# NERSC/swin_v2_weather

Hardware: AMD Instinct MI355X
Metric: ERA5 samples/sec (73x721x1440) swin_73var depth12 (higher is better)
Workload: dtype bf16

## Files before the change

include/swv2.h:

```cpp
#ifndef SWV2_H
#define SWV2_H
#include <stddef.h>
#include <stdint.h>

#ifdef __cplusplus
extern "C" {
#endif

#define SWV2_VERSION 109

enum {
    SWV2_OK = 0,
    SWV2_ERR_INVALID = -1,
    SWV2_ERR_UNSUPPORTED = -2,
    SWV2_ERR_LAUNCH = -3
};

int swv2_version(void);
const char* swv2_last_error(void);

int swv2_attn_geometry(int L, int head_dim, int* Lp, int* DP);

int swv2_attn_fwd_regime(int L, int head_dim, int has_bias, int dbg);

#define SWV2_ATTN_FIRST_GEN 16
#define SWV2_ATTN_PLAIN_STATS 8192
#define SWV2_ATTN_BWD_TWO_PHASE 32

typedef struct swv2_attn_args {
    const void* qkvh;
    const float* logit_scale;
    const float* bias;
    const void* bias_pack;
    void* oh;
    float* lse;
    const void* doh;
    const float* rnorm;
    void* dqkvh;
    float* dlogit_scale;
    float* dbias;
    int Bw, heads, L, head_dim;
    int nwh, nww;
    int mask_thr;
    int max_chunks;
    int dbg;
    void* dbias_ws;
    size_t dbias_ws_bytes;
    int dbias_partials;
} swv2_attn_args;

size_t swv2_attn_dbias_ws_bytes(int heads, int L, int max_chunks);

int swv2_attn_bias_chunks(int Bw);

size_t swv2_attn_pack_bias_bytes(int heads, int L);
int swv2_attn_pack_bias(const float* bias, int heads, int L, void* out, void* stream);
int swv2_attn_pack_bias_multi(const float* bias, int ntab, int heads, int L, void* out, void* stream);

int swv2_attn_fwd(const swv2_attn_args* a, void* stream);
int swv2_attn_bwd(const swv2_attn_args* a, void* stream);


enum swv2_operand_kind {
    SWV2_OP_F32 = 0,
    SWV2_OP_BF16 = 1,
    SWV2_OP_BF16_GELU = 2,
    SWV2_OP_HEADS = 3,
    SWV2_OP_PATCH = 4,
    SWV2_OP_MERGE_LN = 5,
    SWV2_OP_BF16_CSCALE = 6
};

typedef struct swv2_operand {
    int kind;
    const void* ptr;
    const int32_t* rowidx;
    const float* aux0;
    const float* aux1;
    const float* aux2;
    const float* aux3;
    long ld;
    int rows, cols;
    int p[4];
} swv2_operand;

enum swv2_epilogue_kind {
    SWV2_EPI_BF16 = 0,
    SWV2_EPI_F32 = 1,
    SWV2_EPI_QKV_HEADS = 2,
    SWV2_EPI_GELU_GRAD = 3,
    SWV2_EPI_UNPATCH = 4,
    SWV2_EPI_HEADS = 5,
    SWV2_EPI_F32_ACC = 6,
    SWV2_EPI_BF16_GELU = 7,
    SWV2_EPI_UNPATCH_LOSS = 8
};

typedef struct swv2_epilogue {
    int kind;
    void* out;
    const float* bias;
    const void* aux;
    float* aux_out;
    const int32_t* rowidx;
    long ld;
    int p[5];
    const float* loss_tar;
    const float* loss_qw;
    float* loss_part;
    void* loss_resid;
    int q[3];
} swv2_epilogue;

int swv2_linear(const swv2_operand* a, const void* w_bf16, const swv2_epilogue* e, int N, void* stream);

#define SWV2_LINEAR_RESIDENT_QKV128 0
#define SWV2_LINEAR_RESIDENT_QKV192X3 1
#define SWV2_LINEAR_RESIDENT_DX128 2
#define SWV2_LINEAR_WIDE_DMA 3
#define SWV2_LINEAR_WIDE 4
#define SWV2_LINEAR_TILE64 5
#define SWV2_LINEAR_TILE128 6
int swv2_linear_kernel(const swv2_operand* a, const swv2_epilogue* e, int N);

int swv2_linear_wgrad(const swv2_operand* dy, const swv2_operand* x, float* dW, float* db, const int32_t* nmap,
                      const int32_t* kmap, int ldw, int splits, void* stream);
size_t swv2_linear_wgrad_ws_bytes(int M, int N, int K, int splits);
int swv2_linear_wgrad_ws(const swv2_operand* dy, const swv2_operand* x, float* dW, float* db, const int32_t* nmap,
                         const int32_t* kmap, int ldw, int splits, void* ws, size_t ws_bytes, void* stream);
#define SWV2_WGRAD_WIDE 0
#define SWV2_WGRAD_TILE 1
int swv2_linear_wgrad_kernel(const swv2_operand* dy, const swv2_operand* x, int splits, size_t ws_bytes);

typedef struct swv2_wgrad_item {
    swv2_operand dy, x;
    float* dW;
    float* db;
    const int32_t* nmap;
    const int32_t* kmap;
    int ldw;
} swv2_wgrad_item;
size_t swv2_block_wgrad_ws_bytes(int C, int hidden, int heads_dp, int slices);
int swv2_block_wgrad(const swv2_wgrad_item* items4, int slices, void* ws, size_t ws_bytes, void* stream);
#define SWV2_BLOCK_WGRAD_SLAB 0
#define SWV2_BLOCK_WGRAD_GROUPED 1
int swv2_block_wgrad_kernel(const swv2_wgrad_item* items4, int slices, size_t ws_bytes);

int swv2_qk_normalize(void* qkvh_bf16, float* rnorm, int Bw, int heads, int Lp, int L, int DP, void* stream);

int swv2_prep_weight(const float* w, int rows, int cols, int transpose, const int32_t* row_map, int out_rows,
                     const int32_t* col_map, int out_cols, void* out_bf16, void* stream);

typedef struct swv2_prep_item {
    const float* w;
    int rows, cols, transpose;
    const int32_t* row_map;
    int out_rows;
    const int32_t* col_map;
    int out_cols;
    void* out;
    int out_f32;
} swv2_prep_item;
int swv2_prep_chunk(void);
int swv2_prep_item_chunks(int out_rows, int out_cols, int transpose);
int swv2_prep_multi(const swv2_prep_item* items_dev, const int* chunks_dev, int n_chunks, void* stream);

#define SWV2_LN_BWD_MAX_BLOCKS 512
typedef struct swv2_ln_args {
    const void* a;
    const float* res;
    const float* gamma;
    const float* beta;
    const float* scale;
    const int32_t* rowidx;
    float* y;
    float* mean;
    float* rstd;
    const float* dy;
    void* da;
    float* dgamma;
    float* dbeta;
    float* ws;
    int M, C, res_mod, rows_per_sample;
    float eps;
} swv2_ln_args;

int swv2_ln_residual_fwd(const swv2_ln_args* a, void* stream);
int swv2_ln_residual_bwd(const swv2_ln_args* a, void* stream);

int swv2_batch_sum(const float* in, float* out, int B, long n, int accumulate, void* stream);

int swv2_merge_stats(const float* x, float* mean, float* rstd, int B, int H, int W, int C, float eps, void* stream);
int swv2_merge_ln_bwd(const float* x, const void* dn_bf16, const float* gamma, const float* mean, const float* rstd,
                      float* dx, float* dgamma, float* dbeta, int B, int H, int W, int C, void* stream);

int swv2_loss_sums(const float* prd, const float* tar, const float* quad_w, float* sums, int BC, int H, int W, void* stream);
int swv2_loss_grad(const float* prd, const float* tar, const float* quad_w, const float* coef, float* dprd, int BC, int H,
                   int W, void* stream);
#define SWV2_LOSS_PART_SLICES 8
#define SWV2_LOSS_GROUP_ROWS 32
#define SWV2_LOSS_DUMP_BYTES 2048
#define SWV2_LOSS_RESID_PITCH(N) (((N) + 63) / 64 * 64)
int swv2_loss_part_reduce(const float* part, int M, int T, int B, int Cout, int Ct, int coff, float* sums, void* stream);
int swv2_loss_resid_to_image(const void* resid, const float* coef, const float* add, float* out, int B, int Cout, int H, int W, int Cs, int Cadd,
                             void* stream);
int swv2_loss_finalize(const float* sums, int layers, const float* chw, int BC, int C, int absolute, int squared, float* loss, float* coef,
                       void* stream);

int swv2_adam_step(float* p, const float* g, float* m, float* v, long n, float lr, float beta1, float beta2, float eps,
                   int step, float grad_inv_scale, void* stream);

typedef struct swv2_adam_item {
    float* p;
    const float* g;
    float* m;
    float* v;
    long n;
} swv2_adam_item;
int swv2_adam_chunk(void);
int swv2_adam_multi(const swv2_adam_item* items_dev, const int* chunks_dev, int n_chunks, float lr, float beta1, float beta2,
                    float eps, int step, float grad_inv_scale, void* stream);

int swv2_era5_select_normalize(const float* raw, float* out, const int* chan, const float* mean, const float* stdv, int B, int S,
                               int Csel, int Craw, int Hraw, int Wraw, int H, int W, int Cout_total, int coff, void* stream);
int swv2_era5_zenith(float* out, const float* sun, int B, int nz, int H, int W, int Cout_total, int coff, void* stream);
int swv2_era5_static(const float* stat, float* out, int B, int Cs, int H, int W, int Cout_total, int coff, void* stream);

typedef struct {
    const void* oh;
    const void* wp;
    const float* bp;
    const float* gamma; const float* beta; const float* scale;
    const int32_t* rowidx;
    const float* x;
    void* a1; float* mean; float* rstd;
    float* y;
    int Bw, Lp, heads, C, rows_per_sample;
    float eps;
} swv2_proj_ln_args;
typedef struct {
    const float* dy;
    const void* a1; const float* mean; const float* rstd; const float* gamma; const float* scale;
    const int32_t* rowidx;
    const void* wpt;
    void* da1;
    void* doh;
    float* dgamma; float* dbeta; float* ws;
    int Bw, Lp, heads, C, rows_per_sample;
} swv2_proj_ln_bwd_args;
int swv2_proj_ln_supported(int C, int heads, int head_pad);
size_t swv2_proj_ln_bwd_ws_floats(int Mw, int C);
int swv2_proj_ln_fwd(const swv2_proj_ln_args* a, void* stream);
int swv2_proj_ln_bwd(const swv2_proj_ln_bwd_args* a, void* stream);

typedef struct {
    const float* x;
    const void* w1;
    const float* b1;
    const void* w2;
    const float* b2;
    const float* gamma;
    const float* beta;
    const float* scale;
    void* hpre;
    void* a2;
    float* mean;
    float* rstd;
    float* y;
    int M, C, hidden, rows_per_sample;
    float eps;
} swv2_mlp_args;
int swv2_mlp_supported(int C, int hidden);
int swv2_mlp_recompute_supported(int C, int hidden);
int swv2_mlp_fwd(const swv2_mlp_args* a, void* stream);

typedef struct {
    const float* dy;
    const void* a2;
    const float* mean;
    const float* rstd;
    const float* gamma;
    const float* scale;
    const void* hpre;
    const void* w2t;
    const void* w1t;
    void* da2;
    void* dh;
    float* dx;
    float* dgamma;
    float* dbeta;
    float* ws;
    int M, C, hidden, rows_per_sample;
    const float* x;
    const void* w1;
    const float* b1;
} swv2_mlp_bwd_args;
size_t swv2_mlp_bwd_ws_floats(int M, int C);
int swv2_mlp_bwd(const swv2_mlp_bwd_args* a, void* stream);

int swv2_cpb_fwd(const float* w1, const float* b1, const float* w2, const float* b2, const void* keep_bf16, float* bias,
                 int wh, int ww, int heads, int hidden, float drop_p, void* stream);
int swv2_cpb_bwd(const float* dbias, const float* w1, const float* b1, const float* w2, const void* keep_bf16, float* dw1,
                 float* db1, float* dw2, float* db2, int wh, int ww, int heads, int hidden, float drop_p, void* stream);
size_t swv2_cpb_bwd_ws_bytes(int wh, int ww, int heads, int hidden);
int swv2_cpb_bwd_ws(const float* dbias, const float* w1, const float* b1, const float* w2, const void* keep_bf16, float* dw1,
                    float* db1, float* dw2, float* db2, int wh, int ww, int heads, int hidden, float drop_p, void* ws,
                    size_t ws_bytes, void* stream);

int swv2_cpb_fwd_multi(const float* const* params_dev, int nblk, const uint32_t* keep_bits, float* bias, int wh, int ww, int heads,
                       int hidden, float drop_p, void* stream);
size_t swv2_cpb_bwd_multi_ws_bytes(int nblk, int wh, int ww, int heads, int hidden);
int swv2_cpb_bwd_multi(const float* dbias_tables, int nchunk, const float* const* params_dev, int nblk, const uint32_t* keep_bits,
                       float* grads, int wh, int ww, int heads, int hidden, float drop_p, void* ws, size_t ws_bytes, void* stream);

typedef struct swv2_block_desc {
    int B, T, C, heads, head_dim, hidden, L, Lp, DP, nwh, nww, mask_thr;
    const int32_t* rowidx;
    const int32_t* qkv_map;
    const int32_t* proj_map;
    const float *logit_scale, *qkv_b_pad, *proj_b, *n1_w, *n1_b, *fc1_b, *fc2_b, *n2_w, *n2_b;
    const void *w_qkv, *w_proj, *w_fc1, *w_fc2;
    const void *w_qkvt, *w_projt, *w_fc1t, *w_fc2t;
    const float* x;
    const float* bias;
    void* bias_pack;
    const float* dp1;
    const float* dp2;
    void* qkvh;  float* rnorm; void* oh; float* lse; void* a1; float* mean1; float* rstd1; float* x1;
    void* hpre;  void* hact;   void* a2; float* mean2; float* rstd2;
    float* x2;
    const float* dx2;
    void *da2, *dh, *da1, *doh, *dqkvh;
    float* dx1;
    float* ln_ws;
    float* dx;
    float *d_logit_scale, *d_bias, *d_qkv_w, *d_qkv_b, *d_proj_w, *d_proj_b, *d_n1_w, *d_n1_b, *d_fc1_w, *d_fc1_b,
          *d_fc2_w, *d_fc2_b, *d_n2_w, *d_n2_b;
    int wgrad_splits;
    int ev_kernel;
    void* ev_start;
    void* ev_stop;
    int fuse_proj_ln;
    int fuse_mlp;
    void* wgrad_ws;
    size_t wgrad_ws_bytes;
    int wgrad_group;
    void* grad_zero;
    size_t grad_zero_bytes;
    size_t ln_ws_floats;
    int bias_prepacked;
    float* dbias_part;
    size_t dbias_part_bytes;
} swv2_block_desc;

enum swv2_block_step {
    SWV2_STEP_RNORM_ZERO = 1,
    SWV2_STEP_QKV,
    SWV2_STEP_QK_NORMALIZE,
    SWV2_STEP_PACK_BIAS,
    SWV2_STEP_ATTN_FWD,
    SWV2_STEP_PROJ, SWV2_STEP_LN1_FWD,
    SWV2_STEP_PROJ_LN_FWD,
    SWV2_STEP_FC1, SWV2_STEP_FC2, SWV2_STEP_LN2_FWD,
    SWV2_STEP_MLP_FWD,
    SWV2_STEP_LN2_BWD, SWV2_STEP_WGRAD_FC2, SWV2_STEP_DH, SWV2_STEP_WGRAD_FC1, SWV2_STEP_DX1,
    SWV2_STEP_MLP_BWD,
    SWV2_STEP_LN1_BWD,
    SWV2_STEP_PROJ_LN_BWD,
    SWV2_STEP_WGRAD_PROJ, SWV2_STEP_DOH, SWV2_STEP_ATTN_BWD, SWV2_STEP_WGRAD_QKV, SWV2_STEP_DX,
    SWV2_STEP_LN_FOLD,
    SWV2_STEP_WGRAD_GROUP,
    SWV2_STEP_COUNT
};
#define SWV2_BLOCK_MAX_STEPS 12
enum { SWV2_DBIAS_NONE = 0,
       SWV2_DBIAS_ATOMICS = 1,
       SWV2_DBIAS_WGRAD_WS = 2,
       SWV2_DBIAS_PART = 3 };
typedef struct swv2_block_plan_t {
    int mlp_fused;
    int proj_ln_fused;
    int ln_deferred;
    int wgrad_grouped;
    int wgrad_kernel;
    int grad_zero_in_kernel;
    int attn_fwd_chunks, attn_bwd_chunks;
    int dbias_dest;
    size_t need_hact_bytes;
    size_t need_ln_ws_floats;
    size_t need_wgrad_ws_bytes;
    int n_fwd, n_bwd;
    int fwd[SWV2_BLOCK_MAX_STEPS], bwd[SWV2_BLOCK_MAX_STEPS];
} swv2_block_plan_t;
int swv2_block_plan(const swv2_block_desc* d, swv2_block_plan_t* out);
int swv2_block_step_id(int step);
const char* swv2_block_step_name(int step);

int swv2_block_fwd(const swv2_block_desc* d, void* stream);
int swv2_block_bwd(const swv2_block_desc* d, void* stream);

#ifdef __cplusplus
}
#endif
#endif
```

swin_v2_weather_amd/_lib.py:

```python
from __future__ import annotations

import ctypes as C
import os
import subprocess
import threading

HERE = os.path.dirname(os.path.abspath(__file__))
CSRC = os.path.join(HERE, "csrc")
LIB_PATH = os.environ.get("SWV2_LIB") or os.path.join(HERE, "libswv2.so")
SOURCES = ["capi.hip", "attn.hip", "attn2.hip", "attn_bwd_stream.hip", "attn_wide.hip", "attn_d256.hip", "gemm.hip", "gemm_tn.hip", "gemm_tn_slab.hip", "rowops.hip", "block.hip", "cpb.hip", "mlp.hip", "proj_ln.hip", "dataio.hip"]

ABI_VERSION = 109

_lib = None
_lock = threading.Lock()


class Swv2Error(RuntimeError):
    pass


def build_library(force: bool = False, verbose: bool = False) -> str:
    srcs = [os.path.join(CSRC, s) for s in SOURCES]
    deps = srcs + [os.path.join(CSRC, "common.h"), os.path.join(CSRC, "gemm_common.h"), os.path.join(CSRC, "attn_common.h"), os.path.join(HERE, "..", "include", "swv2.h")]
    if not force and os.path.exists(LIB_PATH) and all(os.path.getmtime(LIB_PATH) >= os.path.getmtime(d) for d in deps):
        return LIB_PATH
    hipcc = os.environ.get("HIPCC", "/opt/rocm/bin/hipcc")
    objs, procs = [], []
    os.makedirs(os.path.join(HERE, "build"), exist_ok=True)
    for s in srcs:
        o = os.path.join(HERE, "build", os.path.basename(s) + ".o")
        objs.append(o)
        cmd = [hipcc, "--offload-arch=gfx950", "-O3", "-std=c++17", "-fPIC", "-c", s, "-o", o]
        procs.append((cmd, subprocess.Popen(cmd, stdout=subprocess.PIPE, stderr=subprocess.STDOUT)))
    for cmd, p in procs:
        out, _ = p.communicate()
        if p.returncode != 0:
            raise Swv2Error("hipcc failed: %s\n%s" % (" ".join(cmd), out.decode()))
        if verbose and out:
            print(out.decode())
    cmd = [hipcc, "--offload-arch=gfx950", "-shared", "-fPIC", "-o", LIB_PATH] + objs
    r = subprocess.run(cmd, stdout=subprocess.PIPE, stderr=subprocess.STDOUT)
    if r.returncode != 0:
        raise Swv2Error("link failed: %s\n%s" % (" ".join(cmd), r.stdout.decode()))
    return LIB_PATH


def source_hash() -> str:
    import glob
    import hashlib
    h = hashlib.sha256()
    files = sorted(glob.glob(os.path.join(CSRC, "*"))) + [os.path.join(HERE, "..", "include", "swv2.h")]
    for f in files:
        if os.path.isfile(f):
            h.update(os.path.basename(f).encode())
            h.update(open(f, "rb").read())
    return h.hexdigest()[:16]


class AttnArgs(C.Structure):
    _fields_ = [("qkvh", C.c_void_p), ("logit_scale", C.c_void_p), ("bias", C.c_void_p), ("bias_pack", C.c_void_p), ("oh", C.c_void_p),
                ("lse", C.c_void_p), ("doh", C.c_void_p), ("rnorm", C.c_void_p), ("dqkvh", C.c_void_p),
                ("dlogit_scale", C.c_void_p), ("dbias", C.c_void_p),
                ("Bw", C.c_int), ("heads", C.c_int), ("L", C.c_int), ("head_dim", C.c_int),
                ("nwh", C.c_int), ("nww", C.c_int), ("mask_thr", C.c_int), ("max_chunks", C.c_int), ("dbg", C.c_int),
                ("dbias_ws", C.c_void_p), ("dbias_ws_bytes", C.c_size_t), ("dbias_partials", C.c_int)]


class Operand(C.Structure):
    _fields_ = [("kind", C.c_int), ("ptr", C.c_void_p), ("rowidx", C.c_void_p), ("aux0", C.c_void_p),
                ("aux1", C.c_void_p), ("aux2", C.c_void_p), ("aux3", C.c_void_p), ("ld", C.c_long),
                ("rows", C.c_int), ("cols", C.c_int), ("p", C.c_int * 4)]


class PrepItem(C.Structure):
    _fields_ = [("w", C.c_void_p), ("rows", C.c_int), ("cols", C.c_int), ("transpose", C.c_int), ("row_map", C.c_void_p),
                ("out_rows", C.c_int), ("col_map", C.c_void_p), ("out_cols", C.c_int), ("out", C.c_void_p), ("out_f32", C.c_int)]


class WgradItem(C.Structure):
    _fields_ = [("dy", Operand), ("x", Operand), ("dW", C.c_void_p), ("db", C.c_void_p), ("nmap", C.c_void_p),
                ("kmap", C.c_void_p), ("ldw", C.c_int)]


class Epilogue(C.Structure):
    _fields_ = [("kind", C.c_int), ("out", C.c_void_p), ("bias", C.c_void_p), ("aux", C.c_void_p),
                ("aux_out", C.c_void_p), ("rowidx", C.c_void_p), ("ld", C.c_long), ("p", C.c_int * 5),
                ("loss_tar", C.c_void_p), ("loss_qw", C.c_void_p), ("loss_part", C.c_void_p),
                ("loss_resid", C.c_void_p),
                ("q", C.c_int * 3)]


class ProjLnArgs(C.Structure):
    _fields_ = [(n, C.c_void_p) for n in ("oh", "wp", "bp", "gamma", "beta", "scale", "rowidx", "x", "a1", "mean", "rstd", "y")] + \
               [(n, C.c_int) for n in ("Bw", "Lp", "heads", "C", "rows_per_sample")] + [("eps", C.c_float)]


class ProjLnBwdArgs(C.Structure):
    _fields_ = [(n, C.c_void_p) for n in ("dy", "a1", "mean", "rstd", "gamma", "scale", "rowidx", "wpt", "da1", "doh", "dgamma", "dbeta",
                                           "ws")] + [(n, C.c_int) for n in ("Bw", "Lp", "heads", "C", "rows_per_sample")]


class MlpArgs(C.Structure):
    _fields_ = [(n, C.c_void_p) for n in ("x", "w1", "b1", "w2", "b2", "gamma", "beta", "scale", "hpre", "a2", "mean", "rstd", "y")] + \
               [(n, C.c_int) for n in ("M", "C", "hidden", "rows_per_sample")] + [("eps", C.c_float)]


class MlpBwdArgs(C.Structure):
    _fields_ = [(n, C.c_void_p) for n in ("dy", "a2", "mean", "rstd", "gamma", "scale", "hpre", "w2t", "w1t", "da2", "dh", "dx",
                                           "dgamma", "dbeta", "ws")] + [(n, C.c_int) for n in ("M", "C", "hidden", "rows_per_sample")] + \
               [(n, C.c_void_p) for n in ("x", "w1", "b1")]


class LnArgs(C.Structure):
    _fields_ = [("a", C.c_void_p), ("res", C.c_void_p), ("gamma", C.c_void_p), ("beta", C.c_void_p),
                ("scale", C.c_void_p), ("rowidx", C.c_void_p), ("y", C.c_void_p), ("mean", C.c_void_p),
                ("rstd", C.c_void_p), ("dy", C.c_void_p), ("da", C.c_void_p), ("dgamma", C.c_void_p),
                ("dbeta", C.c_void_p), ("ws", C.c_void_p), ("M", C.c_int), ("C", C.c_int), ("res_mod", C.c_int),
                ("rows_per_sample", C.c_int), ("eps", C.c_float)]


LN_BWD_MAX_BLOCKS = 512
ATTN_FIRST_GEN, ATTN_PLAIN_STATS, ATTN_BWD_TWO_PHASE = 16, 8192, 32
LOSS_PART_SLICES = 8
LOSS_GROUP_ROWS = 32
LOSS_DUMP_BYTES = 2048


def loss_resid_pitch(n: int) -> int:
    return (n + 63) // 64 * 64
class BlockDesc(C.Structure):
    _fields_ = ([(n, C.c_int) for n in ("B", "T", "C", "heads", "head_dim", "hidden", "L", "Lp", "DP", "nwh", "nww", "mask_thr")] +
                [(n, C.c_void_p) for n in (
                    "rowidx", "qkv_map", "proj_map",
                    "logit_scale", "qkv_b_pad", "proj_b", "n1_w", "n1_b", "fc1_b", "fc2_b", "n2_w", "n2_b",
                    "w_qkv", "w_proj", "w_fc1", "w_fc2", "w_qkvt", "w_projt", "w_fc1t", "w_fc2t",
                    "x", "bias", "bias_pack", "dp1", "dp2",
                    "qkvh", "rnorm", "oh", "lse", "a1", "mean1", "rstd1", "x1", "hpre", "hact", "a2", "mean2", "rstd2", "x2",
                    "dx2", "da2", "dh", "da1", "doh", "dqkvh", "dx1", "ln_ws", "dx",
                    "d_logit_scale", "d_bias", "d_qkv_w", "d_qkv_b", "d_proj_w", "d_proj_b", "d_n1_w", "d_n1_b", "d_fc1_w",
                    "d_fc1_b", "d_fc2_w", "d_fc2_b", "d_n2_w", "d_n2_b")] +
                [("wgrad_splits", C.c_int), ("ev_kernel", C.c_int), ("ev_start", C.c_void_p), ("ev_stop", C.c_void_p),
                 ("fuse_proj_ln", C.c_int), ("fuse_mlp", C.c_int), ("wgrad_ws", C.c_void_p), ("wgrad_ws_bytes", C.c_size_t), ("wgrad_group", C.c_int), ("grad_zero", C.c_void_p),
                 ("grad_zero_bytes", C.c_size_t), ("ln_ws_floats", C.c_size_t),
                 ("bias_prepacked", C.c_int), ("dbias_part", C.c_void_p), ("dbias_part_bytes", C.c_size_t)])


BLOCK_MAX_STEPS = 12
DBIAS_NONE, DBIAS_ATOMICS, DBIAS_WGRAD_WS, DBIAS_PART = range(4)


class BlockPlan(C.Structure):
    _fields_ = ([(n, C.c_int) for n in ("mlp_fused", "proj_ln_fused", "ln_deferred", "wgrad_grouped", "wgrad_kernel", "grad_zero_in_kernel",
                                        "attn_fwd_chunks", "attn_bwd_chunks", "dbias_dest")] +
                [(n, C.c_size_t) for n in ("need_hact_bytes", "need_ln_ws_floats", "need_wgrad_ws_bytes")] +
                [("n_fwd", C.c_int), ("n_bwd", C.c_int), ("fwd", C.c_int * BLOCK_MAX_STEPS), ("bwd", C.c_int * BLOCK_MAX_STEPS)])

    def steps(self, phase):
        lib = load()
        return [lib.swv2_block_step_name(s).decode() for s in getattr(self, phase)[:getattr(self, "n_" + phase)]]


def block_plan(desc: BlockDesc) -> BlockPlan:
    plan = BlockPlan()
    check(load().swv2_block_plan(C.byref(desc), C.byref(plan)), "swv2_block_plan")
    return plan


OP_F32, OP_BF16, OP_BF16_GELU, OP_HEADS, OP_PATCH, OP_MERGE_LN, OP_BF16_CSCALE = range(7)
EPI_BF16, EPI_F32, EPI_QKV_HEADS, EPI_GELU_GRAD, EPI_UNPATCH, EPI_HEADS, EPI_F32_ACC, EPI_BF16_GELU, EPI_UNPATCH_LOSS = range(9)
LINEAR_RESIDENT_QKV128, LINEAR_RESIDENT_QKV192X3, LINEAR_RESIDENT_DX128, LINEAR_WIDE_DMA, LINEAR_WIDE, LINEAR_TILE64, LINEAR_TILE128 = range(7)
LINEAR_WIDE_KERNELS, LINEAR_TILE_KERNELS = (LINEAR_WIDE_DMA, LINEAR_WIDE), (LINEAR_TILE64, LINEAR_TILE128)
WGRAD_WIDE, WGRAD_TILE = range(2)
BLOCK_WGRAD_SLAB, BLOCK_WGRAD_GROUPED = range(2)

_P, _I, _L, _F = C.c_void_p, C.c_int, C.c_long, C.c_float
SYMBOLS = {
    "swv2_version": (_I, []),
    "swv2_last_error": (C.c_char_p, []),
    "swv2_attn_geometry": (_I, [_I, _I, C.POINTER(_I), C.POINTER(_I)]),
    "swv2_attn_fwd_regime": (_I, [_I, _I, _I, _I]),
    "swv2_attn_pack_bias_bytes": (C.c_size_t, [_I, _I]),
    "swv2_attn_dbias_ws_bytes": (C.c_size_t, [_I, _I, _I]),
    "swv2_attn_pack_bias": (_I, [_P, _I, _I, _P, _P]),
    "swv2_attn_pack_bias_multi": (_I, [_P, _I, _I, _I, _P, _P]),
    "swv2_attn_bias_chunks": (_I, [_I]),
    "swv2_attn_fwd": (_I, [C.POINTER(AttnArgs), _P]),
    "swv2_attn_bwd": (_I, [C.POINTER(AttnArgs), _P]),
    "swv2_linear": (_I, [C.POINTER(Operand), _P, C.POINTER(Epilogue), _I, _P]),
    "swv2_linear_kernel": (_I, [C.POINTER(Operand), C.POINTER(Epilogue), _I]),
    "swv2_linear_wgrad_kernel": (_I, [C.POINTER(Operand), C.POINTER(Operand), _I, C.c_size_t]),
    "swv2_block_wgrad_kernel": (_I, [C.POINTER(WgradItem), _I, C.c_size_t]),
    "swv2_linear_wgrad": (_I, [C.POINTER(Operand), C.POINTER(Operand), _P, _P, _P, _P, _I, _I, _P]),
    "swv2_linear_wgrad_ws_bytes": (C.c_size_t, [_I, _I, _I, _I]),
    "swv2_qk_normalize": (_I, [_P, _P, _I, _I, _I, _I, _I, _P]),
    "swv2_block_wgrad_ws_bytes": (C.c_size_t, [_I, _I, _I, _I]),
    "swv2_block_wgrad": (_I, [C.POINTER(WgradItem), _I, _P, C.c_size_t, _P]),
    "swv2_linear_wgrad_ws": (_I, [C.POINTER(Operand), C.POINTER(Operand), _P, _P, _P, _P, _I, _I, _P, C.c_size_t, _P]),
    "swv2_prep_weight": (_I, [_P, _I, _I, _I, _P, _I, _P, _I, _P, _P]),
    "swv2_ln_residual_fwd": (_I, [C.POINTER(LnArgs), _P]),
    "swv2_ln_residual_bwd": (_I, [C.POINTER(LnArgs), _P]),
    "swv2_batch_sum": (_I, [_P, _P, _I, _L, _I, _P]),
    "swv2_merge_stats": (_I, [_P, _P, _P, _I, _I, _I, _I, _F, _P]),
    "swv2_merge_ln_bwd": (_I, [_P, _P, _P, _P, _P, _P, _P, _P, _I, _I, _I, _I, _P]),
    "swv2_loss_sums": (_I, [_P, _P, _P, _P, _I, _I, _I, _P]),
    "swv2_loss_grad": (_I, [_P, _P, _P, _P, _P, _I, _I, _I, _P]),
    "swv2_loss_part_reduce": (_I, [_P, _I, _I, _I, _I, _I, _I, _P, _P]),
    "swv2_loss_resid_to_image": (_I, [_P, _P, _P, _P, _I, _I, _I, _I, _I, _I, _P]),
    "swv2_loss_finalize": (_I, [_P, _I, _P, _I, _I, _I, _I, _P, _P, _P]),
    "swv2_prep_chunk": (_I, []),
    "swv2_prep_item_chunks": (_I, [_I, _I, _I]),
    "swv2_prep_multi": (_I, [_P, _P, _I, _P]),
    "swv2_adam_chunk": (_I, []),
    "swv2_adam_multi": (_I, [_P, _P, _I, _F, _F, _F, _F, _I, _F, _P]),
    "swv2_adam_step": (_I, [_P, _P, _P, _P, _L, _F, _F, _F, _F, _I, _F, _P]),
    "swv2_era5_select_normalize": (_I, [_P, _P, _P, _P, _P] + [_I] * 10 + [_P]),
    "swv2_era5_zenith": (_I, [_P, _P, _I, _I, _I, _I, _I, _I, _P]),
    "swv2_era5_static": (_I, [_P, _P, _I, _I, _I, _I, _I, _I, _P]),
    "swv2_proj_ln_supported": (_I, [_I, _I, _I]),
    "swv2_proj_ln_bwd_ws_floats": (C.c_size_t, [_I, _I]),
    "swv2_proj_ln_fwd": (_I, [C.POINTER(ProjLnArgs), _P]),
    "swv2_proj_ln_bwd": (_I, [C.POINTER(ProjLnBwdArgs), _P]),
    "swv2_mlp_supported": (_I, [_I, _I]),
    "swv2_mlp_recompute_supported": (_I, [_I, _I]),
    "swv2_mlp_fwd": (_I, [C.POINTER(MlpArgs), _P]),
    "swv2_mlp_bwd_ws_floats": (C.c_size_t, [_I, _I]),
    "swv2_mlp_bwd": (_I, [C.POINTER(MlpBwdArgs), _P]),
    "swv2_cpb_fwd": (_I, [_P, _P, _P, _P, _P, _P, _I, _I, _I, _I, _F, _P]),
    "swv2_cpb_bwd": (_I, [_P, _P, _P, _P, _P, _P, _P, _P, _P, _I, _I, _I, _I, _F, _P]),
    "swv2_cpb_bwd_ws": (_I, [_P, _P, _P, _P, _P, _P, _P, _P, _P, _I, _I, _I, _I, _F, _P, C.c_size_t, _P]),
    "swv2_cpb_bwd_ws_bytes": (C.c_size_t, [_I, _I, _I, _I]),
    "swv2_cpb_fwd_multi": (_I, [_P, _I, _P, _P, _I, _I, _I, _I, _F, _P]),
    "swv2_cpb_bwd_multi_ws_bytes": (C.c_size_t, [_I, _I, _I, _I, _I]),
    "swv2_cpb_bwd_multi": (_I, [_P, _I, _P, _I, _P, _P, _I, _I, _I, _I, _F, _P, C.c_size_t, _P]),
    "swv2_block_plan": (_I, [C.POINTER(BlockDesc), C.POINTER(BlockPlan)]),
    "swv2_block_step_id": (_I, [_I]),
    "swv2_block_step_name": (C.c_char_p, [_I]),
    "swv2_block_fwd": (_I, [C.POINTER(BlockDesc), _P]),
    "swv2_block_bwd": (_I, [C.POINTER(BlockDesc), _P]),
}


def load() -> C.CDLL:
    global _lib
    if _lib is not None:
        return _lib
    with _lock:
        if _lib is None:
            if not os.path.exists(LIB_PATH):
                raise Swv2Error(f"{LIB_PATH} not found: run `python -c 'import __graft_entry__ as g; g.build()'` "
                                "(the HIP library is required; there is no fallback path)")
            import torch
            lib = C.CDLL(LIB_PATH)
            for name, (res, args) in SYMBOLS.items():
                fn = getattr(lib, name)
                fn.restype, fn.argtypes = res, args
            got = lib.swv2_version()
            if got != ABI_VERSION:
                raise Swv2Error(f"{LIB_PATH} reports ABI revision {got}, this binding mirrors revision {ABI_VERSION} of include/swv2.h: "
                                "rebuild the library (python -c 'import __graft_entry__ as g; g.build()')")
            _lib = lib
    return _lib


def check(rc: int, what: str = "") -> None:
    if rc != 0:
        msg = load().swv2_last_error()
        raise Swv2Error(f"{what} failed with code {rc}: {msg.decode() if msg else ''}")
```

swin_v2_weather_amd/csrc/block.hip:

```cpp
#include "common.h"

namespace {

swv2_operand op(int kind, const void* p, int rows, int cols, long ld, const int32_t* rowidx = nullptr) {
    swv2_operand o = {};
    o.kind = kind; o.ptr = p; o.rowidx = rowidx; o.ld = ld; o.rows = rows; o.cols = cols;
    return o;
}
swv2_operand op_heads(const void* p, int Bw, int heads, int parts, int Lp, int DP) {
    swv2_operand o = op(SWV2_OP_HEADS, p, Bw * Lp, parts * heads * DP, parts);
    o.p[0] = heads; o.p[2] = Lp; o.p[3] = DP;
    return o;
}
swv2_epilogue epi(int kind, void* out, long ld, const float* bias = nullptr, const void* aux = nullptr,
                  float* aux_out = nullptr, const int32_t* rowidx = nullptr) {
    swv2_epilogue e = {};
    e.kind = kind; e.out = out; e.ld = ld; e.bias = bias; e.aux = aux; e.aux_out = aux_out; e.rowidx = rowidx;
    return e;
}
swv2_attn_args attn(const swv2_block_desc* d, int max_chunks) {
    swv2_attn_args a = {};
    a.qkvh = d->qkvh; a.logit_scale = d->logit_scale; a.bias = d->bias; a.bias_pack = d->bias ? d->bias_pack : nullptr;
    a.oh = d->oh; a.lse = d->lse;
    a.Bw = d->B * d->nwh * d->nww; a.heads = d->heads; a.L = d->L; a.head_dim = d->head_dim; a.nwh = d->nwh; a.nww = d->nww;
    a.mask_thr = d->mask_thr; a.max_chunks = max_chunks;
    return a;
}
void wgrad_items(const swv2_block_desc* d, bool fused, swv2_wgrad_item it[4]) {
    const int BT = d->B * d->T, Bw = d->B * d->nwh * d->nww, Mw = Bw * d->Lp, C = d->C, h = d->heads, hid = d->hidden;
    it[0].dy = op(SWV2_OP_BF16, d->da2, BT, C, C);
    it[0].x = fused ? op(SWV2_OP_BF16_GELU, d->hpre, BT, hid, hid) : op(SWV2_OP_BF16, d->hact, BT, hid, hid);
    it[0].dW = d->d_fc2_w; it[0].db = d->d_fc2_b; it[0].ldw = hid;
    it[1].dy = op(SWV2_OP_BF16, d->dh, BT, hid, hid); it[1].x = op(SWV2_OP_F32, d->x1, BT, C, C);
    it[1].dW = d->d_fc1_w; it[1].db = d->d_fc1_b; it[1].ldw = C;
    it[2].dy = op(SWV2_OP_BF16, d->da1, Mw, C, C); it[2].x = op_heads(d->oh, Bw, h, 1, d->Lp, d->DP);
    it[2].dW = d->d_proj_w; it[2].db = d->d_proj_b; it[2].kmap = d->proj_map; it[2].ldw = C;
    it[3].dy = op_heads(d->dqkvh, Bw, h, 3, d->Lp, d->DP); it[3].x = op(SWV2_OP_F32, d->x, Mw, C, C, d->rowidx);
    it[3].dW = d->d_qkv_w; it[3].db = d->d_qkv_b; it[3].nmap = d->qkv_map; it[3].ldw = C;
}
#define TRY(x) do { int rc_ = (x); if (rc_) return rc_; } while (0)

const struct { int id; const char* name; } STEPS[SWV2_STEP_COUNT] = {
    {0, "end"},
    {0, "rnorm_zero"}, {1, "qkv"}, {0, "qk_normalize"}, {0, "pack_bias"}, {2, "attn_fwd"}, {3, "proj"}, {4, "ln1_fwd"}, {3, "proj_ln_fwd"},
    {5, "fc1"}, {6, "fc2"}, {7, "ln2_fwd"}, {5, "mlp_fwd"},
    {11, "ln2_bwd"}, {12, "wgrad_fc2"}, {13, "dh"}, {14, "wgrad_fc1"}, {15, "dx1"}, {13, "mlp_bwd"}, {16, "ln1_bwd"}, {16, "proj_ln_bwd"},
    {17, "wgrad_proj"}, {18, "doh"}, {19, "attn_bwd"}, {20, "wgrad_qkv"}, {21, "dx"}, {0, "ln_fold"}, {22, "wgrad_group"},
};
static_assert(SWV2_STEP_WGRAD_GROUP + 1 == SWV2_STEP_COUNT && SWV2_STEP_MLP_FWD == 12 && SWV2_STEP_LN2_BWD == 13, "STEPS follows enum swv2_block_step");

#define LAUNCH(step, x)                                                                                     \
    do {                                                                                                    \
        const bool t_ = d->ev_kernel == STEPS[step].id && d->ev_start && d->ev_stop;                         \
        if (t_) (void)hipEventRecord((hipEvent_t)d->ev_start, (hipStream_t)st);                             \
        TRY(x);                                                                                             \
        if (t_) (void)hipEventRecord((hipEvent_t)d->ev_stop, (hipStream_t)st);                              \
    } while (0)

int plan_block(const swv2_block_desc* d, swv2_block_plan_t* p) {
    SWV2_CHECK_ARG(d && p, "swv2_block_plan: null descriptor or plan");
    SWV2_CHECK_ARG(d->B > 0 && d->T > 0 && d->C > 0 && d->heads > 0 && d->hidden > 0 && d->Lp > 0 && d->DP > 0 && d->nwh > 0 && d->nww > 0,
                   "swv2_block_plan: non-positive geometry");
    *p = {};
    const int BT = d->B * d->T, Bw = d->B * d->nwh * d->nww, Mw = Bw * d->Lp, C = d->C, h = d->heads, hid = d->hidden;
    const int sp = d->wgrad_splits > 0 ? d->wgrad_splits : 64;
    const size_t ws_bytes = d->wgrad_ws ? d->wgrad_ws_bytes : 0;
    const size_t ln_pair = swv2_mlp_bwd_ws_floats(BT, C) + swv2_proj_ln_bwd_ws_floats(Mw, C);
    p->need_ln_ws_floats = std::max((size_t)SWV2_LN_BWD_MAX_BLOCKS * 2 * C, ln_pair);
    p->need_wgrad_ws_bytes = d->wgrad_group ? swv2_block_wgrad_ws_bytes(C, hid, h * d->DP, 0) : 0;
    const int prod[4][3] = {{BT, C, hid}, {BT, hid, C}, {Mw, C, h * d->DP}, {Mw, 3 * h * d->DP, C}};
    for (const auto& q : prod)
        p->need_wgrad_ws_bytes = std::max(p->need_wgrad_ws_bytes, swv2_linear_wgrad_ws_bytes(q[0], q[1], q[2], sp));

    p->mlp_fused = d->fuse_mlp && swv2_mlp_supported(C, hid);
    p->proj_ln_fused = d->fuse_proj_ln && swv2_proj_ln_supported(C, h, d->DP);
    p->need_hact_bytes = p->mlp_fused ? 0 : (size_t)BT * hid * 2;
    p->ln_deferred = p->mlp_fused && p->proj_ln_fused && d->ln_ws_floats >= ln_pair;
    p->wgrad_grouped = d->wgrad_group && p->mlp_fused && d->wgrad_ws && ws_bytes >= swv2_block_wgrad_ws_bytes(C, hid, h * d->DP, 0);
    p->wgrad_kernel = -1;
    p->grad_zero_in_kernel = p->mlp_fused && d->grad_zero != nullptr;
    p->attn_fwd_chunks = d->bias ? 32 : 64;
    p->attn_bwd_chunks = 64;
    if (d->bias) {
        p->attn_bwd_chunks = swv2_attn_bias_chunks(Bw);
        p->dbias_dest = d->dbias_part ? SWV2_DBIAS_PART : ws_bytes ? SWV2_DBIAS_WGRAD_WS : SWV2_DBIAS_ATOMICS;
    } else if (d->Lp == 176 && h <= 256) {
        p->attn_bwd_chunks = 256 / h;
    }

    auto fwd = [&](int s) { p->fwd[p->n_fwd++] = s; };
    auto bwd = [&](int s) { p->bwd[p->n_bwd++] = s; };
    const bool wide = d->DP > 64;
    if (wide) fwd(SWV2_STEP_RNORM_ZERO);
    fwd(SWV2_STEP_QKV);
    if (wide) fwd(SWV2_STEP_QK_NORMALIZE);
    if (d->bias && d->bias_pack && !d->bias_prepacked) fwd(SWV2_STEP_PACK_BIAS);
    fwd(SWV2_STEP_ATTN_FWD);
    if (p->proj_ln_fused) fwd(SWV2_STEP_PROJ_LN_FWD);
    else { fwd(SWV2_STEP_PROJ); fwd(SWV2_STEP_LN1_FWD); }
    if (p->mlp_fused) fwd(SWV2_STEP_MLP_FWD);
    else { fwd(SWV2_STEP_FC1); fwd(SWV2_STEP_FC2); fwd(SWV2_STEP_LN2_FWD); }

    const bool single = !p->wgrad_grouped;
    if (p->mlp_fused) {
        bwd(SWV2_STEP_MLP_BWD);
        if (single) { bwd(SWV2_STEP_WGRAD_FC2); bwd(SWV2_STEP_WGRAD_FC1); }
    } else {
        bwd(SWV2_STEP_LN2_BWD); bwd(SWV2_STEP_WGRAD_FC2); bwd(SWV2_STEP_DH); bwd(SWV2_STEP_WGRAD_FC1); bwd(SWV2_STEP_DX1);
    }
    bwd(p->proj_ln_fused ? SWV2_STEP_PROJ_LN_BWD : SWV2_STEP_LN1_BWD);
    if (single) bwd(SWV2_STEP_WGRAD_PROJ);
    if (!p->proj_ln_fused) bwd(SWV2_STEP_DOH);
    bwd(SWV2_STEP_ATTN_BWD);
    if (single) bwd(SWV2_STEP_WGRAD_QKV);
    bwd(SWV2_STEP_DX);
    if (p->ln_deferred && single) bwd(SWV2_STEP_LN_FOLD);
    if (p->wgrad_grouped) bwd(SWV2_STEP_WGRAD_GROUP);
    return SWV2_OK;
}

}

extern "C" int swv2_block_step_id(int step) { return step > 0 && step < SWV2_STEP_COUNT ? STEPS[step].id : -1; }
extern "C" const char* swv2_block_step_name(int step) { return step > 0 && step < SWV2_STEP_COUNT ? STEPS[step].name : nullptr; }

extern "C" int swv2_block_plan(const swv2_block_desc* d, swv2_block_plan_t* p) {
    TRY(plan_block(d, p));
    if (p->wgrad_grouped) {
        swv2_wgrad_item it[4] = {};
        wgrad_items(d, true, it);
        p->wgrad_kernel = swv2_block_wgrad_kernel(it, 0, d->wgrad_ws_bytes);
    }
    return SWV2_OK;
}

extern "C" int swv2_block_fwd(const swv2_block_desc* d, void* st) {
    SWV2_CHECK_ARG(d && d->x && d->x2 && d->qkvh && d->rowidx, "swv2_block_fwd: null descriptor field");
    swv2_block_plan_t p;
    TRY(plan_block(d, &p));
    SWV2_CHECK_ARG(d->hact || !p.need_hact_bytes, "swv2_block_fwd: the separate MLP kernels need hact (swv2_block_plan: need_hact_bytes)");
    const int BT = d->B * d->T, Bw = d->B * d->nwh * d->nww, Mw = Bw * d->Lp, C = d->C, h = d->heads, hid = d->hidden;
    for (int i = 0; i < p.n_fwd; ++i) switch (p.fwd[i]) {
    case SWV2_STEP_RNORM_ZERO:
        if (hipMemsetAsync(d->rnorm, 0, (size_t)Bw * h * 2 * d->Lp * sizeof(float), (hipStream_t)st) != hipSuccess) {
            swv2_set_error("swv2_block_fwd: hipMemsetAsync(rnorm) failed");
            return SWV2_ERR_LAUNCH;
        }
        break;
    case SWV2_STEP_QKV: {
        swv2_operand a = op(SWV2_OP_F32, d->x, Mw, C, C, d->rowidx);
        swv2_epilogue e = epi(SWV2_EPI_QKV_HEADS, d->qkvh, 0, d->qkv_b_pad, nullptr, d->rnorm);
        e.p[0] = h; e.p[2] = d->Lp; e.p[3] = d->DP; e.p[4] = d->L;
        LAUNCH(SWV2_STEP_QKV, swv2_linear(&a, d->w_qkv, &e, 3 * h * d->DP, st));
    } break;
    case SWV2_STEP_QK_NORMALIZE: TRY(swv2_qk_normalize(d->qkvh, (float*)d->rnorm, Bw, h, d->Lp, d->L, d->DP, st)); break;
    case SWV2_STEP_PACK_BIAS: TRY(swv2_attn_pack_bias(d->bias, h, d->L, d->bias_pack, st)); break;
    case SWV2_STEP_ATTN_FWD: {
        swv2_attn_args a = attn(d, p.attn_fwd_chunks);
        LAUNCH(SWV2_STEP_ATTN_FWD, swv2_attn_fwd(&a, st));
    } break;
    case SWV2_STEP_PROJ_LN_FWD: {
        swv2_proj_ln_args m = {};
        m.oh = d->oh; m.wp = d->w_proj; m.bp = d->proj_b; m.gamma = d->n1_w; m.beta = d->n1_b; m.scale = d->dp1; m.rowidx = d->rowidx;
        m.x = d->x; m.a1 = d->a1; m.mean = d->mean1; m.rstd = d->rstd1; m.y = d->x1; m.Bw = Bw; m.Lp = d->Lp; m.heads = h; m.C = C;
        m.rows_per_sample = d->T; m.eps = 1e-5f;
        LAUNCH(SWV2_STEP_PROJ_LN_FWD, swv2_proj_ln_fwd(&m, st));
    } break;
    case SWV2_STEP_PROJ: {
        swv2_operand a = op_heads(d->oh, Bw, h, 1, d->Lp, d->DP);
        swv2_epilogue e = epi(SWV2_EPI_BF16, d->a1, C, d->proj_b);
        LAUNCH(SWV2_STEP_PROJ, swv2_linear(&a, d->w_proj, &e, C, st));
    } break;
    case SWV2_STEP_LN1_FWD: {
        swv2_ln_args l = {};
        l.a = d->a1; l.res = d->x; l.gamma = d->n1_w; l.beta = d->n1_b; l.scale = d->dp1; l.rowidx = d->rowidx; l.y = d->x1;
        l.mean = d->mean1; l.rstd = d->rstd1; l.M = Mw; l.C = C; l.res_mod = 0; l.rows_per_sample = d->T; l.eps = 1e-5f;
        LAUNCH(SWV2_STEP_LN1_FWD, swv2_ln_residual_fwd(&l, st));
    } break;
    case SWV2_STEP_MLP_FWD: {
        swv2_mlp_args m = {};
        m.x = d->x1; m.w1 = d->w_fc1; m.b1 = d->fc1_b; m.w2 = d->w_fc2; m.b2 = d->fc2_b; m.gamma = d->n2_w; m.beta = d->n2_b;
        m.scale = d->dp2; m.hpre = d->hpre; m.a2 = d->a2; m.mean = d->mean2; m.rstd = d->rstd2; m.y = d->x2;
        m.M = BT; m.C = C; m.hidden = hid; m.rows_per_sample = d->T; m.eps = 1e-5f;
        LAUNCH(SWV2_STEP_MLP_FWD, swv2_mlp_fwd(&m, st));
    } break;
    case SWV2_STEP_FC1: {
        swv2_operand a = op(SWV2_OP_F32, d->x1, BT, C, C);
        swv2_epilogue e = epi(SWV2_EPI_BF16_GELU, d->hpre, hid, d->fc1_b, nullptr, (float*)d->hact);
        LAUNCH(SWV2_STEP_FC1, swv2_linear(&a, d->w_fc1, &e, hid, st));
    } break;
    case SWV2_STEP_FC2: {
        swv2_operand a = op(SWV2_OP_BF16, d->hact, BT, hid, hid);
        swv2_epilogue e = epi(SWV2_EPI_BF16, d->a2, C, d->fc2_b);
        LAUNCH(SWV2_STEP_FC2, swv2_linear(&a, d->w_fc2, &e, C, st));
    } break;
    case SWV2_STEP_LN2_FWD: {
        swv2_ln_args l = {};
        l.a = d->a2; l.res = d->x1; l.gamma = d->n2_w; l.beta = d->n2_b; l.scale = d->dp2; l.y = d->x2; l.mean = d->mean2;
        l.rstd = d->rstd2; l.M = BT; l.C = C; l.res_mod = 0; l.rows_per_sample = d->T; l.eps = 1e-5f;
        LAUNCH(SWV2_STEP_LN2_FWD, swv2_ln_residual_fwd(&l, st));
    } break;
    }
    return SWV2_OK;
}

extern "C" int swv2_block_bwd(const swv2_block_desc* d, void* st) {
    SWV2_CHECK_ARG(d && d->dx2 && d->dx && d->da2 && d->dh && d->dx1 && d->da1 && d->doh && d->dqkvh && d->ln_ws,
                   "swv2_block_bwd: null descriptor field");
    swv2_block_plan_t p;
    TRY(plan_block(d, &p));
    SWV2_CHECK_ARG(d->hact || !p.need_hact_bytes, "swv2_block_bwd: the separate MLP kernels need hact (swv2_block_plan: need_hact_bytes)");
    const int BT = d->B * d->T, Bw = d->B * d->nwh * d->nww, Mw = Bw * d->Lp, C = d->C, h = d->heads, hid = d->hidden;
    const int sp = d->wgrad_splits > 0 ? d->wgrad_splits : 64;
    swv2_wgrad_item it[4] = {};
    wgrad_items(d, p.mlp_fused, it);
    float* const ln1_ws = p.ln_deferred ? d->ln_ws + swv2_mlp_bwd_ws_floats(BT, C) : d->ln_ws;
    int n_ln1 = 0, n_ln2 = 0;
    for (int i = 0; i < p.n_bwd; ++i) switch (const int s = p.bwd[i]; s) {
    case SWV2_STEP_MLP_BWD: {
        swv2_mlp_bwd_args m = {};
        m.dy = d->dx2; m.a2 = d->a2; m.mean = d->mean2; m.rstd = d->rstd2; m.gamma = d->n2_w; m.scale = d->dp2; m.hpre = d->hpre;
        m.w2t = d->w_fc2t; m.w1t = d->w_fc1t; m.da2 = d->da2; m.dh = d->dh; m.dx = d->dx1; m.dgamma = d->d_n2_w;
        m.dbeta = d->d_n2_b; m.ws = d->ln_ws; m.M = BT; m.C = C; m.hidden = hid; m.rows_per_sample = d->T;
        LAUNCH(SWV2_STEP_MLP_BWD, swv2_mlp_bwd_impl(&m, st, p.ln_deferred ? &n_ln2 : nullptr, p.grad_zero_in_kernel ? (float*)d->grad_zero : nullptr,
                                                    (long)(d->grad_zero_bytes / 4)));
    } break;
    case SWV2_STEP_LN2_BWD: {
        swv2_ln_args l = {};
        l.a = d->a2; l.dy = d->dx2; l.gamma = d->n2_w; l.scale = d->dp2; l.mean = d->mean2; l.rstd = d->rstd2; l.da = d->da2;
        l.dgamma = d->d_n2_w; l.dbeta = d->d_n2_b; l.ws = d->ln_ws; l.M = BT; l.C = C; l.rows_per_sample = d->T;
        LAUNCH(SWV2_STEP_LN2_BWD, swv2_ln_residual_bwd(&l, st));
    } break;
    case SWV2_STEP_WGRAD_FC2: case SWV2_STEP_WGRAD_FC1: case SWV2_STEP_WGRAD_PROJ: case SWV2_STEP_WGRAD_QKV: {
        const swv2_wgrad_item& w = it[s == SWV2_STEP_WGRAD_FC2 ? 0 : s == SWV2_STEP_WGRAD_FC1 ? 1 : s == SWV2_STEP_WGRAD_PROJ ? 2 : 3];
        LAUNCH(s, swv2_linear_wgrad_ws(&w.dy, &w.x, w.dW, w.db, w.nmap, w.kmap, w.ldw, sp, d->wgrad_ws, d->wgrad_ws_bytes, st));
    } break;
    case SWV2_STEP_DH: {
        swv2_epilogue e = epi(SWV2_EPI_GELU_GRAD, d->dh, hid, nullptr, d->hpre);
        LAUNCH(SWV2_STEP_DH, swv2_linear(&it[0].dy, d->w_fc2t, &e, hid, st));
    } break;
    case SWV2_STEP_DX1: {
        swv2_epilogue e = epi(SWV2_EPI_F32, d->dx1, C, nullptr, d->dx2);
        LAUNCH(SWV2_STEP_DX1, swv2_linear(&it[1].dy, d->w_fc1t, &e, C, st));
    } break;
    case SWV2_STEP_PROJ_LN_BWD: {
        swv2_proj_ln_bwd_args m = {};
        m.dy = d->dx1; m.a1 = d->a1; m.mean = d->mean1; m.rstd = d->rstd1; m.gamma = d->n1_w; m.scale = d->dp1; m.rowidx = d->rowidx;
        m.wpt = d->w_projt; m.da1 = d->da1; m.doh = d->doh; m.dgamma = d->d_n1_w; m.dbeta = d->d_n1_b; m.ws = ln1_ws;
        m.Bw = Bw; m.Lp = d->Lp; m.heads = h; m.C = C; m.rows_per_sample = d->T;
        LAUNCH(SWV2_STEP_PROJ_LN_BWD, swv2_proj_ln_bwd_impl(&m, st, p.ln_deferred ? &n_ln1 : nullptr));
    } break;
    case SWV2_STEP_LN1_BWD: {
        swv2_ln_args l = {};
        l.a = d->a1; l.dy = d->dx1; l.gamma = d->n1_w; l.scale = d->dp1; l.rowidx = d->rowidx; l.mean = d->mean1; l.rstd = d->rstd1;
        l.da = d->da1; l.dgamma = d->d_n1_w; l.dbeta = d->d_n1_b; l.ws = d->ln_ws; l.M = Mw; l.C = C; l.rows_per_sample = d->T;
        LAUNCH(SWV2_STEP_LN1_BWD, swv2_ln_residual_bwd(&l, st));
    } break;
    case SWV2_STEP_DOH: {
        swv2_epilogue e = epi(SWV2_EPI_HEADS, d->doh, 0);
        e.p[0] = h; e.p[2] = d->Lp; e.p[3] = d->DP; e.p[4] = d->L;
        LAUNCH(SWV2_STEP_DOH, swv2_linear(&it[2].dy, d->w_projt, &e, h * d->DP, st));
    } break;
    case SWV2_STEP_ATTN_BWD: {
        swv2_attn_args a = attn(d, p.attn_bwd_chunks);
        a.doh = d->doh; a.rnorm = d->rnorm; a.dqkvh = d->dqkvh; a.dlogit_scale = d->d_logit_scale; a.dbias = d->d_bias;
        if (p.dbias_dest == SWV2_DBIAS_PART) { a.dbias_ws = d->dbias_part; a.dbias_ws_bytes = d->dbias_part_bytes; a.dbias_partials = 1; }
        if (p.dbias_dest == SWV2_DBIAS_WGRAD_WS) { a.dbias_ws = d->wgrad_ws; a.dbias_ws_bytes = d->wgrad_ws_bytes; }
        LAUNCH(SWV2_STEP_ATTN_BWD, swv2_attn_bwd(&a, st));
    } break;
    case SWV2_STEP_DX: {
        swv2_epilogue e = epi(SWV2_EPI_F32, d->dx, C, nullptr, d->dx1, nullptr, d->rowidx);
        LAUNCH(SWV2_STEP_DX, swv2_linear(&it[3].dy, d->w_qkvt, &e, C, st));
    } break;
    case SWV2_STEP_LN_FOLD:
        swv2_launch_ln_partials_reduce2(d->ln_ws, d->d_n2_w, d->d_n2_b, n_ln2, ln1_ws, d->d_n1_w, d->d_n1_b, n_ln1, C, (hipStream_t)st);
        break;
    case SWV2_STEP_WGRAD_GROUP: {
        swv2_ln_partials lnp = {{d->ln_ws, ln1_ws}, {d->d_n2_w, d->d_n1_w}, {d->d_n2_b, d->d_n1_b}, {n_ln2, n_ln1}, C};
        LAUNCH(SWV2_STEP_WGRAD_GROUP, swv2_block_wgrad_ln(it, 0, d->wgrad_ws, d->wgrad_ws_bytes, p.ln_deferred ? &lnp : nullptr, st));
    } break;
    }
    return SWV2_OK;
}
```

swin_v2_weather_amd/csrc/common.h:

```cpp
#pragma once
#include <hip/hip_runtime.h>
#include <stdint.h>
#include <stdio.h>
#include <type_traits>

#include "../../include/swv2.h"

typedef short bf16x4 __attribute__((ext_vector_type(4)));
typedef short bf16x8 __attribute__((ext_vector_type(8)));
typedef __bf16 bf4_t __attribute__((ext_vector_type(4)));
typedef __bf16 bf2_t __attribute__((ext_vector_type(2)));
typedef float f32x4 __attribute__((ext_vector_type(4)));
typedef float f32x2 __attribute__((ext_vector_type(2)));

#define SWV2_LOG2E 1.4426950408889634f
#define SWV2_LN100 4.605170185988092f
#define SWV2_NEG_BIG (-1.0e30f)

__device__ __forceinline__ float bf2f(uint16_t v) { return __uint_as_float(((uint32_t)v) << 16); }
__device__ __forceinline__ float bf2f(short v) { return __uint_as_float(((uint32_t)(uint16_t)v) << 16); }
__device__ __forceinline__ uint16_t f2bf(float f) { return __builtin_bit_cast(uint16_t, (__bf16)f); }
__device__ __forceinline__ uint32_t f2bf2(float lo, float hi) {
    f32x2 v = {lo, hi};
    return __builtin_bit_cast(uint32_t, __builtin_convertvector(v, bf2_t));
}
__device__ __forceinline__ bf16x4 f2bf4(f32x4 v) {
    const uint32_t p[2] = {f2bf2(v[0], v[1]), f2bf2(v[2], v[3])};
    return __builtin_bit_cast(bf16x4, p);
}

__device__ __forceinline__ f32x4 mfma16(bf16x4 a, bf16x4 b, f32x4 c) {
    return __builtin_amdgcn_mfma_f32_16x16x16bf16_1k(a, b, c, 0, 0, 0);
}
__device__ __forceinline__ f32x4 mfma32(bf16x8 a, bf16x8 b, f32x4 c) {
    return __builtin_amdgcn_mfma_f32_16x16x32_bf16(a, b, c, 0, 0, 0);
}
typedef __attribute__((address_space(3))) bf16x4 lds_bf16x4;
__device__ __forceinline__ bf16x4 lds_tr_read(const uint16_t* p) {
    return __builtin_amdgcn_ds_read_tr16_b64_v4i16((lds_bf16x4*)p);
}

__device__ __forceinline__ float wave_sum(float v) {
#pragma unroll
    for (int o = 32; o > 0; o >>= 1) v += __shfl_xor(v, o);
    return v;
}

__device__ __forceinline__ float wave_sum_dpp63(float v) {
    auto dpp = [](float x, auto ctrl, auto rmask) {
        return __builtin_bit_cast(float, __builtin_amdgcn_update_dpp(0, __builtin_bit_cast(int, x), decltype(ctrl)::value, decltype(rmask)::value, 0xf, true));
    };
    v += dpp(v, std::integral_constant<int, 0xb1>{}, std::integral_constant<int, 0xf>{});
    v += dpp(v, std::integral_constant<int, 0x4e>{}, std::integral_constant<int, 0xf>{});
    v += dpp(v, std::integral_constant<int, 0x141>{}, std::integral_constant<int, 0xf>{});
    v += dpp(v, std::integral_constant<int, 0x140>{}, std::integral_constant<int, 0xf>{});
    v += dpp(v, std::integral_constant<int, 0x142>{}, std::integral_constant<int, 0xa>{});
    v += dpp(v, std::integral_constant<int, 0x143>{}, std::integral_constant<int, 0xc>{});
    return v;
}

#ifdef SWV2_ALLSUM_SHFL
__device__ __forceinline__ float xor16_allsum(float x) { return x + __shfl_xor(x, 16); }
__device__ __forceinline__ float xor32_allsum(float x) { return x + __shfl_xor(x, 32); }
template <int G>
__device__ __forceinline__ float group_allsum(float v) {
#pragma unroll
    for (int o = 1; o < G; o <<= 1) v += __shfl_xor(v, o);
    return v;
}
#else
__device__ __forceinline__ float xor16_allsum(float x) {
    float y = x;
    asm volatile("s_nop 1\n\tv_permlane16_swap_b32 %0, %1\n\ts_nop 1" : "+v"(x), "+v"(y));
    return x + y;
}
__device__ __forceinline__ float xor32_allsum(float x) {
    float y = x;
    asm volatile("s_nop 1\n\tv_permlane32_swap_b32 %0, %1\n\ts_nop 1" : "+v"(x), "+v"(y));
    return x + y;
}
template <int G>
__device__ __forceinline__ float group_allsum(float v) {
    static_assert(G == 1 || G == 2 || G == 4 || G == 8 || G == 16 || G == 32 || G == 64, "power-of-two lane groups");
    auto dpp = [](float x, auto ctrl) {
        return __builtin_bit_cast(float, __builtin_amdgcn_update_dpp(0, __builtin_bit_cast(int, x), decltype(ctrl)::value, 0xf, 0xf, true));
    };
    if constexpr (G >= 2) v += dpp(v, std::integral_constant<int, 0xb1>{});
    if constexpr (G >= 4) v += dpp(v, std::integral_constant<int, 0x4e>{});
    if constexpr (G >= 8) v += dpp(v, std::integral_constant<int, 0x141>{});
    if constexpr (G >= 16) v += dpp(v, std::integral_constant<int, 0x140>{});
    if constexpr (G >= 32) v = xor16_allsum(v);
    if constexpr (G >= 64) v = xor32_allsum(v);
    return v;
}
#endif

void swv2_set_error(const char* fmt, ...);
#define SWV2_CHECK_ARG(cond, ...)                 \
    do {                                          \
        if (!(cond)) {                            \
            swv2_set_error(__VA_ARGS__);          \
            return SWV2_ERR_INVALID;              \
        }                                         \
    } while (0)
#define SWV2_CHECK_LAUNCH(name)                                                      \
    do {                                                                             \
        hipError_t e_ = hipGetLastError();                                           \
        if (e_ != hipSuccess) {                                                      \
            swv2_set_error("%s: launch failed: %s", name, hipGetErrorString(e_));    \
            return SWV2_ERR_LAUNCH;                                                  \
        }                                                                            \
    } while (0)

void swv2_launch_ln_partials_reduce(const float* ws, float* dgamma, float* dbeta, int nblocks, int C, hipStream_t st);
void swv2_launch_ln_partials_reduce2(const float* ws1, float* dg1, float* db1, int n1, const float* ws2, float* dg2, float* db2,
                                     int n2, int C, hipStream_t st);
int swv2_mlp_bwd_impl(const swv2_mlp_bwd_args* a, void* stream, int* deferred, float* zero, long zero_n);
int swv2_proj_ln_bwd_impl(const swv2_proj_ln_bwd_args* a, void* stream, int* deferred);

struct swv2_ln_partials { const float* ws[2]; float* dgamma[2]; float* dbeta[2]; int n[2]; int C; };
int swv2_block_wgrad_ln(const swv2_wgrad_item* items4, int slices, void* ws, size_t ws_bytes, const swv2_ln_partials* ln, void* stream);

static inline int cdiv(long a, long b) { return (int)((a + b - 1) / b); }
```

swin_v2_weather_amd/csrc/gemm.hip:

```cpp
#include "common.h"

#include <cmath>
#include <cstdlib>
#include "gemm_common.h"

namespace {

constexpr int EP = 68;

struct EpiDesc {
    void* out;
    const float* bias;
    const void* aux;
    float* aux_out;
    const int32_t* rowidx;
    long ld;
    int M, N;
    int p0, p1, p2, p3, p4;
    uint32_t mg0, mg1, mg2;
    const float* loss_tar; const float* loss_qw; float* loss_part; uint16_t* loss_resid; int q0, q1, q2, q3;
};

enum { E_BF16 = 0, E_F32 = 1, E_QKV_HEADS = 2, E_GELU_GRAD = 3, E_UNPATCH = 4, E_HEADS = 5, E_F32_ACC = 6, E_BF16_GELU = 7,
       E_UNPATCH_LOSS = 8, E_UNPATCH_LOSS_SKIP = 9 };
// ... 799 lines not shown
                bf[j] = __builtin_shufflevector(trf(Xs, 0, wc * 64 + 16 * j), trf(Xs, 16, wc * 64 + 16 * j), 0, 1, 2, 3, 4, 5, 6, 7);
#pragma unroll
            for (int i = 0; i < 8; ++i)
                af[i] = __builtin_shufflevector(trf(Ys, 0, wr * 128 + 16 * i), trf(Ys, 16, wr * 128 + 16 * i), 0, 1, 2, 3, 4, 5, 6, 7);
            if (want_db && ((t0 + t) % ntk) == tk) {
                const uint4 a = *(const uint4*)(Ys + cs_off), b = *(const uint4*)(Ys + cs_off + 16 * 256);
                float va[8], vb[8];
                unpack8(a, va); unpack8(b, vb);
#pragma unroll
                for (int e = 0; e < 8; ++e) cs[e] += va[e] + vb[e];
            }
            asm volatile("s_waitcnt vmcnt(8)" ::: "memory");
            asm volatile("s_waitcnt lgkmcnt(0)" ::: "memory");
            __builtin_amdgcn_sched_barrier(0);
            __builtin_amdgcn_s_barrier();
            __builtin_amdgcn_sched_barrier(0);
            __builtin_amdgcn_s_setprio(1);
#pragma unroll
            for (int i = 0; i < 8; ++i)
#pragma unroll
                for (int j = 0; j < 4; ++j) acc[i][j] = mfma32(af[i], bf[j], acc[i][j]);
            __builtin_amdgcn_s_setprio(0);
            __builtin_amdgcn_sched_barrier(0);
            __builtin_amdgcn_s_barrier();
            __builtin_amdgcn_sched_barrier(0);
        }
        if (wr == 0) __builtin_amdgcn_s_barrier();
        asm volatile("s_waitcnt vmcnt(0)" ::: "memory");
    }
    __syncthreads();
    Epi<E_F32> ep;
    ep.d.out = part + (size_t)slice * N * K; ep.d.bias = nullptr; ep.d.aux = nullptr; ep.d.aux_out = nullptr; ep.d.rowidx = nullptr;
    ep.d.ld = K; ep.d.M = N; ep.d.N = K;
    wide_epilogue<E_F32>(ep, acc, (float*)smem + wave * 16 * EP, n_base + wr * 128, k_base + wc * 64, lane);
    if (want_db) {
        __syncthreads();
        float* red = (float*)smem;
#pragma unroll
        for (int e = 0; e < 8; ++e) red[(tid >> 5) * 256 + (tid & 31) * 8 + e] = cs[e];
        __syncthreads();
        if (tid < 256) {
            float sum = 0.f;
#pragma unroll
            for (int r = 0; r < 16; ++r) sum += red[r * 256 + tid];
            dbpart[((size_t)slice * ntk + tk) * N + n_base + tid] = sum;
        }
    }
}

template <int AK, int EK>
__global__ __launch_bounds__(WTH) void gemm_nt_wide_kernel(ALoad<AK> al, const uint16_t* __restrict__ Wb, Epi<EK> ep,
                                                           int M, int N, int K, int mtiles, int ntn) {
    static_assert(!ALoad<AK>::ROW_FASTEST, "row-major staging map only");
    constexpr int TILE = (WBM + WBN) * BK;
    __shared__ __attribute__((aligned(1024))) uint16_t smem[2 * TILE];
    static_assert(2 * TILE * 2 >= 8 * 16 * EP * 4, "the epilogue staging re-uses the tile buffers");
    const int tid = threadIdx.x, lane = tid & 63, wave = __builtin_amdgcn_readfirstlane(tid >> 6);
    const int fr = lane & 15, g = lane >> 4;
    const int wr = wave >> 2, wc = wave & 3;
    int mt, nt;
    if (!wide_tile(blockIdx.x & 7, blockIdx.x >> 3, mtiles, ntn, mt, nt)) return;
    const int m_base = mt * WBM, n_base = nt * WBN;
    const uint32_t lds0 = (uint32_t)(uintptr_t)smem;
    f32x4 acc[8][4];
#pragma unroll
    for (int i = 0; i < 8; ++i)
#pragma unroll
        for (int j = 0; j < 4; ++j) acc[i][j] = (f32x4){0.f, 0.f, 0.f, 0.f};
    {
        const int ksteps = K / BK;
        const int drow = wave * 32 + (lane >> 3);
        uint32_t boff[4];
#pragma unroll
        for (int i = 0; i < 4; ++i) {
            const int row = drow + 8 * i, kcl = (lane & 7) ^ ((row >> 1) & 7);
            boff[i] = 2u * (uint32_t)((n_base + row) * K + kcl * 8);
        }
        typename ALoad<AK>::Raw ra[4];
        int arow[4];
        uint32_t aok = 0;
        const int kc = tid & 7;
#pragma unroll
        for (int i = 0; i < 4; ++i) {
            const int src = al.row_of(m_base + (tid >> 3) + 64 * i);
            arow[i] = max(src, 0);
            aok |= (src >= 0 ? 1u : 0u) << i;
        }
        auto issue = [&](int s, int buf) {
            const uint32_t lb = lds0 + (uint32_t)(buf * TILE * 2) + (uint32_t)(wave * 4096) + WBM * BK * 2;
#pragma unroll
            for (int i = 0; i < 4; ++i) dma_x4(Wb + s * BK, boff[i], lb + 1024 * i);
#pragma unroll
            for (int i = 0; i < 4; ++i) ra[i] = al.raw_unc(arow[i], s * BK + kc * 8);
        };
        auto commit = [&](int buf) {
            uint16_t* As = smem + buf * TILE;
#pragma unroll
            for (int i = 0; i < 4; ++i) {
                uint4 v = al.cvt(ra[i]);
                if (!((aok >> i) & 1)) v = make_uint4(0, 0, 0, 0);
                *(uint4*)(As + swz((tid >> 3) + 64 * i, kc)) = v;
            }
        };
        auto compute = [&](int buf) {
            const uint16_t* As = smem + buf * TILE;
            const uint16_t* Bs = As + WBM * BK;
#pragma unroll
            for (int kk = 0; kk < 2; ++kk) {
                bf16x8 bf[4];
#pragma unroll
                for (int j = 0; j < 4; ++j) bf[j] = *(const bf16x8*)(Bs + swz(wc * 64 + j * 16 + fr, kk * 4 + g));
#pragma unroll
                for (int i = 0; i < 8; ++i) {
                    const bf16x8 af = *(const bf16x8*)(As + swz(wr * 128 + i * 16 + fr, kk * 4 + g));
#pragma unroll
                    for (int j = 0; j < 4; ++j) acc[i][j] = mfma32(af, bf[j], acc[i][j]);
                }
            }
        };
        issue(0, 0);
        asm volatile("s_waitcnt vmcnt(0)" ::: "memory");
        commit(0);
        __syncthreads();
        for (int s = 0; s + 1 < ksteps; ++s) {
            issue(s + 1, (s + 1) & 1);
            __builtin_amdgcn_sched_barrier(0);
            compute(s & 1);
            __builtin_amdgcn_sched_barrier(0);
            asm volatile("s_waitcnt vmcnt(0)" ::: "memory");
            commit((s + 1) & 1);
            __syncthreads();
        }
        compute((ksteps - 1) & 1);
        __syncthreads();
    }
    wide_epilogue<EK>(ep, acc, (float*)smem + wave * 16 * EP, m_base + wr * 128, n_base + wc * 64, lane);
}

#ifdef SWV2_RW_STAMPS
__device__ unsigned long long rw_stamps[256 * 8];
#define RSTAMP_DECL unsigned long long st_prev = 0, st_acc[8] = {0, 0, 0, 0, 0, 0, 0, 0};
#define RSTAMP_START() do { asm volatile("s_memtime %0\n\ts_waitcnt lgkmcnt(0)" : "=s"(st_prev) : : "memory"); } while (0)
#define RSTAMP(k) do { unsigned long long t_; asm volatile("s_memtime %0\n\ts_waitcnt lgkmcnt(0)" : "=s"(t_) : : "memory"); \
                       st_acc[k] += t_ - st_prev; st_prev = t_; } while (0)
#define RSTAMP_WAITV() asm volatile("s_waitcnt vmcnt(0)" ::: "memory")
#else
#define RSTAMP_DECL
#define RSTAMP_START() do {} while (0)
#define RSTAMP(k) do {} while (0)
#define RSTAMP_WAITV() do {} while (0)
#endif
__device__ __forceinline__ int swzk(int r, int kc, int K) { return r * K + ((kc ^ ((r >> 1) & 7)) << 3); }

template <int AK, int EK, int N, int K, int BMT, int HS = 16>
__global__ __launch_bounds__(512) void gemm_rw_kernel(ALoad<AK> al, const uint16_t* __restrict__ Wb, Epi<EK> ep, int M) {
    constexpr int NTH = 512, KC = K / 8;
    constexpr int ACH = BMT * KC / NTH;
    constexpr int RT = BMT / 64;
    constexpr int CT = N / 32;
    constexpr int WCH = N * KC / NTH;
    constexpr int A_BYTES = BMT * K * 2, ST_BYTES = 8 * 16 * EP * 4;
    constexpr int AS_BYTES = A_BYTES > ST_BYTES ? A_BYTES : ST_BYTES;
    static_assert(BMT * KC % NTH == 0 && N * KC % NTH == 0 && K % 64 == 0 && N % 64 == 0, "tile shapes");
    static_assert(N * K * 2 + AS_BYTES <= 160 * 1024, "LDS budget");
    __shared__ __attribute__((aligned(16))) uint16_t Ws[N * K];
    __shared__ __attribute__((aligned(16))) unsigned char as_raw[AS_BYTES];
    __shared__ __attribute__((aligned(16))) float bs[N];
    uint16_t* As = (uint16_t*)as_raw;
    float* stage_all = (float*)as_raw;

    const int tid = threadIdx.x, lane = tid & 63, wave = tid >> 6;
    const int fr = lane & 15, g = lane >> 4;
    const int wr = wave >> 1, wc = wave & 1;
    const int ntiles = (M + BMT - 1) / BMT;
    static_assert(EK != E_F32 || (RT == 1 && CT == 4), "the E_F32 prefetch below covers one 16 x 64 wave tile");
    for (int i = tid; i < N; i += NTH) bs[i] = ep.d.bias ? ep.d.bias[i] : 0.f;
    int erow_nxt = -1, erow_cur = -1;
    f32x4 aux_nxt[4], aux_cur[4];
    const int ecol = wc * (N / 2) + (lane & 3) * 16;

    typename ALoad<AK>::Raw ra[ACH];
    int arow[ACH];
    int erow_res = -1;
    auto crow = [&](int c) { return AK == A_HEADS ? ((c >> 1) & (BMT - 1)) : c / KC; };
    auto ccol = [&](int c) { return AK == A_HEADS ? (((c / (2 * BMT)) << 1) | (c & 1)) : c % KC; };
    static_assert(AK != A_HEADS || (BMT & (BMT - 1)) == 0, "head-major chunk map needs a power-of-two tile height");
    uint32_t ain = 0;
    uint32_t aok = 0;
    bool ein = false;
    auto resolve = [&](int t) {
        ain = 0;
#pragma unroll
        for (int i = 0; i < ACH; ++i) {
            const int c = tid + i * NTH, m = t * BMT + crow(c);
            const bool in = (t < ntiles) && (m < M);
            ain |= (uint32_t)in << i;
            if constexpr (AK == A_F32) arow[i] = al.d.rowidx[min(m, M - 1)];
            else arow[i] = min(m, M - 1);
        }
        if constexpr (EK == E_F32) {
            const int m = t * BMT + wr * 16 + (lane >> 2);
            ein = (t < ntiles) && (m < M);
            erow_res = ein ? ep.d.rowidx[m] : -1;
        }
    };
    auto issue = [&]() {
        aok = 0;
#pragma unroll
        for (int i = 0; i < ACH; ++i) {
            const int c = tid + i * NTH;
            const int r = ((ain >> i) & 1) ? arow[i] : -1;
            if constexpr (AK == A_HEADS) ra[i] = al.raw_at(r, ccol(c) * 8);
            else ra[i] = al.raw_unc(max(r, 0), ccol(c) * 8);
            aok |= (uint32_t)(r >= 0) << i;
        }
        if constexpr (EK == E_F32) {
            erow_nxt = ein ? erow_res : -1;
            const float* ax = (const float*)ep.d.aux + (long)max(erow_nxt, 0) * ep.d.ld + ecol;
#pragma unroll
            for (int i = 0; i < 4; ++i) aux_nxt[i] = *(const f32x4*)(ax + 4 * i);
        }
    };
    auto commit = [&]() {
#pragma unroll
        for (int i = 0; i < ACH; ++i) {
            const int c = tid + i * NTH;
            *(uint4*)(As + swzk(crow(c), ccol(c), K)) = ((aok >> i) & 1) ? al.cvt(ra[i]) : make_uint4(0, 0, 0, 0);
        }
    };
    const int G = gridDim.x;
    RSTAMP_DECL
    auto tile_step = [&](int t) {
        RSTAMP_WAITV();
        RSTAMP(0);
        commit();
        if constexpr (EK == E_F32) {
            erow_cur = erow_nxt;
#pragma unroll
            for (int i = 0; i < 4; ++i) aux_cur[i] = aux_nxt[i];
        }
        RSTAMP(1);
        __syncthreads();
        RSTAMP(2);
        issue();
        resolve(t + 2 * G);
        RSTAMP(3);
        f32x4 acc[RT][CT];
#pragma unroll
        for (int i = 0; i < RT; ++i)
#pragma unroll
            for (int j = 0; j < CT; ++j) acc[i][j] = (f32x4){0.f, 0.f, 0.f, 0.f};
#pragma unroll
        for (int ks = 0; ks < K / 32; ++ks) {
            bf16x8 af[RT];
#pragma unroll
            for (int i = 0; i < RT; ++i) af[i] = *(const bf16x8*)(As + swzk(wr * 16 * RT + i * 16 + fr, ks * 4 + g, K));
#pragma unroll
            for (int j = 0; j < CT; ++j) {
                const bf16x8 bf = *(const bf16x8*)(Ws + swzk(wc * (N / 2) + j * 16 + fr, ks * 4 + g, K));
#pragma unroll
                for (int i = 0; i < RT; ++i) acc[i][j] = mfma32(af[i], bf, acc[i][j]);
            }
        }
        asm volatile("" :: "v"(acc[0][0][0]), "v"(acc[RT - 1][CT - 1][3]));
        RSTAMP(4);
        __syncthreads();
        RSTAMP(5);
        float* st = stage_all + wave * 16 * EP;
#pragma unroll
        for (int i = 0; i < RT; ++i)
#pragma unroll
            for (int j0 = 0; j0 < CT; j0 += 4) {
#pragma unroll
                for (int j = 0; j < 4; ++j)
#pragma unroll
                    for (int r = 0; r < 4; ++r) st[(4 * g + r) * EP + 16 * j + fr] = acc[i][j0 + j][r];
                const int m0 = t * BMT + wr * 16 * RT + i * 16, n0 = wc * (N / 2) + j0 * 16;
                if constexpr (EK == E_QKV_HEADS) {
                    const EpiDesc& d = ep.d;
                    const int h = d.p0, Lp = d.p2, L = d.p4;
                    const int r = lane & 15, slot = lane >> 4, nb = n0 + slot * 16, m = m0 + r;
                    if (m < d.M) {
                        const int ph = HS == 16 ? nb >> 4 : nb >> 5, lp = (h == 1) ? ph : fdiv(ph, h, d.mg1), hd = ph - lp * h;
                        const int part = lp + d.p1;
                        const int bw = fdiv(m, Lp, d.mg0), tt = m - bw * Lp;
                        const bool valid = tt < L;
                        float v[16];
                        float ss = 0.f;
#pragma unroll
                        for (int j = 0; j < 16; j += 4) {
                            const f32x4 x = *(const f32x4*)(st + r * EP + slot * 16 + j) + *(const f32x4*)(bs + nb + j);
#pragma unroll
                            for (int e = 0; e < 4; ++e) {
                                v[j + e] = valid ? x[e] : 0.f;
                                ss = fmaf(v[j + e], v[j + e], ss);
                            }
                        }
                        if constexpr (HS == 32) ss += __shfl_xor(ss, 16);
                        float rn = 1.f;
                        if (part < 2) {
                            rn = 1.f / fmaxf(sqrtf(ss), 1e-12f);
                            if (HS == 16 || !(slot & 1)) d.aux_out[(((long)bw * h + hd) * 2 + part) * Lp + tt] = valid ? rn : 0.f;
                        }
                        uint16_t* o = (uint16_t*)d.out + ((((long)bw * h + hd) * 3 + part) * Lp + tt) * HS + (HS == 32 ? (slot & 1) * 16 : 0);
                        float w8[8];
#pragma unroll
                        for (int e = 0; e < 8; ++e) w8[e] = v[e] * rn;
                        *(uint4*)o = pack8(w8);
#pragma unroll
                        for (int e = 0; e < 8; ++e) w8[e] = v[8 + e] * rn;
                        *(uint4*)(o + 8) = pack8(w8);
                    }
                } else if constexpr (EK == E_F32) {
                    if (erow_cur >= 0) {
                        float* o = (float*)ep.d.out + (long)erow_cur * ep.d.ld + ecol;
                        const int r = lane >> 2, c0 = (lane & 3) * 16;
#pragma unroll
                        for (int q = 0; q < 4; ++q)
                            *(f32x4*)(o + 4 * q) = *(const f32x4*)(st + r * EP + c0 + 4 * q) + *(const f32x4*)(bs + ecol + 4 * q) + aux_cur[q];
                    }
                } else {
                    ep.tile(st, m0, n0, lane);
                }
            }
        RSTAMP(6);
        __syncthreads();
        RSTAMP(7);
    };
    int t = blockIdx.x;
    resolve(t);
    issue();
    resolve(t + G);
#pragma unroll
    for (int i = 0; i < WCH; ++i) {
        const int c = tid + i * NTH, n = c / KC, kc = c - n * KC;
        *(uint4*)(Ws + swzk(n, kc, K)) = *(const uint4*)(Wb + (long)n * K + kc * 8);
    }

    RSTAMP_START();
    for (; t < ntiles; t += G) tile_step(t);
#ifdef SWV2_RW_STAMPS
    if (tid == 0)
        for (int k = 0; k < 8; ++k) rw_stamps[blockIdx.x * 8 + k] = st_acc[k];
#endif
}

enum class LinearKernel {
    RESIDENT_QKV128 = SWV2_LINEAR_RESIDENT_QKV128, RESIDENT_QKV192X3 = SWV2_LINEAR_RESIDENT_QKV192X3, RESIDENT_DX128 = SWV2_LINEAR_RESIDENT_DX128,
    WIDE_DMA = SWV2_LINEAR_WIDE_DMA, WIDE = SWV2_LINEAR_WIDE, TILE64 = SWV2_LINEAR_TILE64, TILE128 = SWV2_LINEAR_TILE128
};

constexpr bool qkv_pair(int ak, int ek) { return ak == A_F32 && ek == E_QKV_HEADS; }
constexpr bool dx_pair(int ak, int ek) { return ak == A_HEADS && ek == E_F32; }
constexpr bool loss_epi(int ek) { return ek == E_UNPATCH_LOSS || ek == E_UNPATCH_LOSS_SKIP; }
constexpr bool wide_pair(int ak, int ek) {
    return (ak == A_F32 || ak == A_BF16 || ak == A_HEADS) &&
           (ek == E_BF16 || ek == E_F32 || ek == E_F32_ACC || ek == E_QKV_HEADS || ek == E_HEADS || ek == E_GELU_GRAD || ek == E_BF16_GELU);
}
constexpr bool dma_loader(int ak) { return ak == A_BF16 || ak == A_HEADS; }

LinearKernel linear_kernel_for(int ak, int ek, const swv2_operand* a, const swv2_epilogue* e, int N, int wide) {
    const int M = a->rows, K = a->cols;
    if (qkv_pair(ak, ek) && M >= 256 * 128 && a->rowidx) {
        if (N == 384 && K == 128 && e->p[3] == 16) return LinearKernel::RESIDENT_QKV128;
        if (N == 768 && K == 192 && e->p[3] == 32 && e->p[0] == 8) return LinearKernel::RESIDENT_QKV192X3;
    }
    if (dx_pair(ak, ek) && N == 128 && K == 384 && M >= 256 * 64 && e->rowidx && e->aux && !a->rowidx) return LinearKernel::RESIDENT_DX128;
    if (wide_pair(ak, ek)) {
        const bool part192 = dx_pair(ak, ek) && N == 192 && K == 768 && !a->rowidx && M >= 64 * WBM &&
                             (double)a->rows * a->cols * 2 < 4.29e9;
        if (wide && (N % WBN == 0 || part192) && K % BK == 0 && (N >= 512 || part192) && K >= 512 && M >= 16 * WBM) {
            const bool small = (double)a->rows * (ak == A_HEADS ? a->cols : a->ld) * 2 < 4.29e9;
            return dma_loader(ak) && small && K % 128 == 0 && (ak == A_HEADS || !a->rowidx) ? LinearKernel::WIDE_DMA : LinearKernel::WIDE;
        }
    }
    if (loss_epi(ek)) return LinearKernel::TILE64;
    if (qkv_pair(ak, ek) || dx_pair(ak, ek)) {
        const double w1 = cdiv(M, BM), w2 = cdiv(M, BM / 2), slots = 768.0;
        const double e1 = w1 / (std::ceil(w1 / slots) * slots), e2 = w2 / (std::ceil(w2 / slots) * slots);
        if (e2 > e1 + 0.08) return LinearKernel::TILE64;
    }
    return LinearKernel::TILE128;
}

int linear_epi_kind(int ak, const swv2_epilogue* e) {
    static_assert(E_BF16 == SWV2_EPI_BF16 && E_BF16_GELU == SWV2_EPI_BF16_GELU && A_F32 == SWV2_OP_F32 && A_BF16_CS == SWV2_OP_BF16_CSCALE,
                  "A_* / E_* mirror the public kinds");
    if (ak == A_BF16_CS) {
        if (e->kind == SWV2_EPI_F32) return E_F32;
        swv2_set_error("swv2_linear: SWV2_OP_BF16_CSCALE supports SWV2_EPI_F32 only (got %d)", e->kind);
        return SWV2_ERR_INVALID;
    }
    if (ak == A_F32 && e->kind == SWV2_EPI_UNPATCH_LOSS) return e->p[3] ? E_UNPATCH_LOSS_SKIP : E_UNPATCH_LOSS;
    if (e->kind >= SWV2_EPI_BF16 && e->kind <= SWV2_EPI_BF16_GELU) return e->kind;
    swv2_set_error("swv2_linear: unknown epilogue kind %d (or not available for operand kind %d)", e->kind, ak);
    return SWV2_ERR_INVALID;
}

template <int EK>
Epi<EK> make_epi(const swv2_epilogue* e, int M, int N) {
    Epi<EK> ep;
    ep.d.out = e->out; ep.d.bias = e->bias; ep.d.aux = e->aux; ep.d.aux_out = e->aux_out; ep.d.rowidx = e->rowidx;
    ep.d.ld = e->ld; ep.d.M = M; ep.d.N = N;
    ep.d.p0 = e->p[0]; ep.d.p1 = e->p[1]; ep.d.p2 = e->p[2]; ep.d.p3 = e->p[3]; ep.d.p4 = e->p[4];
    ep.d.mg0 = ep.d.mg1 = ep.d.mg2 = 0;
    ep.d.loss_tar = nullptr; ep.d.loss_qw = nullptr; ep.d.loss_part = nullptr; ep.d.loss_resid = nullptr; ep.d.q0 = ep.d.q1 = ep.d.q2 = ep.d.q3 = 0;
    if (EK == E_QKV_HEADS || EK == E_HEADS) { ep.d.mg0 = fdiv_magic(e->p[2]); ep.d.mg1 = fdiv_magic(e->p[0]); ep.d.mg2 = fdiv_magic(e->p[3]); }
    if (EK == E_UNPATCH || loss_epi(EK)) { ep.d.mg0 = fdiv_magic((e->p[1] / 4) * (e->p[2] / 4)); ep.d.mg1 = fdiv_magic(e->p[2] / 4); }
    if (loss_epi(EK)) {
        ep.d.loss_tar = e->loss_tar; ep.d.loss_qw = e->loss_qw; ep.d.loss_part = e->loss_part; ep.d.loss_resid = (uint16_t*)e->loss_resid;
        ep.d.q0 = e->q[0]; ep.d.q1 = e->q[1];
        const long nb = M / ((e->p[1] / 4) * (e->p[2] / 4)), plane = (long)e->p[1] * e->p[2];
        ep.d.q2 = e->q[2] ? e->q[2] : (int)(nb * e->p[0] * plane);
        ep.d.q3 = (int)(nb * e->ld * plane);
    }
    return ep;
}

template <int AK, int EK>
int launch_nt2(const swv2_operand* a, const void* w, const swv2_epilogue* e, int M, int N, int K, hipStream_t st) {
    const Epi<EK> ep = make_epi<EK>(e, M, N);
    const uint16_t* wb = (const uint16_t*)w;
    const LinearKernel kern = linear_kernel_for(AK, EK, a, e, N, swv2_gemm_wide());
    switch (kern) {
        case LinearKernel::RESIDENT_QKV128:
            if constexpr (qkv_pair(AK, EK)) {
                Epi<EK> ep1 = ep;
                ep1.d.p1 = 0;
                hipLaunchKernelGGL((gemm_rw_kernel<AK, EK, 384, 128, 128>), dim3(256), dim3(512), 0, st, make_loader<AK>(a), wb, ep1, M);
            }
            break;
        case LinearKernel::RESIDENT_QKV192X3:
            if constexpr (qkv_pair(AK, EK)) {
                for (int part = 0; part < 3; ++part) {
                    Epi<EK> ep2 = ep;
                    ep2.d.N = 256;
                    ep2.d.p1 = part;
                    ep2.d.bias = e->bias ? e->bias + 256 * part : nullptr;
                    hipLaunchKernelGGL((gemm_rw_kernel<AK, EK, 256, 192, 128, 32>), dim3(256), dim3(512), 0, st, make_loader<AK>(a),
                                       wb + (size_t)part * 256 * 192, ep2, M);
                }
            }
            break;
        case LinearKernel::RESIDENT_DX128:
            if constexpr (dx_pair(AK, EK))
                hipLaunchKernelGGL((gemm_rw_kernel<AK, EK, 128, 384, 64>), dim3(256), dim3(512), 0, st, make_loader<AK>(a), wb, ep, M);
            break;
        case LinearKernel::WIDE_DMA:
        case LinearKernel::WIDE:
            if constexpr (wide_pair(AK, EK)) {
                SWV2_CHECK_ARG((double)N * K * 2 < 4.29e9, "swv2_linear: weight too large for the wide kernel's 32-bit offsets");
                const int mtiles = cdiv(M, WBM), ntn = cdiv(N, WBN), groups = cdiv(mtiles, 8);
                const int vmax = cdiv(groups, 8) * 8 * ntn;
                if (kern == LinearKernel::WIDE_DMA) {
                    if constexpr (dma_loader(AK))
                        hipLaunchKernelGGL((gemm_nt_wide_dma_kernel<AK, EK>), dim3(8 * (vmax < 32 || !swv2_wide_persist() ? vmax : 32)), dim3(WTH), 0, st,
                                           make_loader<AK>(a), wb, ep, M, N, K, mtiles, ntn, vmax);
                } else {
                    hipLaunchKernelGGL((gemm_nt_wide_kernel<AK, EK>), dim3(8 * vmax), dim3(WTH), 0, st, make_loader<AK>(a), wb, ep, M, N, K, mtiles, ntn);
                }
            }
            break;
        case LinearKernel::TILE64:
            if constexpr (qkv_pair(AK, EK) || dx_pair(AK, EK) || loss_epi(EK))
                hipLaunchKernelGGL((gemm_nt_kernel<AK, EK, BM / 2>), dim3(cdiv(M, BM / 2)), dim3(NTHREADS), 0, st, make_loader<AK>(a), wb, ep, M, N, K);
            break;
        case LinearKernel::TILE128:
            if constexpr (!loss_epi(EK))
                hipLaunchKernelGGL((gemm_nt_kernel<AK, EK>), dim3(cdiv(M, BM)), dim3(NTHREADS), 0, st, make_loader<AK>(a), wb, ep, M, N, K);
            break;
    }
    SWV2_CHECK_LAUNCH("swv2_linear");
    return SWV2_OK;
}

template <int AK>
int launch_nt1(const swv2_operand* a, const void* w, const swv2_epilogue* e, int M, int N, int K, hipStream_t st) {
    const int ek = linear_epi_kind(AK, e);
    if (ek < 0) return ek;
    if constexpr (AK == A_BF16_CS) {
        return launch_nt2<AK, E_F32>(a, w, e, M, N, K, st);
    } else {
    if constexpr (AK == A_F32) {
        if (ek == E_UNPATCH_LOSS_SKIP) return launch_nt2<AK, E_UNPATCH_LOSS_SKIP>(a, w, e, M, N, K, st);
        if (ek == E_UNPATCH_LOSS) return launch_nt2<AK, E_UNPATCH_LOSS>(a, w, e, M, N, K, st);
    }
    switch (ek) {
        case E_BF16: return launch_nt2<AK, E_BF16>(a, w, e, M, N, K, st);
        case E_F32: return launch_nt2<AK, E_F32>(a, w, e, M, N, K, st);
        case E_F32_ACC: return launch_nt2<AK, E_F32_ACC>(a, w, e, M, N, K, st);
        case E_QKV_HEADS: return launch_nt2<AK, E_QKV_HEADS>(a, w, e, M, N, K, st);
        case E_HEADS: return launch_nt2<AK, E_HEADS>(a, w, e, M, N, K, st);
        case E_GELU_GRAD: return launch_nt2<AK, E_GELU_GRAD>(a, w, e, M, N, K, st);
        case E_UNPATCH: return launch_nt2<AK, E_UNPATCH>(a, w, e, M, N, K, st);
        case E_BF16_GELU: return launch_nt2<AK, E_BF16_GELU>(a, w, e, M, N, K, st);
    }
    return SWV2_ERR_INVALID;
    }
}

}

int swv2_tn_wide_launch(const swv2_operand* y, const swv2_operand* x, float* part, float* dbpart, int M, int N, int K, int S, hipStream_t st) {
    const int tiles = (N / WBM) * (K / WBN), wgs = S * tiles, per_xcd = cdiv(wgs, 8);
#define SWV2_TNW(YK_, XK_)                                                                                                           \
    hipLaunchKernelGGL((gemm_tn_wide_kernel<YK_, XK_>), dim3(8 * per_xcd), dim3(WTH), 0, st, make_loader<YK_>(y), make_loader<XK_>(x), part, \
                       dbpart, M, N, K, S, wgs, per_xcd)
    if (y->kind == SWV2_OP_BF16 && x->kind == SWV2_OP_BF16) SWV2_TNW(A_BF16, A_BF16);
    else if (y->kind == SWV2_OP_BF16 && x->kind == SWV2_OP_HEADS) SWV2_TNW(A_BF16, A_HEADS);
    else if (y->kind == SWV2_OP_HEADS && x->kind == SWV2_OP_BF16) SWV2_TNW(A_HEADS, A_BF16);
    else { swv2_set_error("swv2_linear_wgrad: wide kernel: operand pair (%d, %d) not instantiated", y->kind, x->kind); return SWV2_ERR_UNSUPPORTED; }
#undef SWV2_TNW
    SWV2_CHECK_LAUNCH("swv2_linear_wgrad");
    return SWV2_OK;
}

#ifdef SWV2_RW_STAMPS
extern "C" int swv2_debug_rw_stamps(void* out) {
    return hipMemcpyFromSymbol(out, HIP_SYMBOL(rw_stamps), sizeof(unsigned long long) * 256 * 8) == hipSuccess ? 0 : -3;
}
#endif

extern "C" int swv2_linear_kernel(const swv2_operand* a, const swv2_epilogue* e, int N) {
    SWV2_CHECK_ARG(a && e && N > 0 && a->rows > 0 && a->cols > 0, "swv2_linear_kernel: null operand / epilogue or empty product");
    SWV2_CHECK_ARG(a->kind >= SWV2_OP_F32 && a->kind <= SWV2_OP_BF16_CSCALE, "swv2_linear_kernel: unknown operand kind %d", a->kind);
    const int ek = linear_epi_kind(a->kind, e);
    return ek < 0 ? ek : (int)linear_kernel_for(a->kind, ek, a, e, N, swv2_gemm_wide());
}

extern "C" int swv2_linear(const swv2_operand* a, const void* w_bf16, const swv2_epilogue* e, int N, void* stream) {
    int rc = check_operand(a, "swv2_linear");
    if (rc) return rc;
    SWV2_CHECK_ARG(w_bf16 && e && e->out && N > 0, "swv2_linear: null weight / epilogue / N");
    SWV2_CHECK_ARG(((uintptr_t)w_bf16 & 15) == 0 && ((uintptr_t)e->out & 15) == 0, "swv2_linear: unaligned pointer");
    if (e->kind == SWV2_EPI_BF16_GELU) SWV2_CHECK_ARG(e->aux_out != nullptr, "swv2_linear: GELU epilogue needs aux_out");
    if (e->kind == SWV2_EPI_BF16 || e->kind == SWV2_EPI_GELU_GRAD || e->kind == SWV2_EPI_BF16_GELU)
        SWV2_CHECK_ARG(e->ld % 8 == 0 && e->ld >= N, "swv2_linear: output pitch %ld must be a multiple of 8 and >= N", e->ld);
    if (e->kind == SWV2_EPI_F32 || e->kind == SWV2_EPI_F32_ACC)
        SWV2_CHECK_ARG(e->ld % 4 == 0 && e->ld >= N, "swv2_linear: output pitch %ld must be a multiple of 4 and >= N", e->ld);
    if (e->kind == SWV2_EPI_QKV_HEADS || e->kind == SWV2_EPI_HEADS)
        SWV2_CHECK_ARG((e->p[3] == 16 || e->p[3] == 32 || e->p[3] == 64 || e->p[3] == 96 || e->p[3] == 128 || e->p[3] == 256) && N % e->p[3] == 0 && e->p[0] > 0 && e->p[2] > 0,
                       "swv2_linear: head-split epilogue needs DP in {16,32,64,96,128,256} and N a multiple of DP (DP=%d N=%d)", e->p[3], N);
    if (e->kind == SWV2_EPI_UNPATCH || e->kind == SWV2_EPI_UNPATCH_LOSS)
        SWV2_CHECK_ARG(N == e->p[0] * 16, "swv2_linear: un-patchify needs N == Cout*16");
    if (e->kind == SWV2_EPI_UNPATCH_LOSS) {
        SWV2_CHECK_ARG(a->kind == SWV2_OP_F32, "swv2_linear: the loss epilogue takes an fp32 operand");
        SWV2_CHECK_ARG((e->p[4] == 0 || (e->p[4] >= e->p[0] && e->q[2] > 0)) && (!e->aux_out || e->ld >= e->p[0]) && e->q[2] >= 0,
                       "swv2_linear: loss epilogue: p[4] (channels of the destination tensor) needs q[2] (its dump offset), aux_out needs ld >= Cout");
        SWV2_CHECK_ARG(e->loss_tar && e->loss_qw && e->loss_part && e->loss_resid && e->q[0] >= e->q[1] + e->p[0] && e->q[1] >= 0,
                       "swv2_linear: the loss epilogue needs target, quadrature weights, sums, residual and q[1] + Cout <= q[0]");
        SWV2_CHECK_ARG((((uintptr_t)e->loss_tar | (uintptr_t)e->loss_resid) & 15) == 0, "swv2_linear: unaligned loss pointer");
        const double plane_ = (double)e->p[1] * e->p[2], nb_ = (double)a->rows / ((e->p[1] / 4) * (e->p[2] / 4));
        SWV2_CHECK_ARG((e->p[1] / 4) * (e->p[2] / 4) >= SWV2_LOSS_GROUP_ROWS, "swv2_linear: the loss epilogue needs at least %d patches per sample", SWV2_LOSS_GROUP_ROWS);
        const double cmax_ = fmax(fmax((double)e->p[3], (double)e->p[0]), fmax((double)e->p[4], e->aux_out ? (double)e->ld : 0.0));
        SWV2_CHECK_ARG(nb_ * e->q[0] * plane_ < 4.29e9 && nb_ * cmax_ * plane_ + 1024 < 4.29e9 && (double)a->rows * SWV2_LOSS_RESID_PITCH(N) + 2048 < 4.29e9 && (double)e->q[2] < 4.29e9,
                       "swv2_linear: the loss epilogue indexes its tensors with 32-bit element offsets (tensor too large)");
    }
    const int M = a->rows, K = a->cols;
    hipStream_t st = (hipStream_t)stream;
    switch (a->kind) {
        case SWV2_OP_F32: return launch_nt1<A_F32>(a, w_bf16, e, M, N, K, st);
        case SWV2_OP_BF16: return launch_nt1<A_BF16>(a, w_bf16, e, M, N, K, st);
        case SWV2_OP_BF16_GELU: return launch_nt1<A_BF16_GELU>(a, w_bf16, e, M, N, K, st);
        case SWV2_OP_HEADS: return launch_nt1<A_HEADS>(a, w_bf16, e, M, N, K, st);
        case SWV2_OP_PATCH: return launch_nt1<A_PATCH>(a, w_bf16, e, M, N, K, st);
        case SWV2_OP_MERGE_LN: return launch_nt1<A_MERGE_LN>(a, w_bf16, e, M, N, K, st);
        case SWV2_OP_BF16_CSCALE: return launch_nt1<A_BF16_CS>(a, w_bf16, e, M, N, K, st);
    }
    swv2_set_error("swv2_linear: unknown operand kind %d", a->kind);
    return SWV2_ERR_INVALID;
}
```

swin_v2_weather_amd/csrc/gemm_common.h:

```cpp
#pragma once
#include <cstdlib>
#include "common.h"

int swv2_tn_wide_launch(const swv2_operand* y, const swv2_operand* x, float* part, float* dbpart, int M, int N, int K, int S, hipStream_t st);

size_t swv2_tn_slab_ws_bytes(int C, int hidden, int heads_dp);
bool swv2_tn_slab_covers(const swv2_wgrad_item* it, size_t ws_bytes);
int swv2_tn_slab_launch(const swv2_wgrad_item* it, void* ws, size_t ws_bytes, const swv2_ln_partials* ln, hipStream_t st);

inline int swv2_env_switch(const char* name) { const char* v = getenv(name); return v ? atoi(v) : 1; }
inline int swv2_gemm_wide() { return swv2_env_switch("SWV2_GEMM_WIDE"); }
inline int swv2_wide_persist() { return swv2_env_switch("SWV2_WIDE_PERSIST"); }

namespace {

constexpr int BM = 128, BN = 128, BK = 64;
constexpr int KCH = BK / 8;
constexpr int NTHREADS = 256;

__device__ __forceinline__ int swz(int r, int kc) { return r * BK + ((kc ^ ((r >> 1) & 7)) << 3); }

__device__ __forceinline__ void erf_parts(float x, float& erf_v, float& gauss) {
    const float z = fabsf(x) * 0.70710678118654752f;
    const float t = __builtin_amdgcn_rcpf(fmaf(0.3275911f, z, 1.f));
    gauss = __expf(-z * z);
    const float poly = t * fmaf(t, fmaf(t, fmaf(t, fmaf(t, 1.061405429f, -1.453152027f), 1.421413741f), -0.284496736f), 0.254829592f);
    const float e = fmaf(-poly, gauss, 1.f);
    erf_v = copysignf(e, x);
}
__device__ __forceinline__ int fdiv(int n, int d, uint32_t magic) {
    int q = (int)__umulhi((uint32_t)n, magic);
    return q - (q * d > n);
}
static inline uint32_t fdiv_magic(int d) { return d > 1 ? (uint32_t)((0x100000000ull + (uint64_t)d - 1) / (uint64_t)d) : 0u; }

__device__ __forceinline__ float gelu_f(float x) {
    float e, gs;
    erf_parts(x, e, gs);
    return 0.5f * x * (1.f + e);
}
__device__ __forceinline__ float gelu_grad_f(float x) {
    float e, gs;
    erf_parts(x, e, gs);
    return fmaf(x * 0.3989422804014327f, gs, 0.5f * (1.f + e));
}

constexpr int GT_LO = (127 - 14) << 7;
constexpr int GT_HALF = 18 * 128;
constexpr int GT_N = 2 * GT_HALF;
typedef unsigned short u16x2_t __attribute__((ext_vector_type(2)));

__device__ __forceinline__ uint16_t gelu_tab_arg(int i) { return (uint16_t)(((i / GT_HALF) << 15) | (GT_LO + i % GT_HALF)); }

template <int ESZ>
__device__ __forceinline__ uint32_t gelu_tab_off2(uint32_t w, bool& bad) {
    const u16x2_t a = __builtin_bit_cast(u16x2_t, w & 0x7fff7fffu);
    const u16x2_t lo = {(unsigned short)GT_LO, (unsigned short)GT_LO};
    const u16x2_t mx = {(unsigned short)(GT_HALF - 1), (unsigned short)(GT_HALF - 1)};
    const u16x2_t idx = a - lo;
    const u16x2_t idc = __builtin_elementwise_min(idx, mx);
    bad = bad || (__builtin_bit_cast(uint32_t, idx) != __builtin_bit_cast(uint32_t, idc));
    const u16x2_t sg = __builtin_bit_cast(u16x2_t, w) >> 15;
    const u16x2_t half = {(unsigned short)GT_HALF, (unsigned short)GT_HALF};
    const u16x2_t off = (idc + sg * half) * (unsigned short)ESZ;
    return __builtin_bit_cast(uint32_t, off);
}

template <int ESZ>
__device__ __forceinline__ uint32_t gelu_tab_off2_abs(uint32_t w, bool& bad) {
    const u16x2_t a = __builtin_bit_cast(u16x2_t, w & 0x7fff7fffu);
    const u16x2_t lo = {(unsigned short)GT_LO, (unsigned short)GT_LO};
    const u16x2_t mx = {(unsigned short)(GT_HALF - 1), (unsigned short)(GT_HALF - 1)};
    const u16x2_t idx = a - lo;
    const u16x2_t idc = __builtin_elementwise_min(idx, mx);
    bad = bad || (__builtin_bit_cast(uint32_t, idx) != __builtin_bit_cast(uint32_t, idc));
    const u16x2_t off = idc * (unsigned short)ESZ;
    return __builtin_bit_cast(uint32_t, off);
}

__device__ __forceinline__ uint4 pack8(const float* v) {
    uint4 r;
    r.x = f2bf2(v[0], v[1]); r.y = f2bf2(v[2], v[3]); r.z = f2bf2(v[4], v[5]); r.w = f2bf2(v[6], v[7]);
    return r;
}
__device__ __forceinline__ void unpack8(uint4 c, float* v) {
    const uint32_t w[4] = {c.x, c.y, c.z, c.w};
#pragma unroll
    for (int i = 0; i < 4; ++i) {
        v[2 * i] = __uint_as_float(w[i] << 16);
        v[2 * i + 1] = __uint_as_float(w[i] & 0xffff0000u);
    }
}

struct LoadDesc {
    const void* ptr;
    const int32_t* rowidx;
    const float* aux0;
    const float* aux1;
    const float* aux2;
    const float* aux3;
    long ld;
    int M, K;
    int p0, p1, p2, p3;
    uint32_t mg0, mg1, mg2;
};

template <int KIND> struct ALoad;

enum { A_F32 = 0, A_BF16 = 1, A_BF16_GELU = 2, A_HEADS = 3, A_PATCH = 4, A_MERGE_LN = 5, A_BF16_CS = 6 };

struct RawF32 { f32x4 a, b; };
__device__ __forceinline__ uint4 cvt_f32x8(const RawF32& r) {
    uint4 o;
    o.x = f2bf2(r.a[0], r.a[1]); o.y = f2bf2(r.a[2], r.a[3]); o.z = f2bf2(r.b[0], r.b[1]); o.w = f2bf2(r.b[2], r.b[3]);
    return o;
}

template <> struct ALoad<A_F32> {
    static constexpr bool ROW_FASTEST = false;
    static constexpr bool LINEAR = true;
    typedef RawF32 Raw;
    LoadDesc d;
    __device__ __forceinline__ Raw raw_lin(uint32_t off) const {
        const float* p = (const float*)d.ptr + off;
        Raw o = {*(const f32x4*)p, *(const f32x4*)(p + 4)};
        return o;
    }
    __device__ __forceinline__ int row_of(int m) const { return m >= d.M ? -1 : (d.rowidx ? d.rowidx[m] : m); }
    __device__ __forceinline__ Raw raw_at(int r, int k0) const {
        Raw z = {(f32x4){0.f, 0.f, 0.f, 0.f}, (f32x4){0.f, 0.f, 0.f, 0.f}};
        if (r < 0 || k0 >= d.K) return z;
        const float* p = (const float*)d.ptr + (long)r * d.ld + k0;
        Raw o = {*(const f32x4*)p, *(const f32x4*)(p + 4)};
        return o;
    }
    __device__ __forceinline__ Raw raw(int m, int k0) const { return raw_at(row_of(m), k0); }
    __device__ __forceinline__ Raw raw_unc(int r, int k0) const {
        const float* p = (const float*)d.ptr + (long)r * d.ld + k0;
        Raw o = {*(const f32x4*)p, *(const f32x4*)(p + 4)};
        return o;
    }
    __device__ __forceinline__ uint4 cvt(const Raw& r) const { return cvt_f32x8(r); }
    __device__ __forceinline__ uint4 chunk(int m, int k0) const { return cvt(raw(m, k0)); }
};
template <> struct ALoad<A_BF16> {
    static constexpr bool ROW_FASTEST = false;
    static constexpr bool LINEAR = true;
    typedef uint4 Raw;
    LoadDesc d;
    __device__ __forceinline__ Raw raw_lin(uint32_t off) const { return *(const uint4*)((const uint16_t*)d.ptr + off); }
    __device__ __forceinline__ uint4 cvt(const Raw& r) const { return r; }
    __device__ __forceinline__ int row_of(int m) const { return m >= d.M ? -1 : (d.rowidx ? d.rowidx[m] : m); }
    __device__ __forceinline__ Raw raw_at(int r, int k0) const {
        if (r < 0 || k0 >= d.K) return make_uint4(0, 0, 0, 0);
        return *(const uint4*)((const uint16_t*)d.ptr + (long)r * d.ld + k0);
    }
    __device__ __forceinline__ Raw raw_unc(int r, int k0) const { return *(const uint4*)((const uint16_t*)d.ptr + (long)r * d.ld + k0); }
    __device__ __forceinline__ Raw raw(int m, int k0) const { return raw_at(row_of(m), k0); }
    __device__ __forceinline__ uint4 chunk(int m, int k0) const { return raw(m, k0); }
};
struct RawCS { uint4 v; float s; };
// ... 203 lines not shown
```

swin_v2_weather_amd/csrc/gemm_tn.hip:

```cpp
#include "gemm_common.h"

namespace {

constexpr int TM = 128;
constexpr int TP = 136;
constexpr int TCH = TM * 16 / NTHREADS;

struct TnOut {
    float* dW; float* db; const int32_t* nmap; const int32_t* kmap; int ldw, M, N, K, ntk, tiles; float* ws;
};
constexpr int TN_SMEM = 2 * TM * TP;

#ifdef SWV2_TN_STAMPS
#define TSTAMP_DECL unsigned long long st_prev = 0, st_acc[8] = {0, 0, 0, 0, 0, 0, 0, 0};
#define TSTAMP_START() do { asm volatile("s_memtime %0\n\ts_waitcnt lgkmcnt(0)" : "=s"(st_prev) : : "memory"); } while (0)
#define TSTAMP(k) do { unsigned long long t_; asm volatile("s_memtime %0\n\ts_waitcnt lgkmcnt(0)" : "=s"(t_) : : "memory"); \
                       st_acc[k] += t_ - st_prev; st_prev = t_; } while (0)
#define TSTAMP_WAITV() asm volatile("s_waitcnt vmcnt(0)" ::: "memory")
#else
#define TSTAMP_DECL
#define TSTAMP_START() do {} while (0)
#define TSTAMP(k) do {} while (0)
#define TSTAMP_WAITV() do {} while (0)
#endif
// ... 340 lines not shown
    o.dW = dW; o.db = db; o.nmap = nmap; o.kmap = kmap; o.ldw = ldw; o.M = M; o.N = N; o.K = K;
    o.ntk = cdiv(K, BN); o.tiles = cdiv(N, BN) * o.ntk; o.ws = ws;
    return o;
}

enum class WgradKernel { WIDE = SWV2_WGRAD_WIDE, TILE = SWV2_WGRAD_TILE };

WgradKernel wgrad_kernel_for(const swv2_operand* y, const swv2_operand* x, size_t ws_bytes, int wide) {
    const int yk = y->kind, xk = x->kind;
    const bool kinds = (yk == A_BF16 || yk == A_HEADS) && (xk == A_BF16 || xk == A_HEADS || xk == A_F32) && !(yk == A_HEADS && xk == A_HEADS) &&
                       !y->rowidx && (xk == A_F32 || !x->rowidx);
    const TnWidePlan wp = tn_wide_plan(y->rows, y->cols, x->cols);
    return wide && wp.ok && kinds && ws_bytes >= wp.total ? WgradKernel::WIDE : WgradKernel::TILE;
}

int launch_tn_wide(const swv2_operand* y, const swv2_operand* x, float* dW, float* db, const int32_t* nmap, const int32_t* kmap, int ldw,
                   int M, int N, int K, float* ws, hipStream_t st) {
    const TnWidePlan wp = tn_wide_plan(M, N, K);
    float* part = ws;
    float* dbpart = db ? (float*)((char*)ws + wp.part_bytes) : nullptr;
    swv2_operand xb = *x;
    if (x->kind == SWV2_OP_F32) {
        uint16_t* cb = (uint16_t*)((char*)ws + wp.part_bytes + wp.db_bytes);
        const long chunks = (long)M * (K / 8);
        hipLaunchKernelGGL(cast_rows_kernel, dim3((unsigned)((chunks + 255) / 256)), dim3(256), 0, st, (const float*)x->ptr, x->rowidx, cb,
                           M, K, x->ld);
        xb.kind = SWV2_OP_BF16; xb.ptr = cb; xb.rowidx = nullptr; xb.ld = K;
    }
    int rc = swv2_tn_wide_launch(y, &xb, part, dbpart, M, N, K, wp.S, st);
    if (rc) return rc;
    const long quads = (long)N * K / 4;
    hipLaunchKernelGGL(tn_wide_reduce_kernel, dim3((unsigned)((quads + 255) / 256)), dim3(256), 0, st, (const float*)part,
                       (const float*)dbpart, dW, db, nmap, kmap, ldw, N, K, wp.S);
    SWV2_CHECK_LAUNCH("swv2_linear_wgrad");
    return SWV2_OK;
}

template <int YK, int XK>
int launch_tn_tile(const swv2_operand* y, const swv2_operand* x, float* dW, float* db, const int32_t* nmap,
                   const int32_t* kmap, int ldw, int M, int N, int K, int splits, float* ws, size_t ws_bytes, hipStream_t st) {
    const TnPlan p = tn_plan(M, N, K, splits);
    if (ws && ws_bytes < p.ws_bytes) {
        swv2_set_error("swv2_linear_wgrad_ws: workspace of %zu bytes, %zu needed (swv2_linear_wgrad_ws_bytes)", ws_bytes, p.ws_bytes);
        return SWV2_ERR_INVALID;
    }
    const TnOut o = tn_out(dW, db, nmap, kmap, ldw, M, N, K, ws);
    if (y->rowidx || (x->rowidx && XK != A_F32)) {
        swv2_set_error("swv2_linear_wgrad: a row gather is supported for a fp32 X operand only (dY kind %d, X kind %d)", y->kind, x->kind);
        return SWV2_ERR_UNSUPPORTED;
    }
    if constexpr (XK == A_F32) {
        if (x->rowidx)
            hipLaunchKernelGGL((gemm_tn_kernel<YK, XK, true>), dim3(p.tiles * p.slices), dim3(NTHREADS), 0, st, make_loader<YK>(y),
                               make_loader<XK>(x), o, p.real_slices);
        else
            hipLaunchKernelGGL((gemm_tn_kernel<YK, XK, false>), dim3(p.tiles * p.slices), dim3(NTHREADS), 0, st, make_loader<YK>(y),
                               make_loader<XK>(x), o, p.real_slices);
    } else {
        hipLaunchKernelGGL((gemm_tn_kernel<YK, XK, false>), dim3(p.tiles * p.slices), dim3(NTHREADS), 0, st, make_loader<YK>(y),
                           make_loader<XK>(x), o, p.real_slices);
    }
    if (ws) {
        TnReduce r = {};
        r.o[0] = o; r.first[0] = 0; r.first[1] = r.first[2] = r.first[3] = r.first[4] = p.tiles; r.slices = p.real_slices;
        hipLaunchKernelGGL(tn_reduce_kernel, dim3(BN * BN / 64, p.tiles), dim3(256), 0, st, r);
    }
    SWV2_CHECK_LAUNCH("swv2_linear_wgrad");
    return SWV2_OK;
}

template <int YK, int XK>
int launch_tn2(const swv2_operand* y, const swv2_operand* x, float* dW, float* db, const int32_t* nmap,
               const int32_t* kmap, int ldw, int M, int N, int K, int splits, float* ws, size_t ws_bytes, hipStream_t st) {
    switch (wgrad_kernel_for(y, x, ws ? ws_bytes : 0, swv2_gemm_wide())) {
        case WgradKernel::WIDE: return launch_tn_wide(y, x, dW, db, nmap, kmap, ldw, M, N, K, ws, st);
        case WgradKernel::TILE: break;
    }
    return launch_tn_tile<YK, XK>(y, x, dW, db, nmap, kmap, ldw, M, N, K, splits, ws, ws_bytes, st);
}

template <int YK>
int launch_tn1(const swv2_operand* y, const swv2_operand* x, float* dW, float* db, const int32_t* nmap,
               const int32_t* kmap, int ldw, int M, int N, int K, int splits, float* ws, size_t wsb, hipStream_t st) {
    if (x->kind == SWV2_OP_F32) return launch_tn2<YK, A_F32>(y, x, dW, db, nmap, kmap, ldw, M, N, K, splits, ws, wsb, st);
    if constexpr (YK == A_BF16) {
        switch (x->kind) {
            case SWV2_OP_BF16: return launch_tn2<YK, A_BF16>(y, x, dW, db, nmap, kmap, ldw, M, N, K, splits, ws, wsb, st);
            case SWV2_OP_BF16_GELU: return launch_tn2<YK, A_BF16_GELU>(y, x, dW, db, nmap, kmap, ldw, M, N, K, splits, ws, wsb, st);
            case SWV2_OP_HEADS: return launch_tn2<YK, A_HEADS>(y, x, dW, db, nmap, kmap, ldw, M, N, K, splits, ws, wsb, st);
            case SWV2_OP_PATCH: return launch_tn2<YK, A_PATCH>(y, x, dW, db, nmap, kmap, ldw, M, N, K, splits, ws, wsb, st);
        }
    }
    if constexpr (YK == A_F32) {
        if (x->kind == SWV2_OP_MERGE_LN) return launch_tn2<YK, A_MERGE_LN>(y, x, dW, db, nmap, kmap, ldw, M, N, K, splits, ws, wsb, st);
    }
    swv2_set_error("swv2_linear_wgrad: operand pair (dY kind %d, X kind %d) is not instantiated", y->kind, x->kind);
    return SWV2_ERR_UNSUPPORTED;
}

}

extern "C" size_t swv2_linear_wgrad_ws_bytes(int M, int N, int K, int splits) {
    if (!(M > 0 && N > 0 && K > 0 && splits > 0)) return 0;
    const TnWidePlan w = tn_wide_plan(M, N, K);
    return std::max(tn_plan(M, N, K, splits).ws_bytes, w.ok ? w.total : (size_t)0);
}

extern "C" int swv2_linear_wgrad_ws(const swv2_operand* dy, const swv2_operand* x, float* dW, float* db, const int32_t* nmap,
                                    const int32_t* kmap, int ldw, int splits, void* ws, size_t ws_bytes, void* stream) {
    int rc = check_operand(dy, "swv2_linear_wgrad(dy)");
    if (rc) return rc;
    rc = check_operand(x, "swv2_linear_wgrad(x)");
    if (rc) return rc;
    SWV2_CHECK_ARG(dW && splits > 0 && ldw > 0, "swv2_linear_wgrad: null dW, non-positive splits or bad pitch");
    SWV2_CHECK_ARG(dy->rows == x->rows, "swv2_linear_wgrad: row counts differ (%d vs %d)", dy->rows, x->rows);
    SWV2_CHECK_ARG(!(db && dy->kind == SWV2_OP_PATCH), "swv2_linear_wgrad: no bias gradient with a patch-layout dY (row-fastest staging)");
    const int M = dy->rows, N = dy->cols, K = x->cols;
    hipStream_t st = (hipStream_t)stream;
    float* w = (float*)ws;
    switch (dy->kind) {
        case SWV2_OP_F32: return launch_tn1<A_F32>(dy, x, dW, db, nmap, kmap, ldw, M, N, K, splits, w, ws_bytes, st);
        case SWV2_OP_BF16: return launch_tn1<A_BF16>(dy, x, dW, db, nmap, kmap, ldw, M, N, K, splits, w, ws_bytes, st);
        case SWV2_OP_HEADS: return launch_tn1<A_HEADS>(dy, x, dW, db, nmap, kmap, ldw, M, N, K, splits, w, ws_bytes, st);
        case SWV2_OP_PATCH: return launch_tn1<A_PATCH>(dy, x, dW, db, nmap, kmap, ldw, M, N, K, splits, w, ws_bytes, st);
        case SWV2_OP_BF16_CSCALE: return launch_tn1<A_BF16_CS>(dy, x, dW, db, nmap, kmap, ldw, M, N, K, splits, w, ws_bytes, st);
    }
    swv2_set_error("swv2_linear_wgrad: unsupported dY operand kind %d", dy->kind);
    return SWV2_ERR_INVALID;
}

extern "C" int swv2_linear_wgrad(const swv2_operand* dy, const swv2_operand* x, float* dW, float* db, const int32_t* nmap,
                                 const int32_t* kmap, int ldw, int splits, void* stream) {
    return swv2_linear_wgrad_ws(dy, x, dW, db, nmap, kmap, ldw, splits, nullptr, 0, stream);
}

extern "C" int swv2_linear_wgrad_kernel(const swv2_operand* dy, const swv2_operand* x, int splits, size_t ws_bytes) {
    SWV2_CHECK_ARG(dy && x && splits > 0 && dy->rows > 0 && dy->rows == x->rows, "swv2_linear_wgrad_kernel: null operand, non-positive splits or row mismatch");
    return (int)wgrad_kernel_for(dy, x, ws_bytes, swv2_gemm_wide());
}

namespace {
int group_slices(int total_tiles, int requested) {
    if (requested > 0) return std::max(8, requested / 8 * 8);
    return std::max(8, (2 * 256 / total_tiles) / 8 * 8);
}
}

extern "C" size_t swv2_block_wgrad_ws_bytes(int C, int hidden, int heads_dp, int slices) {
    if (C <= 0 || hidden <= 0 || heads_dp <= 0) return 0;
    const int tt = 2 * cdiv(C, BN) * cdiv(hidden, BN) + cdiv(C, BN) * cdiv(heads_dp, BN) + cdiv(3 * heads_dp, BN) * cdiv(C, BN);
    return std::max((size_t)group_slices(tt, slices) * tt * BN * BN * sizeof(float), swv2_tn_slab_ws_bytes(C, hidden, heads_dp));
}

extern "C" int swv2_block_wgrad(const swv2_wgrad_item* it, int slices, void* ws, size_t ws_bytes, void* stream) {
    return swv2_block_wgrad_ln(it, slices, ws, ws_bytes, nullptr, stream);
}

namespace {
enum class BlockWgradKernel { SLAB = SWV2_BLOCK_WGRAD_SLAB, GROUPED = SWV2_BLOCK_WGRAD_GROUPED };

BlockWgradKernel block_wgrad_kernel_for(const swv2_wgrad_item* it, int slices, size_t ws_bytes) {
    return slices <= 0 && swv2_tn_slab_covers(it, ws_bytes) ? BlockWgradKernel::SLAB : BlockWgradKernel::GROUPED;
}

int launch_tn_group(const swv2_wgrad_item* it, int slices, void* ws, size_t ws_bytes, const swv2_ln_partials* ln, hipStream_t st) {
    TnGroup g = {};
    int tt = 0;
    for (int i = 0; i < 4; ++i) {
        g.first[i] = tt;
        tt += cdiv(it[i].dy.cols, BN) * cdiv(it[i].x.cols, BN);
    }
    g.first[4] = tt;
    const int S = group_slices(tt, slices);
    SWV2_CHECK_ARG(ws_bytes >= (size_t)S * tt * BN * BN * sizeof(float), "swv2_block_wgrad: workspace of %zu bytes, %zu needed",
                   ws_bytes, (size_t)S * tt * BN * BN * sizeof(float));
    if (ln && ln->C > 0)
        swv2_launch_ln_partials_reduce2(ln->ws[0], ln->dgamma[0], ln->dbeta[0], ln->n[0], ln->ws[1], ln->dgamma[1], ln->dbeta[1], ln->n[1], ln->C, st);
    TnReduce r = {};
    for (int i = 0; i < 4; ++i) {
        g.o[i] = tn_out(it[i].dW, it[i].db, it[i].nmap, it[i].kmap, it[i].ldw, it[i].dy.rows, it[i].dy.cols, it[i].x.cols,
                        (float*)ws + (size_t)g.first[i] * S * BN * BN);
        r.o[i] = g.o[i];
    }
    for (int i = 0; i < 5; ++i) r.first[i] = g.first[i];
    g.y0 = make_loader<A_BF16>(&it[0].dy); g.x0 = make_loader<A_BF16_GELU>(&it[0].x);
    g.y1 = make_loader<A_BF16>(&it[1].dy); g.x1 = make_loader<A_F32>(&it[1].x);
    g.y2 = make_loader<A_BF16>(&it[2].dy); g.x2 = make_loader<A_HEADS>(&it[2].x);
    g.y3 = make_loader<A_HEADS>(&it[3].dy); g.x3 = make_loader<A_F32>(&it[3].x);
    g.slices = r.slices = S;
    hipLaunchKernelGGL(gemm_tn_group_kernel, dim3(tt * S), dim3(NTHREADS), 0, st, g);
    hipLaunchKernelGGL(tn_reduce_kernel, dim3(BN * BN / 64, tt), dim3(256), 0, st, r);
    SWV2_CHECK_LAUNCH("swv2_block_wgrad");
    return SWV2_OK;
}
}

extern "C" int swv2_block_wgrad_kernel(const swv2_wgrad_item* it, int slices, size_t ws_bytes) {
    SWV2_CHECK_ARG(it, "swv2_block_wgrad_kernel: null items");
    return (int)block_wgrad_kernel_for(it, slices, ws_bytes);
}

int swv2_block_wgrad_ln(const swv2_wgrad_item* it, int slices, void* ws, size_t ws_bytes, const swv2_ln_partials* ln, void* stream) {
    SWV2_CHECK_ARG(it && ws, "swv2_block_wgrad: null items or workspace");
    static const int want[4][2] = {{SWV2_OP_BF16, SWV2_OP_BF16_GELU}, {SWV2_OP_BF16, SWV2_OP_F32}, {SWV2_OP_BF16, SWV2_OP_HEADS},
                                   {SWV2_OP_HEADS, SWV2_OP_F32}};
    for (int i = 0; i < 4; ++i) {
        int rc = check_operand(&it[i].dy, "swv2_block_wgrad(dy)");
        if (rc) return rc;
        rc = check_operand(&it[i].x, "swv2_block_wgrad(x)");
        if (rc) return rc;
        SWV2_CHECK_ARG(it[i].dy.kind == want[i][0] && it[i].x.kind == want[i][1],
                       "swv2_block_wgrad: item %d must be (dY kind %d, X kind %d)", i, want[i][0], want[i][1]);
        SWV2_CHECK_ARG(it[i].dW && it[i].ldw > 0 && it[i].dy.rows == it[i].x.rows, "swv2_block_wgrad: item %d: null dW or row mismatch", i);
        SWV2_CHECK_ARG(!it[i].dy.rowidx && (i == 3 ? it[i].x.rowidx != nullptr : it[i].x.rowidx == nullptr),
                       "swv2_block_wgrad: item %d: only the qkv product's X rows are gathered (and they must be)", i);
    }
    switch (block_wgrad_kernel_for(it, slices, ws_bytes)) {
        case BlockWgradKernel::SLAB: return swv2_tn_slab_launch(it, ws, ws_bytes, ln, (hipStream_t)stream);
        case BlockWgradKernel::GROUPED: break;
    }
    return launch_tn_group(it, slices, ws, ws_bytes, ln, (hipStream_t)stream);
}
```

swin_v2_weather_amd/csrc/gemm_tn_slab.hip:

```cpp
#include "gemm_common.h"
#pragma clang diagnostic ignored "-Wc++20-extensions"

namespace {

#ifdef SWV2_SLAB_PART_F32
typedef float sl_part_t;
#else
typedef uint16_t sl_part_t;
#endif
constexpr int SL_TH = 512;
constexpr int SL_SMEM = 160 * 1024;
constexpr int SL_IDX_CAP = 4096;
enum { F_ROW = 0, F_ROWG = 1, F_F32 = 2, F_F32G = 3, F_HEAD = 4 };

__device__ __forceinline__ void sl_dma(const void* base, uint32_t byte_off, uint32_t lds_addr) {
    asm volatile("s_mov_b32 m0, %2\n\ts_nop 0\n\tglobal_load_lds_dwordx4 %0, %1" : : "v"(byte_off), "s"(base), "s"(lds_addr) : "memory");
}

#ifdef SWV2_SLAB_STAMPS
#define SSTAMP_DECL unsigned long long st_prev = 0, st_acc[8] = {0, 0, 0, 0, 0, 0, 0, 0};
#define SSTAMP_START() do { asm volatile("s_memtime %0\n\ts_waitcnt lgkmcnt(0)" : "=s"(st_prev) : : "memory"); } while (0)
#define SSTAMP(k) do { unsigned long long t_; asm volatile("s_waitcnt lgkmcnt(0)\n\ts_memtime %0\n\ts_waitcnt lgkmcnt(0)" : "=s"(t_) : : "memory"); \
                       st_acc[k] += t_ - st_prev; st_prev = t_; } while (0)
#else
// ... 357 lines not shown
    if (want_db && fr == 0) {
#pragma unroll
        for (int i = 0; i < IA; ++i)
            if (i % WGK == wgk) {
#pragma unroll
                for (int r = 0; r < 4; ++r) P.dbpart[(size_t)slice * P.N + n0 + n_w + 16 * i + 4 * g + r] = accdb[i / WGK][r];
            }
    }
}

__global__ __launch_bounds__(SL_TH) void gemm_tn_slab_c128_kernel(SlArgs a) {
    __shared__ __attribute__((aligned(1024))) unsigned char smem[SL_SMEM];
    const int b = blockIdx.x;
    if (b < a.p[1].first) slab_job<F_ROW, F_ROWG, 128, 512, 1, 8, 32, 3>(a.p[0], b - a.p[0].first, smem, a.stamps);
    else if (b < a.p[2].first) slab_job<F_ROW, F_F32, 512, 128, 8, 1, 32, 3>(a.p[1], b - a.p[1].first, smem, a.stamps);
    else if (b < a.p[3].first) slab_job<F_ROW, F_HEAD, 128, 128, 2, 4, 64, 4>(a.p[2], b - a.p[2].first, smem, a.stamps);
    else slab_job<F_HEAD, F_F32G, 384, 128, 8, 1, 32, 3>(a.p[3], b - a.p[3].first, smem, a.stamps);
}
__global__ __launch_bounds__(SL_TH) void gemm_tn_slab_c192_kernel(SlArgs a) {
    __shared__ __attribute__((aligned(1024))) unsigned char smem[SL_SMEM];
    const int b = blockIdx.x;
    if (b < a.p[1].first) slab_job<F_ROW, F_ROWG, 192, 384, 1, 8, 32, 3>(a.p[0], b - a.p[0].first, smem, a.stamps);
    else if (b < a.p[2].first) slab_job<F_ROW, F_F32, 384, 192, 8, 1, 32, 3>(a.p[1], b - a.p[1].first, smem, a.stamps);
    else if (b < a.p[3].first) slab_job<F_ROW, F_HEAD, 192, 256, 2, 4, 32, 4>(a.p[2], b - a.p[2].first, smem, a.stamps);
    else slab_job<F_HEAD, F_F32G, 384, 192, 8, 1, 32, 3, true>(a.p[3], b - a.p[3].first, smem, a.stamps);
}

struct SlLnRed { const float* ws[2]; float* dg[2]; float* db[2]; int n[2]; int C; };
struct SlRed { float* dW; float* db; const int32_t* nmap; const int32_t* kmap; const sl_part_t* part; const float* dbpart;
               int ldw, N, K, TN, TK, WGK, IA, JB, ntk, S, first, dbfirst; };
struct SlRedArgs { SlRed p[4]; int total, dbtotal; SlLnRed ln; int cpw; };
__global__ __launch_bounds__(512) void tn_slab_reduce_kernel(SlRedArgs a) {
    __shared__ f32x4 red[8][64];
    const int b = blockIdx.x;
    const int lane = threadIdx.x & 63, sg = threadIdx.x >> 6;
    if (b >= a.total + a.dbtotal) {
        const int bb = b - a.total - a.dbtotal, per_set = (2 * a.ln.C + 15) / 16;
        const int set = bb / per_set, col = threadIdx.x & 15, sl = threadIdx.x >> 4;
        const int jc = (bb - set * per_set) * 16 + col;
        float sum = 0.f;
        if (jc < 2 * a.ln.C) {
            const float* w = a.ln.ws[set];
#pragma unroll 4
            for (int r = sl; r < a.ln.n[set]; r += 32) sum += w[(size_t)r * 2 * a.ln.C + jc];
        }
        float* redf = (float*)red;
        redf[sl * 16 + col] = sum;
        __syncthreads();
        for (int hh = 16; hh > 0; hh >>= 1) {
            if (sl < hh) redf[sl * 16 + col] += redf[(sl + hh) * 16 + col];
            __syncthreads();
        }
        if (sl == 0 && jc < 2 * a.ln.C) {
            if (jc < a.ln.C) a.ln.dg[set][jc] += redf[col]; else a.ln.db[set][jc - a.ln.C] += redf[col];
        }
        return;
    }
    if (b >= a.total) {
        const int bb = b - a.total;
        const int pi = (bb >= a.p[1].dbfirst) + (bb >= a.p[2].dbfirst) + (bb >= a.p[3].dbfirst);
        const SlRed& p = a.p[pi];
        const int n = (bb - p.dbfirst) * 64 + lane;
        float a0 = 0.f, a1 = 0.f;
        if (p.db && p.dbpart && n < p.N) {
            int q = sg;
            for (; q + 8 < p.S; q += 16) { a0 += p.dbpart[(size_t)q * p.N + n]; a1 += p.dbpart[(size_t)(q + 8) * p.N + n]; }
            if (q < p.S) a0 += p.dbpart[(size_t)q * p.N + n];
        }
        float* redf = (float*)red;
        redf[sg * 64 + lane] = a0 + a1;
        __syncthreads();
        if (sg == 0 && p.db && p.dbpart && n < p.N) {
            const int nn = p.nmap ? p.nmap[n] : n;
            float t = 0.f;
#pragma unroll
            for (int e = 0; e < 8; ++e) t += redf[e * 64 + lane];
            if (nn >= 0) p.db[nn] += t;
        }
        return;
    }
    const int pi = (b >= a.p[1].first) + (b >= a.p[2].first) + (b >= a.p[3].first);
    const SlRed& p = a.p[pi];
    const int NG = 8 / a.cpw;
    const int cg = (b - p.first) * a.cpw + sg / NG, sl0 = sg % NG;
    int kk = -1, nn[4] = {-1, -1, -1, -1};
    float old[4] = {0.f, 0.f, 0.f, 0.f};
    if (sl0 == 0) {
        const int cpt = 8 * p.IA * p.JB, tile = cg / cpt, c = cg - tile * cpt;
        const int wave = c / (p.IA * p.JB), ij = c - wave * (p.IA * p.JB), i = ij / p.JB, jj = ij - i * p.JB;
        const int wgn = wave / p.WGK, wgk = wave - wgn * p.WGK, g = lane >> 4, fr = lane & 15;
        const int n0 = (tile / p.ntk) * p.TN + wgn * p.IA * 16 + 16 * i + 4 * g;
        const int k = (tile % p.ntk) * p.TK + wgk * p.JB * 16 + 16 * jj + fr;
        kk = p.kmap ? p.kmap[k] : k;
#pragma unroll
        for (int r = 0; r < 4; ++r) nn[r] = p.nmap ? p.nmap[n0 + r] : n0 + r;
#pragma unroll
        for (int r = 0; r < 4; ++r) old[r] = p.dW[(long)max(nn[r], 0) * p.ldw + max(kk, 0)];
    }
    const sl_part_t* src = p.part + (size_t)cg * p.S * 256 + lane * 4;
#ifdef SWV2_SLAB_PART_F32
    auto ld = [](const sl_part_t* q) -> f32x4 { return *(const f32x4*)q; };
#else
    auto ld = [](const sl_part_t* q) -> f32x4 {
        const bf16x4 v = *(const bf16x4*)q;
        return (f32x4){bf2f(v[0]), bf2f(v[1]), bf2f(v[2]), bf2f(v[3])};
    };
#endif
    f32x4 s0 = {0.f, 0.f, 0.f, 0.f}, s1 = s0, s2 = s0, s3 = s0;
    int s = sl0;
    for (; s + 3 * NG < p.S; s += 4 * NG) {
        s0 += ld(src + (size_t)s * 256);
        s1 += ld(src + (size_t)(s + NG) * 256);
        s2 += ld(src + (size_t)(s + 2 * NG) * 256);
        s3 += ld(src + (size_t)(s + 3 * NG) * 256);
    }
    for (; s < p.S; s += NG) s0 += ld(src + (size_t)s * 256);
    red[sg][lane] = (s0 + s1) + (s2 + s3);
    __syncthreads();
    if (sl0 == 0 && kk >= 0) {
        f32x4 t;
        if (a.cpw == 1) t = ((red[0][lane] + red[1][lane]) + (red[2][lane] + red[3][lane])) + ((red[4][lane] + red[5][lane]) + (red[6][lane] + red[7][lane]));
        else t = (red[sg][lane] + red[sg + 1][lane]) + (red[sg + 2][lane] + red[sg + 3][lane]);
#pragma unroll
        for (int r = 0; r < 4; ++r)
            if (nn[r] >= 0) p.dW[(long)nn[r] * p.ldw + kk] = old[r] + t[r];
    }
}

struct SlShape { int TN[4], TK[4], SR[4], WGN[4], WGK[4]; };
const SlShape SL_SETS[2] = {{{128, 512, 128, 384}, {512, 128, 128, 128}, {32, 32, 64, 32}, {1, 8, 2, 8}, {8, 1, 4, 1}},
                            {{192, 384, 192, 384}, {384, 192, 256, 192}, {32, 32, 32, 32}, {1, 8, 2, 8}, {8, 1, 4, 1}}};
const int SL_BLOCKS[2][4] = {{128, 512, 8, 16}, {192, 768, 8, 32}};
int sl_set(int C, int hidden, int heads_dp) {
    for (int i = 0; i < 2; ++i)
        if (C == SL_BLOCKS[i][0] && hidden == SL_BLOCKS[i][1] && heads_dp == SL_BLOCKS[i][2] * SL_BLOCKS[i][3]) return i;
    return -1;
}

constexpr int SL_CU_BOUND = 320;
int sl_cus() {
    static thread_local int cus[16] = {};
    int dev = 0;
    if (hipGetDevice(&dev) != hipSuccess || dev < 0 || dev >= 16) return 256;
    if (!cus[dev]) {
        int v = 0;
        if (hipDeviceGetAttribute(&v, hipDeviceAttributeMultiprocessorCount, dev) != hipSuccess || v <= 0) v = 256;
        cus[dev] = v < SL_CU_BOUND ? v : SL_CU_BOUND;
    }
    return cus[dev];
}

struct SlPlan { bool ok; int set; int wgs[4], ntile[4], S[4]; size_t part_off[4], db_off[4], total; };

SlPlan sl_plan(const swv2_wgrad_item* it, int cus) {
    SlPlan p = {};
    const int N[4] = {it[0].dy.cols, it[1].dy.cols, it[2].dy.cols, it[3].dy.cols};
    const int K[4] = {it[0].x.cols, it[1].x.cols, it[2].x.cols, it[3].x.cols};
    const int C = N[0], hid = K[0];
    p.set = sl_set(C, hid, K[2]);
    if (p.set < 0) return p;
    const SlShape& sh = SL_SETS[p.set];
    if (!(N[1] == hid && K[1] == C && N[2] == C && N[3] == 3 * K[2] && K[3] == C)) return p;
    if (!(it[2].x.p[3] == SL_BLOCKS[p.set][3] && it[3].dy.p[3] == SL_BLOCKS[p.set][3] && it[2].x.p[0] == SL_BLOCKS[p.set][2] &&
          it[3].dy.p[0] == SL_BLOCKS[p.set][2])) return p;
    if (!(it[0].dy.ld == C && it[0].x.ld == hid && it[1].dy.ld == hid && it[1].x.ld == C && it[2].dy.ld == C && it[3].x.ld == C)) return p;
    if (cus < 16 || cus > 1024) return p;
    double cost[4], tot = 0;
    const double wgt[4] = {1.55, 1.0, 1.0, 1.1};
    for (int i = 0; i < 4; ++i) {
        const double xb = it[i].x.kind == SWV2_OP_F32 ? 4.0 : 2.0;
        p.ntile[i] = (N[i] / sh.TN[i]) * (K[i] / sh.TK[i]);
        cost[i] = wgt[i] * (double)it[i].dy.rows * (2.0 * N[i] * (K[i] / sh.TK[i]) + xb * K[i] * (N[i] / sh.TN[i]));
        tot += cost[i];
    }
    int used = 0;
    for (int i = 0; i < 4; ++i) {
        const int T = cdiv(it[i].dy.rows, sh.SR[i]);
        int sl = (int)(cus * cost[i] / tot / p.ntile[i] + 0.5);
        sl = std::max(1, std::min(sl, T));
        p.S[i] = sl;
        p.wgs[i] = sl * p.ntile[i];
        used += p.wgs[i];
    }
    for (int guard = 0; used != cus && guard < 64; ++guard) {
        int best = -1;
        double br = 0;
        for (int i = 0; i < 4; ++i) {
            const int T = cdiv(it[i].dy.rows, sh.SR[i]);
            if (used < cus ? (p.S[i] >= T || used + p.ntile[i] > cus) : p.S[i] <= 1) continue;
            const double r = cost[i] / p.S[i];
            if (best < 0 || (used < cus ? r > br : r < br)) { best = i; br = r; }
        }
        if (best < 0) break;
        const int d = used < cus ? 1 : -1;
        p.S[best] += d; p.wgs[best] += d * p.ntile[best]; used += d * p.ntile[best];
    }
    size_t off = 0;
    for (int i = 0; i < 4; ++i) {
        const int T = cdiv(it[i].dy.rows, sh.SR[i]);
        if ((double)it[i].dy.rows * std::max(N[i], K[i]) * 4.0 >= 4.29e9) return p;
        p.part_off[i] = off;
        off += (size_t)p.wgs[i] * sh.TN[i] * sh.TK[i] * sizeof(float);
        p.db_off[i] = off;
        off += (size_t)p.S[i] * N[i] * sizeof(float);
        off = (off + 255) / 256 * 256;
    }
    p.total = off;
    p.ok = true;
    return p;
}

SlOp sl_op(const swv2_operand& o) {
    SlOp s = {};
    s.ptr = o.ptr; s.rowidx = o.rowidx; s.ld = (int)o.ld;
    if (o.kind == SWV2_OP_HEADS) {
        s.heads = o.p[0]; s.parts = (int)o.ld; s.Lp = o.p[2]; s.DP = o.p[3];
        s.mgLp = fdiv_magic(s.Lp); s.mgDP = fdiv_magic(s.DP); s.mgH = fdiv_magic(s.heads);
    }
    return s;
}

}

size_t swv2_tn_slab_ws_bytes(int C, int hidden, int heads_dp) {
    const int set = sl_set(C, hidden, heads_dp);
    if (set < 0) return 0;
    const int cus = SL_CU_BOUND;
    const SlShape& sh = SL_SETS[set];
    size_t tile = 0;
    for (int i = 0; i < 4; ++i) tile = std::max(tile, (size_t)sh.TN[i] * sh.TK[i] * 4);
    return (size_t)cus * tile + (size_t)cus * std::max(hidden, 3 * heads_dp) * 4 + 4 * 256;
}

bool swv2_tn_slab_covers(const swv2_wgrad_item* it, size_t ws_bytes) {
    const SlPlan pl = sl_plan(it, sl_cus());
    if (pl.ok && ws_bytes < pl.total) {
        static int once = 0;
        if (!once++) fprintf(stderr, "swv2: grouped weight gradient declined (workspace %zu bytes, %zu needed): size it with swv2_block_wgrad_ws_bytes; "
                                     "running the 128 x 128 tile kernels\n", ws_bytes, pl.total);
    }
    return pl.ok && ws_bytes >= pl.total;
}

int swv2_tn_slab_launch(const swv2_wgrad_item* it, void* ws, size_t ws_bytes, const swv2_ln_partials* ln, hipStream_t st) {
    const SlPlan pl = sl_plan(it, sl_cus());
    SWV2_CHECK_ARG(pl.ok && ws_bytes >= pl.total, "swv2_block_wgrad(slab): items or workspace not covered (swv2_tn_slab_covers)");
    const SlShape& sh = SL_SETS[pl.set];
    SlArgs a = {};
    SlRedArgs r = {};
    int first = 0, rfirst = 0, dbfirst = 0;
    int cpw = 2;
    for (int i = 0; i < 4; ++i)
        if (pl.S[i] > 40 || ((it[i].dy.cols * it[i].x.cols / 256) & 1)) cpw = 1;
    r.cpw = cpw;
    for (int i = 0; i < 4; ++i) {
        SlProd& p = a.p[i];
        p.y = sl_op(it[i].dy); p.x = sl_op(it[i].x);
        p.part = (sl_part_t*)((char*)ws + pl.part_off[i]);
        p.dbpart = it[i].db ? (float*)((char*)ws + pl.db_off[i]) : nullptr;
        p.M = it[i].dy.rows; p.N = it[i].dy.cols; p.K = it[i].x.cols;
        p.first = first; p.wgs = pl.wgs[i]; p.ntile = pl.ntile[i];
        first += pl.wgs[i];
        SlRed& q = r.p[i];
        q.dW = it[i].dW; q.db = it[i].db; q.nmap = it[i].nmap; q.kmap = it[i].kmap; q.part = p.part; q.dbpart = p.dbpart;
        q.ldw = it[i].ldw; q.N = p.N; q.K = p.K; q.TN = sh.TN[i]; q.TK = sh.TK[i]; q.WGK = sh.WGK[i];
        q.IA = sh.TN[i] / (16 * sh.WGN[i]); q.JB = sh.TK[i] / (16 * sh.WGK[i]); q.ntk = p.K / sh.TK[i]; q.S = pl.S[i]; q.first = rfirst;
        rfirst += p.N * p.K / 256 / cpw;
        q.dbfirst = dbfirst;
        dbfirst += cdiv(p.N, 64);
    }
    r.total = rfirst;
    r.dbtotal = dbfirst;
    int lnblocks = 0;
    if (ln && ln->C > 0) {
        for (int i = 0; i < 2; ++i) { r.ln.ws[i] = ln->ws[i]; r.ln.dg[i] = ln->dgamma[i]; r.ln.db[i] = ln->dbeta[i]; r.ln.n[i] = ln->n[i]; }
        r.ln.C = ln->C;
        lnblocks = 2 * cdiv(2 * ln->C, 16);
    }
#ifdef SWV2_SLAB_STAMPS
    if (ws_bytes >= pl.total + (size_t)first * 64) a.stamps = (unsigned long long*)((char*)ws + ws_bytes - (size_t)first * 64);
    { static int once = 0; if (!once++) fprintf(stderr, "slab plan: workgroups %d %d %d %d\n", pl.wgs[0], pl.wgs[1], pl.wgs[2], pl.wgs[3]); }
#endif
    if (pl.set == 0) hipLaunchKernelGGL(gemm_tn_slab_c128_kernel, dim3(first), dim3(SL_TH), 0, st, a);
    else hipLaunchKernelGGL(gemm_tn_slab_c192_kernel, dim3(first), dim3(SL_TH), 0, st, a);
    hipLaunchKernelGGL(tn_slab_reduce_kernel, dim3(rfirst + dbfirst + lnblocks), dim3(512), 0, st, r);
    SWV2_CHECK_LAUNCH("swv2_block_wgrad(slab)");
    return 0;
}
```

swin_v2_weather_amd/networks/swinv2_global.py:

```python
from __future__ import annotations

import math
import os
from types import SimpleNamespace
from typing import Any, List, Optional, Tuple, Type, Union

import torch
import torch.nn as nn
import torch.nn.functional as F
from torch.utils.checkpoint import checkpoint

from .. import _lib as L
from .. import ops

BF16 = torch.bfloat16


def to_2tuple(x):
    return tuple(x) if isinstance(x, (tuple, list)) else (x, x)


def bchw_to_bhwc(x: torch.Tensor) -> torch.Tensor:
    return x.permute(0, 2, 3, 1)


def bhwc_to_bchw(x: torch.Tensor) -> torch.Tensor:
    return x.permute(0, 3, 1, 2)


def _need_gpu(x: torch.Tensor, who: str):
    if not x.is_cuda:
        raise L.Swv2Error(f"{who}: the swv2 hot path runs on an MI355X only (got a {x.device} tensor); there is no "
                          "CPU fallback")


def _zeros_like_shapes(device, *shapes):
    sizes = [((int(torch.Size(s).numel()) + 3) // 4) * 4 for s in shapes]
    flat = torch.zeros(sum(sizes), dtype=torch.float32, device=device)
    out, off = [], 0
    for s, n in zip(shapes, sizes):
        out.append(flat[off:off + int(torch.Size(s).numel())].view(*s))
        off += n
    return out


_OPT_EPOCH = [0]


def _bump_opt_epoch(*_a, **_k):
    _OPT_EPOCH[0] += 1


from torch.optim.optimizer import register_optimizer_step_post_hook as _reg_opt_hook

_reg_opt_hook(_bump_opt_epoch)


class _WeightCache:

    def __init__(self):
        self._c = {}

    @staticmethod
    def _ver(params):
        return tuple((p.data_ptr(), p._version, _OPT_EPOCH[0]) for p in params)

    def get(self, key, params, builder):
        ver = self._ver(params)
        hit = self._c.get(key)
        if hit is not None and hit[0] == ver:
            return hit[1]
        with torch.no_grad():
            val = builder()
        self._c[key] = (ver, val)
        return val

    def prep(self, key, w, batch, **spec):
        ver = self._ver((w,))
        hit = self._c.get(key)
        if hit is not None and hit[0] == ver:
            return hit[1]
        val = batch.add(w, out=None if hit is None else hit[1], **spec)
        self._c[key] = (None, val)
        batch.on_launched(lambda c=self._c, k=key, v=(ver, val): c.__setitem__(k, v))
        return val


def window_partition(x, window_size: Tuple[int, int]):
    B, H, W, C = x.shape
    x = x.view(B, H // window_size[0], window_size[0], W // window_size[1], window_size[1], C)
    return x.permute(0, 1, 3, 2, 4, 5).contiguous().view(-1, window_size[0], window_size[1], C)


def window_reverse(windows, window_size: Tuple[int, int], img_size: Tuple[int, int]):
    H, W = img_size
    C = windows.shape[-1]
    x = windows.view(-1, H // window_size[0], W // window_size[1], window_size[0], window_size[1], C)
    return x.permute(0, 1, 3, 2, 4, 5).contiguous().view(-1, H, W, C)


def _carve(sizes, align=256):
    offs, off = [], 0
    for s in sizes:
        offs.append(off)
        off += (s + align - 1) // align * align
    return offs, off


class _BlockRunner:

    ACTS = ("qkvh", "rnorm", "oh", "lse", "a1", "mean1", "rstd1", "x1", "hpre", "hact", "a2", "mean2", "rstd2", "bias_pack")
    SCRATCH = ("da2", "dh", "da1", "doh", "dqkvh", "dx1", "ln_ws", "wgrad_ws")

    def __init__(self, blk, plan, Cc, hid, device):
        self.plan, self.C, self.hid, self.device = plan, Cc, hid, device
        h, Lp, DP, Bw, B, T, Lw = plan.heads, plan.Lp, plan.DP, plan.Bw, plan.B, plan.T, plan.L
        BT, Mw = B * T, Bw * Lp
        d = L.BlockDesc()
        d.B, d.T, d.C, d.heads, d.head_dim, d.hidden = B, T, Cc, h, plan.d, hid
        d.L, d.Lp, d.DP, d.nwh, d.nww, d.mask_thr = Lw, Lp, DP, plan.nwh, plan.nww, plan.mask_thr
        d.rowidx, d.qkv_map, d.proj_map = plan.rowidx.data_ptr(), plan.qkv_map.data_ptr(), plan.proj_map.data_ptr()
        d.wgrad_splits = int(os.environ.get("SWV2_WGRAD_SPLITS", "128"))
        d.wgrad_group = int(os.environ.get("SWV2_WGRAD_GROUP", "1"))
        d.fuse_mlp = int(os.environ.get("SWV2_FUSE_MLP", "1"))
        d.fuse_proj_ln = int(os.environ.get("SWV2_FUSE_PROJ_LN", "1"))
        d.wgrad_ws = d.grad_zero = 1
        d.ln_ws_floats = d.wgrad_ws_bytes = 1 << 62
        full = L.block_plan(d)
        d.ln_ws_floats, d.wgrad_ws_bytes = full.need_ln_ws_floats, full.need_wgrad_ws_bytes
        self.launch_plan = lp = L.block_plan(d)
        if any(getattr(lp, n) != getattr(full, n) for n in ("mlp_fused", "proj_ln_fused", "ln_deferred", "wgrad_grouped", "wgrad_kernel")):
            raise L.Swv2Error("swv2_block_plan: the reported workspace needs do not cover the full plan")
        d.wgrad_ws = d.grad_zero = None
        self.desc = d
        act_sizes = [Bw * h * 3 * Lp * DP * 2, Bw * h * 2 * Lp * 4, Bw * h * Lp * DP * 2, Bw * h * Lp * 4, Mw * Cc * 2, Mw * 4,
                     Mw * 4, BT * Cc * 4, BT * hid * 2, lp.need_hact_bytes, BT * Cc * 2, BT * 4, BT * 4,
                     L.load().swv2_attn_pack_bias_bytes(h, Lw)]
        self.act_off, self.act_bytes = _carve(act_sizes)
        scr_sizes = [BT * Cc * 2, BT * hid * 2, Mw * Cc * 2, Bw * h * Lp * DP * 2, Bw * h * 3 * Lp * DP * 2, BT * Cc * 4,
                     d.ln_ws_floats * 4, d.wgrad_ws_bytes]
        self.scr_off, self.scr_bytes = _carve(scr_sizes)
        self.grad_shapes = [(h,), (3 * Cc, Cc), (3 * Cc,), (Cc, Cc), (Cc,), (Cc,), (Cc,), (hid, Cc), (hid,), (Cc, hid), (Cc,),
                            (Cc,), (Cc,)]
        self.grad_names = ["d_logit_scale", "d_qkv_w", "d_qkv_b", "d_proj_w", "d_proj_b", "d_n1_w", "d_n1_b", "d_fc1_w",
                           "d_fc1_b", "d_fc2_w", "d_fc2_b", "d_n2_w", "d_n2_b"]
        gs = [int(torch.Size(s).numel()) * 4 for s in self.grad_shapes]
        self.grad_off, self.grad_bytes = _carve(gs, 64)
        self.bias_elems = h * Lw * Lw

    def set_params(self, wc, logit_scale, qkv_w, qkv_b, proj_w, proj_b, n1_w, n1_b, fc1_w, fc1_b, fc2_w, fc2_b, n2_w, n2_b,
                   backward, batch=None):
        plan, d = self.plan, self.desc
        h, DP = plan.heads, plan.DP
        own = batch is None
        if own:
            batch = ops.PrepBatch()
        keep = [wc.prep("qkv", qkv_w, batch, row_map=plan.qkv_map, out_rows=3 * h * DP),
                wc.prep("qkv_b", qkv_b, batch, row_map=plan.qkv_map, out_rows=3 * h * DP, f32=True),
                wc.prep("proj", proj_w, batch, col_map=plan.proj_map, out_cols=h * DP),
                wc.prep("fc1", fc1_w, batch),
                wc.prep("fc2", fc2_w, batch)]
        d.w_qkv, d.qkv_b_pad, d.w_proj, d.w_fc1, d.w_fc2 = (t.data_ptr() for t in keep)
        if backward:
            kb = [wc.prep("qkvt", qkv_w, batch, transpose=True, col_map=plan.qkv_map, out_cols=3 * h * DP),
                  wc.prep("projt", proj_w, batch, transpose=True, row_map=plan.proj_map, out_rows=h * DP),
                  wc.prep("fc1t", fc1_w, batch, transpose=True),
                  wc.prep("fc2t", fc2_w, batch, transpose=True)]
            d.w_qkvt, d.w_projt, d.w_fc1t, d.w_fc2t = (t.data_ptr() for t in kb)
            keep += kb
        if own:
            batch.launch()
        d.logit_scale, d.proj_b, d.n1_w, d.n1_b = logit_scale.data_ptr(), proj_b.data_ptr(), n1_w.data_ptr(), n1_b.data_ptr()
        d.fc1_b, d.fc2_b, d.n2_w, d.n2_b = fc1_b.data_ptr(), fc2_b.data_ptr(), n2_w.data_ptr(), n2_b.data_ptr()
        return keep

    def set_acts(self, acts):
        base, d = acts.data_ptr(), self.desc
        for name, off in zip(self.ACTS, self.act_off):
            setattr(d, name, base + off)


class _BlockFn(torch.autograd.Function):
    @staticmethod
    def forward(ctx, x, bias, dp1, dp2, logit_scale, qkv_w, qkv_b, proj_w, proj_b, n1_w, n1_b, fc1_w, fc1_b, fc2_w,
                fc2_b, n2_w, n2_b, blk, ckpt=0, cpb=None):
        B, gh, gw, Cc = x.shape
        run = blk._runner(B, x.device)
        d = run.desc
        x = x.contiguous()
        keep = run.set_params(blk._wcache, logit_scale, qkv_w, qkv_b, proj_w, proj_b, n1_w, n1_b, fc1_w, fc1_b, fc2_w, fc2_b,
                              n2_w, n2_b, backward=False)
        bias_c = None if (bias is None or cpb is not None) else bias.detach().float().contiguous()
        acts = torch.empty(run.act_bytes, dtype=torch.uint8, device=x.device)
        x2 = torch.empty(B, gh, gw, Cc, dtype=torch.float32, device=x.device)
        run.set_acts(acts)
        d.x, d.x2 = x.data_ptr(), x2.data_ptr()
        d.bias = None if bias_c is None else bias_c.data_ptr()
        d.bias_prepacked, d.dbias_part, d.dbias_part_bytes = 0, None, 0
        if cpb is not None:
            cpb[0].point(d, cpb[1])
        d.dp1 = None if dp1 is None else dp1.data_ptr()
        d.dp2 = None if dp2 is None else dp2.data_ptr()
        ops.block_event_pair("fwd", d)
        L.check(ops._timed("block_fwd", L.load().swv2_block_fwd, run.desc, ops._stream()), "swv2_block_fwd")
        del keep
        ctx.blk, ctx.run, ctx.has_bias, ctx.ckpt, ctx.cpb = blk, run, bias is not None, int(ckpt), cpb
        e = x.new_empty(0)
        if ckpt:
            acts = e
            xs = x.to(BF16) if ckpt == 2 else x
        else:
            xs = x
        ctx.save_for_backward(xs, bias_c if bias_c is not None else e, dp1 if dp1 is not None else e, dp2 if dp2 is not None else e,
                              acts, logit_scale, qkv_w, qkv_b, proj_w, proj_b, n1_w, n1_b, fc1_w, fc1_b, fc2_w, fc2_b, n2_w, n2_b)
        return x2

    @staticmethod
    def backward(ctx, dx2):
        (x, bias_c, dp1, dp2, acts, logit_scale, qkv_w, qkv_b, proj_w, proj_b, n1_w, n1_b, fc1_w, fc1_b, fc2_w, fc2_b, n2_w,
         n2_b) = ctx.saved_tensors
        blk, run, cpb = ctx.blk, ctx.run, ctx.cpb
        d = run.desc
        dev = x.device
        keep = run.set_params(blk._wcache, logit_scale, qkv_w, qkv_b, proj_w, proj_b, n1_w, n1_b, fc1_w, fc1_b, fc2_w, fc2_b,
                              n2_w, n2_b, backward=True)
        dx2 = dx2.contiguous().float()
        own_bias = ctx.has_bias and cpb is None
        d.bias_prepacked, d.dbias_part, d.dbias_part_bytes = 0, None, 0
        if ctx.ckpt:
            x = x.float() if x.dtype != torch.float32 else x
            acts = torch.empty(run.act_bytes, dtype=torch.uint8, device=dev)
            x2_tmp = torch.empty_like(x)
            run.set_acts(acts)
            d.x, d.x2 = x.data_ptr(), x2_tmp.data_ptr()
            d.bias = bias_c.data_ptr() if own_bias else None
            if cpb is not None:
                cpb[0].point(d, cpb[1])
            d.dp1 = dp1.data_ptr() if dp1.numel() else None
            d.dp2 = dp2.data_ptr() if dp2.numel() else None
            d.ev_kernel = 0
            L.check(L.load().swv2_block_fwd(run.desc, ops._stream()), "swv2_block_fwd (recompute)")
            del x2_tmp
        run.set_acts(acts)
        scratch = torch.empty(run.scr_bytes, dtype=torch.uint8, device=dev)
        sb = scratch.data_ptr()
        for name, off in zip(run.SCRATCH, run.scr_off):
            setattr(d, name, sb + off)
        params = (logit_scale, qkv_w, qkv_b, proj_w, proj_b, n1_w, n1_b, fc1_w, fc1_b, fc2_w, fc2_b, n2_w, n2_b)
        wants_param_grads = any(ctx.needs_input_grad[4:17])
        reuse = blk._pass_grads_of(torch._C._current_graph_task_id()) \
            if (wants_param_grads and os.environ.get("SWV2_GRAD_ACC_INPLACE", "1") != "0") else None
        views = blk._bucket_views(params) if (reuse is None and blk._ddp_bucket_grads and not blk._bv_in_use) else None
        dbias_view = None
        if reuse is not None:
            for name, ptr in zip(run.grad_names, reuse):
                setattr(d, name, ptr)
            d.grad_zero, d.grad_zero_bytes = None, 0
            if ctx.has_bias and cpb is None:
                dbias_view = torch.zeros_like(bias_c)
        elif views is not None:
            blk._bv_in_use = True
            torch._foreach_zero_(views)
            for name, v in zip(run.grad_names, views):
                setattr(d, name, v.data_ptr())
            d.grad_zero, d.grad_zero_bytes = None, 0
        else:
            in_kernel = bool(run.launch_plan.grad_zero_in_kernel)
            nfl = (run.grad_bytes // 4 + 3) // 4 * 4
            nb = (bias_c.numel() + 3) // 4 * 4 if own_bias else 0
            grads = (torch.empty if in_kernel else torch.zeros)(nfl + nb, dtype=torch.float32, device=dev)
            gb = grads.data_ptr()
            d.grad_zero, d.grad_zero_bytes = (gb, (nfl + nb) * 4) if in_kernel else (None, 0)
            if nb:
                dbias_view = grads[nfl:nfl + bias_c.numel()].view_as(bias_c)
            for name, off in zip(run.grad_names, run.grad_off):
                setattr(d, name, gb + off)
        if blk._ddp_bucket_grads and reuse is None:
            blk._queue_view_refresh(params)
        dbias = (dbias_view if dbias_view is not None else torch.zeros_like(bias_c)) if own_bias else None
        dx = torch.empty_like(x)
        d.x, d.dx2, d.dx = x.data_ptr(), dx2.data_ptr(), dx.data_ptr()
        d.bias = bias_c.data_ptr() if own_bias else None
        d.d_bias = dbias.data_ptr() if own_bias else None
        if cpb is not None:
# ... 836 lines not shown
```

Measured before the change: 225.9.

## Fuse qkv weight-gradient partials into the resident dx GEMM kernel

Adds a WG variant of the resident dx GEMM. While it computes dx from dqkv heads, it also stages the gathered input rows x in LDS and accumulates per-slice qkv weight- and bias-gradient partials with MFMA, since the dqkv tile is already resident. The slab wgrad kernel then skips the qkv item and folds those partials in its reduce, so dqkv and x are not streamed a second time. In exchange it adds LDS use, register pressure and extra MFMA work to the dx kernel, plus a larger workspace. It is on by default through SWV2_DX_WGRAD.

After: 228.1 (median of 5 runs). About the same (+1.0%).

```diff
diff --git a/include/swv2.h b/include/swv2.h
--- a/include/swv2.h
+++ b/include/swv2.h
@@ -7,7 +7,7 @@
 extern "C" {
 #endif
 
-#define SWV2_VERSION 109
+#define SWV2_VERSION 110
 
 enum {
     SWV2_OK = 0,
@@ -145,6 +145,14 @@
 #define SWV2_BLOCK_WGRAD_SLAB 0
 #define SWV2_BLOCK_WGRAD_GROUPED 1
 int swv2_block_wgrad_kernel(const swv2_wgrad_item* items4, int slices, size_t ws_bytes);
+
+#define SWV2_LINEAR_RESIDENT_DX128_WGRAD 7
+size_t swv2_dx_wgrad_ws_bytes(int C, int heads_dp);
+size_t swv2_block_wgrad_dx_ws_bytes(int C, int hidden, int heads_dp);
+int swv2_linear_dx_wgrad_kernel(const swv2_operand* a, const swv2_epilogue* e, int N, size_t ws_bytes);
+int swv2_linear_dx_wgrad(const swv2_operand* a, const void* w_bf16, const swv2_epilogue* e, int N, const float* x, long xld, void* ws,
+                         size_t ws_bytes, void* stream);
+int swv2_dx_wgrad_fold(const void* ws, size_t ws_bytes, int rows, float* dW, float* db, const int32_t* nmap, int ldw, void* stream);
 
 int swv2_qk_normalize(void* qkvh_bf16, float* rnorm, int Bw, int heads, int Lp, int L, int DP, void* stream);
 
@@ -351,6 +359,7 @@
     int bias_prepacked;
     float* dbias_part;
     size_t dbias_part_bytes;
+    int dx_wgrad;
 } swv2_block_desc;
 
 enum swv2_block_step {
@@ -391,6 +400,7 @@
     size_t need_wgrad_ws_bytes;
     int n_fwd, n_bwd;
     int fwd[SWV2_BLOCK_MAX_STEPS], bwd[SWV2_BLOCK_MAX_STEPS];
+    int dx_wgrad;
 } swv2_block_plan_t;
 int swv2_block_plan(const swv2_block_desc* d, swv2_block_plan_t* out);
 int swv2_block_step_id(int step);
diff --git a/swin_v2_weather_amd/_lib.py b/swin_v2_weather_amd/_lib.py
--- a/swin_v2_weather_amd/_lib.py
+++ b/swin_v2_weather_amd/_lib.py
@@ -10,7 +10,7 @@
 LIB_PATH = os.environ.get("SWV2_LIB") or os.path.join(HERE, "libswv2.so")
 SOURCES = ["capi.hip", "attn.hip", "attn2.hip", "attn_bwd_stream.hip", "attn_wide.hip", "attn_d256.hip", "gemm.hip", "gemm_tn.hip", "gemm_tn_slab.hip", "rowops.hip", "block.hip", "cpb.hip", "mlp.hip", "proj_ln.hip", "dataio.hip"]
 
-ABI_VERSION = 109
+ABI_VERSION = 110
 
 _lib = None
 _lock = threading.Lock()
@@ -143,7 +143,7 @@
                 [("wgrad_splits", C.c_int), ("ev_kernel", C.c_int), ("ev_start", C.c_void_p), ("ev_stop", C.c_void_p),
                  ("fuse_proj_ln", C.c_int), ("fuse_mlp", C.c_int), ("wgrad_ws", C.c_void_p), ("wgrad_ws_bytes", C.c_size_t), ("wgrad_group", C.c_int), ("grad_zero", C.c_void_p),
                  ("grad_zero_bytes", C.c_size_t), ("ln_ws_floats", C.c_size_t),
-                 ("bias_prepacked", C.c_int), ("dbias_part", C.c_void_p), ("dbias_part_bytes", C.c_size_t)])
+                 ("bias_prepacked", C.c_int), ("dbias_part", C.c_void_p), ("dbias_part_bytes", C.c_size_t), ("dx_wgrad", C.c_int)])
 
 
 BLOCK_MAX_STEPS = 12
@@ -154,7 +154,7 @@
     _fields_ = ([(n, C.c_int) for n in ("mlp_fused", "proj_ln_fused", "ln_deferred", "wgrad_grouped", "wgrad_kernel", "grad_zero_in_kernel",
                                         "attn_fwd_chunks", "attn_bwd_chunks", "dbias_dest")] +
                 [(n, C.c_size_t) for n in ("need_hact_bytes", "need_ln_ws_floats", "need_wgrad_ws_bytes")] +
-                [("n_fwd", C.c_int), ("n_bwd", C.c_int), ("fwd", C.c_int * BLOCK_MAX_STEPS), ("bwd", C.c_int * BLOCK_MAX_STEPS)])
+                [("n_fwd", C.c_int), ("n_bwd", C.c_int), ("fwd", C.c_int * BLOCK_MAX_STEPS), ("bwd", C.c_int * BLOCK_MAX_STEPS), ("dx_wgrad", C.c_int)])
 
     def steps(self, phase):
         lib = load()
@@ -170,6 +170,7 @@
 OP_F32, OP_BF16, OP_BF16_GELU, OP_HEADS, OP_PATCH, OP_MERGE_LN, OP_BF16_CSCALE = range(7)
 EPI_BF16, EPI_F32, EPI_QKV_HEADS, EPI_GELU_GRAD, EPI_UNPATCH, EPI_HEADS, EPI_F32_ACC, EPI_BF16_GELU, EPI_UNPATCH_LOSS = range(9)
 LINEAR_RESIDENT_QKV128, LINEAR_RESIDENT_QKV192X3, LINEAR_RESIDENT_DX128, LINEAR_WIDE_DMA, LINEAR_WIDE, LINEAR_TILE64, LINEAR_TILE128 = range(7)
+LINEAR_RESIDENT_DX128_WGRAD = 7
 LINEAR_WIDE_KERNELS, LINEAR_TILE_KERNELS = (LINEAR_WIDE_DMA, LINEAR_WIDE), (LINEAR_TILE64, LINEAR_TILE128)
 WGRAD_WIDE, WGRAD_TILE = range(2)
 BLOCK_WGRAD_SLAB, BLOCK_WGRAD_GROUPED = range(2)
@@ -196,6 +197,11 @@
     "swv2_qk_normalize": (_I, [_P, _P, _I, _I, _I, _I, _I, _P]),
     "swv2_block_wgrad_ws_bytes": (C.c_size_t, [_I, _I, _I, _I]),
     "swv2_block_wgrad": (_I, [C.POINTER(WgradItem), _I, _P, C.c_size_t, _P]),
+    "swv2_dx_wgrad_ws_bytes": (C.c_size_t, [_I, _I]),
+    "swv2_block_wgrad_dx_ws_bytes": (C.c_size_t, [_I, _I, _I]),
+    "swv2_linear_dx_wgrad_kernel": (_I, [C.POINTER(Operand), C.POINTER(Epilogue), _I, C.c_size_t]),
+    "swv2_linear_dx_wgrad": (_I, [C.POINTER(Operand), _P, C.POINTER(Epilogue), _I, _P, _L, _P, C.c_size_t, _P]),
+    "swv2_dx_wgrad_fold": (_I, [_P, C.c_size_t, _I, _P, _P, _P, _I, _P]),
     "swv2_linear_wgrad_ws": (_I, [C.POINTER(Operand), C.POINTER(Operand), _P, _P, _P, _P, _I, _I, _P, C.c_size_t, _P]),
     "swv2_prep_weight": (_I, [_P, _I, _I, _I, _P, _I, _P, _I, _P, _P]),
     "swv2_ln_residual_fwd": (_I, [C.POINTER(LnArgs), _P]),
diff --git a/swin_v2_weather_amd/csrc/block.hip b/swin_v2_weather_amd/csrc/block.hip
--- a/swin_v2_weather_amd/csrc/block.hip
+++ b/swin_v2_weather_amd/csrc/block.hip
@@ -78,6 +78,15 @@
     p->ln_deferred = p->mlp_fused && p->proj_ln_fused && d->ln_ws_floats >= ln_pair;
     p->wgrad_grouped = d->wgrad_group && p->mlp_fused && d->wgrad_ws && ws_bytes >= swv2_block_wgrad_ws_bytes(C, hid, h * d->DP, 0);
     p->wgrad_kernel = -1;
+    {
+        swv2_operand a = op_heads(p, Bw, h, 3, d->Lp, d->DP);
+        swv2_epilogue e = epi(SWV2_EPI_F32, p, C, nullptr, p, nullptr, (const int32_t*)p);
+        const size_t dx_ws = swv2_block_wgrad_dx_ws_bytes(C, hid, h * d->DP);
+        const bool dx_able = d->dx_wgrad && d->wgrad_group && p->mlp_fused && dx_ws && swv2_linear_kernel(&a, &e, C) == SWV2_LINEAR_RESIDENT_DX128 &&
+                             (double)Mw * 768 < 4.29e9;
+        if (dx_able) p->need_wgrad_ws_bytes = std::max(p->need_wgrad_ws_bytes, dx_ws);
+        p->dx_wgrad = dx_able && p->wgrad_grouped && ws_bytes >= dx_ws;
+    }
     p->grad_zero_in_kernel = p->mlp_fused && d->grad_zero != nullptr;
     p->attn_fwd_chunks = d->bias ? 32 : 64;
     p->attn_bwd_chunks = 64;
@@ -130,6 +139,7 @@
         swv2_wgrad_item it[4] = {};
         wgrad_items(d, true, it);
         p->wgrad_kernel = swv2_block_wgrad_kernel(it, 0, d->wgrad_ws_bytes);
+        if (p->wgrad_kernel != SWV2_BLOCK_WGRAD_SLAB) p->dx_wgrad = 0;
     }
     return SWV2_OK;
 }
@@ -214,6 +224,8 @@
     const int sp = d->wgrad_splits > 0 ? d->wgrad_splits : 64;
     swv2_wgrad_item it[4] = {};
     wgrad_items(d, p.mlp_fused, it);
+    if (p.dx_wgrad && swv2_block_wgrad_kernel(it, 0, d->wgrad_ws_bytes) != SWV2_BLOCK_WGRAD_SLAB) p.dx_wgrad = 0;
+    void* const qkv_part = p.dx_wgrad ? (char*)d->wgrad_ws + swv2_block_dx_part_offset(C, hid, h * d->DP) : nullptr;
     float* const ln1_ws = p.ln_deferred ? d->ln_ws + swv2_mlp_bwd_ws_floats(BT, C) : d->ln_ws;
     int n_ln1 = 0, n_ln2 = 0;
     for (int i = 0; i < p.n_bwd; ++i) switch (const int s = p.bwd[i]; s) {
@@ -270,15 +282,16 @@
     } break;
     case SWV2_STEP_DX: {
         swv2_epilogue e = epi(SWV2_EPI_F32, d->dx, C, nullptr, d->dx1, nullptr, d->rowidx);
-        LAUNCH(SWV2_STEP_DX, swv2_linear(&it[3].dy, d->w_qkvt, &e, C, st));
+        if (qkv_part) LAUNCH(SWV2_STEP_DX, swv2_block_dx_wgrad(&it[3].dy, d->w_qkvt, &e, C, d->x, C, qkv_part, st));
+        else LAUNCH(SWV2_STEP_DX, swv2_linear(&it[3].dy, d->w_qkvt, &e, C, st));
     } break;
     case SWV2_STEP_LN_FOLD:
         swv2_launch_ln_partials_reduce2(d->ln_ws, d->d_n2_w, d->d_n2_b, n_ln2, ln1_ws, d->d_n1_w, d->d_n1_b, n_ln1, C, (hipStream_t)st);
         break;
     case SWV2_STEP_WGRAD_GROUP: {
         swv2_ln_partials lnp = {{d->ln_ws, ln1_ws}, {d->d_n2_w, d->d_n1_w}, {d->d_n2_b, d->d_n1_b}, {n_ln2, n_ln1}, C};
-        LAUNCH(SWV2_STEP_WGRAD_GROUP, swv2_block_wgrad_ln(it, 0, d->wgrad_ws, d->wgrad_ws_bytes, p.ln_deferred ? &lnp : nullptr, st));
-    } break;
-    }
-    return SWV2_OK;
-}
+        LAUNCH(SWV2_STEP_WGRAD_GROUP, swv2_block_wgrad_ln(it, 0, d->wgrad_ws, d->wgrad_ws_bytes, p.ln_deferred ? &lnp : nullptr, qkv_part, st));
+    } break;
+    }
+    return SWV2_OK;
+}
diff --git a/swin_v2_weather_amd/csrc/common.h b/swin_v2_weather_amd/csrc/common.h
--- a/swin_v2_weather_amd/csrc/common.h
+++ b/swin_v2_weather_amd/csrc/common.h
@@ -119,6 +119,9 @@
 int swv2_proj_ln_bwd_impl(const swv2_proj_ln_bwd_args* a, void* stream, int* deferred);
 
 struct swv2_ln_partials { const float* ws[2]; float* dgamma[2]; float* dbeta[2]; int n[2]; int C; };
-int swv2_block_wgrad_ln(const swv2_wgrad_item* items4, int slices, void* ws, size_t ws_bytes, const swv2_ln_partials* ln, void* stream);
+int swv2_block_wgrad_ln(const swv2_wgrad_item* items4, int slices, void* ws, size_t ws_bytes, const swv2_ln_partials* ln, const void* qkv_part,
+                        void* stream);
+int swv2_block_dx_wgrad(const swv2_operand* a, const void* w, const swv2_epilogue* e, int N, const float* x, long xld, void* part, void* stream);
+size_t swv2_block_dx_part_offset(int C, int hidden, int heads_dp);
 
 static inline int cdiv(long a, long b) { return (int)((a + b - 1) / b); }
diff --git a/swin_v2_weather_amd/csrc/gemm.hip b/swin_v2_weather_amd/csrc/gemm.hip
--- a/swin_v2_weather_amd/csrc/gemm.hip
+++ b/swin_v2_weather_amd/csrc/gemm.hip
@@ -975,8 +975,10 @@
 #endif
 __device__ __forceinline__ int swzk(int r, int kc, int K) { return r * K + ((kc ^ ((r >> 1) & 7)) << 3); }
 
-template <int AK, int EK, int N, int K, int BMT, int HS = 16>
-__global__ __launch_bounds__(512) void gemm_rw_kernel(ALoad<AK> al, const uint16_t* __restrict__ Wb, Epi<EK> ep, int M) {
+struct RwWgrad { const float* x; uint16_t* part; float* dbpart; long xld; };
+
+template <int AK, int EK, int N, int K, int BMT, int HS = 16, bool WG = false>
+__global__ __launch_bounds__(512) void gemm_rw_kernel(ALoad<AK> al, const uint16_t* __restrict__ Wb, Epi<EK> ep, int M, [[maybe_unused]] RwWgrad wg) {
     constexpr int NTH = 512, KC = K / 8;
     constexpr int ACH = BMT * KC / NTH;
     constexpr int RT = BMT / 64;
@@ -985,10 +987,14 @@
     constexpr int A_BYTES = BMT * K * 2, ST_BYTES = 8 * 16 * EP * 4;
     constexpr int AS_BYTES = A_BYTES > ST_BYTES ? A_BYTES : ST_BYTES;
     static_assert(BMT * KC % NTH == 0 && N * KC % NTH == 0 && K % 64 == 0 && N % 64 == 0, "tile shapes");
-    static_assert(N * K * 2 + AS_BYTES <= 160 * 1024, "LDS budget");
+    static_assert(!WG || (AK == A_HEADS && EK == E_F32 && N == 128 && K == 384 && BMT == 64), "WG: the dx instantiation only");
+    constexpr int X_BYTES = WG ? BMT * N * 2 : N * 4;
+    static_assert(N * K * 2 + AS_BYTES + X_BYTES <= 160 * 1024, "LDS budget");
     __shared__ __attribute__((aligned(16))) uint16_t Ws[N * K];
     __shared__ __attribute__((aligned(16))) unsigned char as_raw[AS_BYTES];
-    __shared__ __attribute__((aligned(16))) float bs[N];
+    __shared__ __attribute__((aligned(16))) unsigned char x_raw[X_BYTES];
+    [[maybe_unused]] float* const bs = (float*)x_raw;
+    [[maybe_unused]] uint16_t* const xs = (uint16_t*)x_raw;
     uint16_t* As = (uint16_t*)as_raw;
     float* stage_all = (float*)as_raw;
 
@@ -997,7 +1003,9 @@
     const int wr = wave >> 1, wc = wave & 1;
     const int ntiles = (M + BMT - 1) / BMT;
     static_assert(EK != E_F32 || (RT == 1 && CT == 4), "the E_F32 prefetch below covers one 16 x 64 wave tile");
-    for (int i = tid; i < N; i += NTH) bs[i] = ep.d.bias ? ep.d.bias[i] : 0.f;
+    if constexpr (!WG) {
+        for (int i = tid; i < N; i += NTH) bs[i] = ep.d.bias ? ep.d.bias[i] : 0.f;
+    }
     int erow_nxt = -1, erow_cur = -1;
     f32x4 aux_nxt[4], aux_cur[4];
     const int ecol = wc * (N / 2) + (lane & 3) * 16;
@@ -1011,7 +1019,23 @@
     uint32_t ain = 0;
     uint32_t aok = 0;
     bool ein = false;
+    [[maybe_unused]] RawF32 rx[2];
+    [[maybe_unused]] int xrow[2] = {0, 0};
+    [[maybe_unused]] uint32_t xin = 0, xok = 0;
+    [[maybe_unused]] uint32_t a_off = 0;
+    [[maybe_unused]] const uint32_t a_thr = (uint32_t)((tid >> 7) * 3 * al.d.p2 * 16 + (tid & 1) * 8);
     auto resolve = [&](int t) {
+        if constexpr (WG) {
+            const int m = min(t * BMT + ((tid >> 1) & (BMT - 1)), M - 1), bw = fdiv(m, al.d.p2, al.d.mg0);
+            a_off = (uint32_t)bw * (uint32_t)(384 * al.d.p2) + (uint32_t)((m - bw * al.d.p2) * 16) + a_thr;
+            xin = 0;
+#pragma unroll
+            for (int i = 0; i < 2; ++i) {
+                const int m = t * BMT + (tid >> 4) + 32 * i;
+                xin |= (uint32_t)((t < ntiles) && (m < M)) << i;
+                xrow[i] = ep.d.rowidx[min(m, M - 1)];
+            }
+        }
         ain = 0;
 #pragma unroll
         for (int i = 0; i < ACH; ++i) {
@@ -1033,7 +1057,11 @@
         for (int i = 0; i < ACH; ++i) {
             const int c = tid + i * NTH;
             const int r = ((ain >> i) & 1) ? arow[i] : -1;
-            if constexpr (AK == A_HEADS) ra[i] = al.raw_at(r, ccol(c) * 8);
+            if constexpr (WG) {
+                const uint16_t* const ab = (const uint16_t*)al.d.ptr + (size_t)((12 * (i & 1) + (i >> 1)) * 16 * al.d.p2);
+                ra[i] = r >= 0 ? *(const uint4*)(ab + a_off) : make_uint4(0, 0, 0, 0);
+            }
+            else if constexpr (AK == A_HEADS) ra[i] = al.raw_at(r, ccol(c) * 8);
             else ra[i] = al.raw_unc(max(r, 0), ccol(c) * 8);
             aok |= (uint32_t)(r >= 0) << i;
         }
@@ -1043,15 +1071,81 @@
 #pragma unroll
             for (int i = 0; i < 4; ++i) aux_nxt[i] = *(const f32x4*)(ax + 4 * i);
         }
+        if constexpr (WG) {
+            xok = 0;
+#pragma unroll
+            for (int i = 0; i < 2; ++i) {
+                const int r = ((xin >> i) & 1) ? xrow[i] : -1;
+                const float* px = wg.x + (long)max(r, 0) * wg.xld + (tid & 15) * 8;
+                rx[i].a = *(const f32x4*)px;
+                rx[i].b = *(const f32x4*)(px + 4);
+                xok |= (uint32_t)(r >= 0) << i;
+            }
+        }
     };
     auto commit = [&]() {
+        [[maybe_unused]] uint16_t* const as0 = As + swzk(crow(tid), ccol(tid), K);
 #pragma unroll
         for (int i = 0; i < ACH; ++i) {
             const int c = tid + i * NTH;
-            *(uint4*)(As + swzk(crow(c), ccol(c), K)) = ((aok >> i) & 1) ? al.cvt(ra[i]) : make_uint4(0, 0, 0, 0);
+            if constexpr (WG) *(uint4*)(as0 + 64 * i) = ((aok >> i) & 1) ? ra[i] : make_uint4(0, 0, 0, 0);
+            else *(uint4*)(As + swzk(crow(c), ccol(c), K)) = ((aok >> i) & 1) ? al.cvt(ra[i]) : make_uint4(0, 0, 0, 0);
+        }
+        if constexpr (WG) {
+#pragma unroll
+            for (int i = 0; i < 2; ++i) {
+                const int r = tid >> 4, ch = tid & 15;
+                *(uint4*)(xs + r * N + ((((ch >> 1) ^ (r & 7))) << 4) + (ch & 1) * 8 + 32 * N * i) = ((xok >> i) & 1) ? cvt_f32x8(rx[i]) : make_uint4(0, 0, 0, 0);
+            }
         }
     };
     const int G = gridDim.x;
+    constexpr int WI = WG ? 3 : 1, WJ = WG ? N / 16 : 1;
+    [[maybe_unused]] f32x4 wacc[WI][WJ], accdb[WI];
+    if constexpr (WG) {
+#pragma unroll
+        for (int i = 0; i < WI; ++i) {
+            accdb[i] = (f32x4){0.f, 0.f, 0.f, 0.f};
+#pragma unroll
+            for (int j = 0; j < WJ; ++j) wacc[i][j] = (f32x4){0.f, 0.f, 0.f, 0.f};
+        }
+    }
+    [[maybe_unused]] auto wgrad_tile = [&]() {
+        if constexpr (WG) {
+            const bf16x8 ones = {0x3F80, 0x3F80, 0x3F80, 0x3F80, 0x3F80, 0x3F80, 0x3F80, 0x3F80};
+            auto tr_a = [&](int r0, int c) -> bf16x4 {
+                const int row = r0 + 4 * g + (fr >> 2), kc = (c >> 3) + ((fr >> 1) & 1);
+                return lds_tr_read(As + swzk(row, kc, K) + (fr & 1) * 4);
+            };
+            auto tr_x = [&](int r0, int c) -> bf16x4 {
+                const int row = r0 + 4 * g + (fr >> 2);
+                return lds_tr_read(xs + row * N + (((c >> 4) ^ (row & 7)) << 4) + (fr & 3) * 4);
+            };
+#pragma unroll
+            for (int kk = 0; kk < BMT / 32; ++kk) {
+                bf16x8 af[WI];
+#pragma unroll
+                for (int i = 0; i < WI; ++i) {
+                    const bf16x4 a0 = tr_a(32 * kk, wave * 48 + 16 * i), a1 = tr_a(32 * kk + 16, wave * 48 + 16 * i);
+                    af[i] = __builtin_shufflevector(a0, a1, 0, 1, 2, 3, 4, 5, 6, 7);
+                    accdb[i] = mfma32(af[i], ones, accdb[i]);
+                }
+#pragma unroll
+                for (int j0 = 0; j0 < WJ; j0 += 2) {
+                    bf16x8 bf[2];
+#pragma unroll
+                    for (int j = 0; j < 2; ++j) {
+                        const bf16x4 b0 = tr_x(32 * kk, 16 * (j0 + j)), b1 = tr_x(32 * kk + 16, 16 * (j0 + j));
+                        bf[j] = __builtin_shufflevector(b0, b1, 0, 1, 2, 3, 4, 5, 6, 7);
+                    }
+#pragma unroll
+                    for (int j = 0; j < 2; ++j)
+#pragma unroll
+                        for (int i = 0; i < WI; ++i) wacc[i][j0 + j] = mfma32(af[i], bf[j], wacc[i][j0 + j]);
+                }
+            }
+        }
+    };
     RSTAMP_DECL
     auto tile_step = [&](int t) {
         RSTAMP_WAITV();
@@ -1068,19 +1162,26 @@
         issue();
         resolve(t + 2 * G);
         RSTAMP(3);
+        wgrad_tile();
         f32x4 acc[RT][CT];
 #pragma unroll
         for (int i = 0; i < RT; ++i)
 #pragma unroll
             for (int j = 0; j < CT; ++j) acc[i][j] = (f32x4){0.f, 0.f, 0.f, 0.f};
+        [[maybe_unused]] const int sw_lo = (g ^ ((fr >> 1) & 3)) << 3, sw_hi = ((fr >> 3) & 1) << 5;
+        [[maybe_unused]] const int sw_eo[2] = {fr * K + sw_lo + sw_hi, fr * K + sw_lo - sw_hi};
+        auto frag_at = [&](const uint16_t* base, int row16, int ks) -> bf16x8 {
+            if constexpr (WG) return *(const bf16x8*)(base + sw_eo[ks & 1] + row16 * K + (ks << 5));
+            else return *(const bf16x8*)(base + swzk(row16 + fr, ks * 4 + g, K));
+        };
 #pragma unroll
         for (int ks = 0; ks < K / 32; ++ks) {
             bf16x8 af[RT];
 #pragma unroll
-            for (int i = 0; i < RT; ++i) af[i] = *(const bf16x8*)(As + swzk(wr * 16 * RT + i * 16 + fr, ks * 4 + g, K));
+            for (int i = 0; i < RT; ++i) af[i] = frag_at(As, wr * 16 * RT + i * 16, ks);
 #pragma unroll
             for (int j = 0; j < CT; ++j) {
-                const bf16x8 bf = *(const bf16x8*)(Ws + swzk(wc * (N / 2) + j * 16 + fr, ks * 4 + g, K));
+                const bf16x8 bf = frag_at(Ws, wc * (N / 2) + j * 16, ks);
 #pragma unroll
                 for (int i = 0; i < RT; ++i) acc[i][j] = mfma32(af[i], bf, acc[i][j]);
             }
@@ -1139,8 +1240,11 @@
                         float* o = (float*)ep.d.out + (long)erow_cur * ep.d.ld + ecol;
                         const int r = lane >> 2, c0 = (lane & 3) * 16;
 #pragma unroll
-                        for (int q = 0; q < 4; ++q)
-                            *(f32x4*)(o + 4 * q) = *(const f32x4*)(st + r * EP + c0 + 4 * q) + *(const f32x4*)(bs + ecol + 4 * q) + aux_cur[q];
+                        for (int q = 0; q < 4; ++q) {
+                            f32x4 b4 = {0.f, 0.f, 0.f, 0.f};
+                            if constexpr (!WG) b4 = *(const f32x4*)(bs + ecol + 4 * q);
+                            *(f32x4*)(o + 4 * q) = *(const f32x4*)(st + r * EP + c0 + 4 * q) + b4 + aux_cur[q];
+                        }
                     }
                 } else {
                     ep.tile(st, m0, n0, lane);
@@ -1162,6 +1266,22 @@
 
     RSTAMP_START();
     for (; t < ntiles; t += G) tile_step(t);
+    if constexpr (WG) {
+        const int S = min(G, ntiles), slice = blockIdx.x;
+        if (slice < S) {
+            uint16_t* out = wg.part + ((size_t)(wave * WI * WJ) * S + slice) * 256 + lane * 4;
+#pragma unroll
+            for (int i = 0; i < WI; ++i)
+#pragma unroll
+                for (int j = 0; j < WJ; ++j) *(bf16x4*)(out + (size_t)(i * WJ + j) * S * 256) = f2bf4(wacc[i][j]);
+            if (fr == 0) {
+#pragma unroll
+                for (int i = 0; i < WI; ++i)
+#pragma unroll
+                    for (int r = 0; r < 4; ++r) wg.dbpart[(size_t)slice * K + wave * 48 + 16 * i + 4 * g + r] = accdb[i][r];
+            }
+        }
+    }
 #ifdef SWV2_RW_STAMPS
     if (tid == 0)
         for (int k = 0; k < 8; ++k) rw_stamps[blockIdx.x * 8 + k] = st_acc[k];
@@ -1250,7 +1370,7 @@
             if constexpr (qkv_pair(AK, EK)) {
                 Epi<EK> ep1 = ep;
                 ep1.d.p1 = 0;
-                hipLaunchKernelGGL((gemm_rw_kernel<AK, EK, 384, 128, 128>), dim3(256), dim3(512), 0, st, make_loader<AK>(a), wb, ep1, M);
+                hipLaunchKernelGGL((gemm_rw_kernel<AK, EK, 384, 128, 128>), dim3(256), dim3(512), 0, st, make_loader<AK>(a), wb, ep1, M, RwWgrad{});
             }
             break;
         case LinearKernel::RESIDENT_QKV192X3:
@@ -1261,13 +1381,13 @@
                     ep2.d.p1 = part;
                     ep2.d.bias = e->bias ? e->bias + 256 * part : nullptr;
                     hipLaunchKernelGGL((gemm_rw_kernel<AK, EK, 256, 192, 128, 32>), dim3(256), dim3(512), 0, st, make_loader<AK>(a),
-                                       wb + (size_t)part * 256 * 192, ep2, M);
+                                       wb + (size_t)part * 256 * 192, ep2, M, RwWgrad{});
                 }
             }
             break;
         case LinearKernel::RESIDENT_DX128:
             if constexpr (dx_pair(AK, EK))
-                hipLaunchKernelGGL((gemm_rw_kernel<AK, EK, 128, 384, 64>), dim3(256), dim3(512), 0, st, make_loader<AK>(a), wb, ep, M);
+                hipLaunchKernelGGL((gemm_rw_kernel<AK, EK, 128, 384, 64>), dim3(256), dim3(512), 0, st, make_loader<AK>(a), wb, ep, M, RwWgrad{});
             break;
         case LinearKernel::WIDE_DMA:
         case LinearKernel::WIDE:
@@ -1336,6 +1456,69 @@
 #undef SWV2_TNW
     SWV2_CHECK_LAUNCH("swv2_linear_wgrad");
     return SWV2_OK;
+}
+
+static bool dx_wgrad_shape(const swv2_operand* a, const swv2_epilogue* e, int N) {
+    return a->kind == SWV2_OP_HEADS && e->kind == SWV2_EPI_F32 && N == 128 && a->cols == 384 && a->p[0] == 8 && a->p[3] == 16 && a->ld == 3 && !a->rowidx &&
+           e->rowidx && e->aux && !e->bias && e->ld >= N && e->ld % 4 == 0;
+}
+
+size_t swv2_dx_wgrad_part_bytes(int C, int heads_dp) {
+#ifdef SWV2_SLAB_PART_F32
+    return 0;
+#else
+    return C == 128 && heads_dp == 128 ? (size_t)SWV2_DXW_SLICES * (3 * heads_dp * C * 2 + 3 * heads_dp * 4) : 0;
+#endif
+}
+
+int swv2_linear_dx_launch(const swv2_operand* a, const void* w, const swv2_epilogue* e, int N, const float* x, long xld, void* ws, int fused,
+                          hipStream_t st) {
+    SWV2_CHECK_ARG(dx_wgrad_shape(a, e, N), "swv2_linear_dx_wgrad: not the d(qkv) -> dx product of a C 128 block (head-major operand of 3 x 8 x 16 "
+                                            "columns, fp32 output of 128 columns with scatter table and residual, no bias)");
+    const int M = a->rows;
+    const Epi<E_F32> ep = make_epi<E_F32>(e, M, N);
+    RwWgrad wg = {};
+    if (fused) {
+        SWV2_CHECK_ARG(x && ws && xld >= N && xld % 4 == 0 && ((uintptr_t)x & 15) == 0 && ((uintptr_t)ws & 15) == 0,
+                       "swv2_linear_dx_wgrad: null / unaligned x or workspace");
+        SWV2_CHECK_ARG((double)M * 384 * 2 < 4.29e9, "swv2_linear_dx_wgrad: operand too large for 32-bit offsets (%d rows)", M);
+        wg.x = x; wg.xld = xld; wg.part = (uint16_t*)ws;
+        wg.dbpart = (float*)((char*)ws + (size_t)SWV2_DXW_SLICES * 384 * 128 * 2);
+        hipLaunchKernelGGL((gemm_rw_kernel<A_HEADS, E_F32, 128, 384, 64, 16, true>), dim3(SWV2_DXW_SLICES), dim3(512), 0, st, make_loader<A_HEADS>(a),
+                           (const uint16_t*)w, ep, M, wg);
+    } else {
+        hipLaunchKernelGGL((gemm_rw_kernel<A_HEADS, E_F32, 128, 384, 64>), dim3(256), dim3(512), 0, st, make_loader<A_HEADS>(a), (const uint16_t*)w, ep,
+                           M, wg);
+    }
+    SWV2_CHECK_LAUNCH("swv2_linear_dx_wgrad");
+    return SWV2_OK;
+}
+
+int swv2_block_dx_wgrad(const swv2_operand* a, const void* w, const swv2_epilogue* e, int N, const float* x, long xld, void* part, void* stream) {
+    return swv2_linear_dx_launch(a, w, e, N, x, xld, part, 1, (hipStream_t)stream);
+}
+
+extern "C" size_t swv2_dx_wgrad_ws_bytes(int C, int heads_dp) { return swv2_dx_wgrad_part_bytes(C, heads_dp); }
+
+extern "C" int swv2_linear_dx_wgrad_kernel(const swv2_operand* a, const swv2_epilogue* e, int N, size_t ws_bytes) {
+    SWV2_CHECK_ARG(a && e && N > 0 && a->rows > 0 && a->cols > 0, "swv2_linear_dx_wgrad_kernel: null operand / epilogue or empty product");
+    if (!dx_wgrad_shape(a, e, N)) {
+        swv2_set_error("swv2_linear_dx_wgrad_kernel: not the d(qkv) -> dx product of a C 128 block");
+        return SWV2_ERR_UNSUPPORTED;
+    }
+    const size_t need = swv2_dx_wgrad_part_bytes(N, a->cols / 3);
+    return need && ws_bytes >= need ? SWV2_LINEAR_RESIDENT_DX128_WGRAD : SWV2_LINEAR_RESIDENT_DX128;
+}
+
+extern "C" int swv2_linear_dx_wgrad(const swv2_operand* a, const void* w_bf16, const swv2_epilogue* e, int N, const float* x, long xld, void* ws,
+                                    size_t ws_bytes, void* stream) {
+    int rc = check_operand(a, "swv2_linear_dx_wgrad");
+    if (rc) return rc;
+    SWV2_CHECK_ARG(w_bf16 && e && e->out && N > 0, "swv2_linear_dx_wgrad: null weight / epilogue / N");
+    SWV2_CHECK_ARG(((uintptr_t)w_bf16 & 15) == 0 && ((uintptr_t)e->out & 15) == 0 && ((uintptr_t)e->aux & 15) == 0, "swv2_linear_dx_wgrad: unaligned pointer");
+    const int k = swv2_linear_dx_wgrad_kernel(a, e, N, ws ? ws_bytes : 0);
+    if (k < 0) return k;
+    return swv2_linear_dx_launch(a, w_bf16, e, N, x, xld, ws, k == SWV2_LINEAR_RESIDENT_DX128_WGRAD, (hipStream_t)stream);
 }
 
 #ifdef SWV2_RW_STAMPS
diff --git a/swin_v2_weather_amd/csrc/gemm_common.h b/swin_v2_weather_amd/csrc/gemm_common.h
--- a/swin_v2_weather_amd/csrc/gemm_common.h
+++ b/swin_v2_weather_amd/csrc/gemm_common.h
@@ -6,7 +6,13 @@
 
 size_t swv2_tn_slab_ws_bytes(int C, int hidden, int heads_dp);
 bool swv2_tn_slab_covers(const swv2_wgrad_item* it, size_t ws_bytes);
-int swv2_tn_slab_launch(const swv2_wgrad_item* it, void* ws, size_t ws_bytes, const swv2_ln_partials* ln, hipStream_t st);
+int swv2_tn_slab_launch(const swv2_wgrad_item* it, void* ws, size_t ws_bytes, const swv2_ln_partials* ln, const void* qkv_part, hipStream_t st);
+int swv2_tn_slab_fold_qkv(const void* qkv_part, int rows, float* dW, float* db, const int32_t* nmap, int ldw, hipStream_t st);
+
+constexpr int SWV2_DXW_SLICES = 256;
+size_t swv2_dx_wgrad_part_bytes(int C, int heads_dp);
+int swv2_linear_dx_launch(const swv2_operand* a, const void* w, const swv2_epilogue* e, int N, const float* x, long xld, void* ws, int fused,
+                          hipStream_t st);
 
 inline int swv2_env_switch(const char* name) { const char* v = getenv(name); return v ? atoi(v) : 1; }
 inline int swv2_gemm_wide() { return swv2_env_switch("SWV2_GEMM_WIDE"); }
diff --git a/swin_v2_weather_amd/csrc/gemm_tn.hip b/swin_v2_weather_amd/csrc/gemm_tn.hip
--- a/swin_v2_weather_amd/csrc/gemm_tn.hip
+++ b/swin_v2_weather_amd/csrc/gemm_tn.hip
@@ -516,8 +516,20 @@
     return std::max((size_t)group_slices(tt, slices) * tt * BN * BN * sizeof(float), swv2_tn_slab_ws_bytes(C, hidden, heads_dp));
 }
 
+size_t swv2_block_dx_part_offset(int C, int hidden, int heads_dp) { return (swv2_block_wgrad_ws_bytes(C, hidden, heads_dp, 0) + 255) / 256 * 256; }
+
+extern "C" size_t swv2_block_wgrad_dx_ws_bytes(int C, int hidden, int heads_dp) {
+    const size_t part = swv2_dx_wgrad_part_bytes(C, heads_dp);
+    return part && swv2_tn_slab_ws_bytes(C, hidden, heads_dp) ? swv2_block_dx_part_offset(C, hidden, heads_dp) + part : 0;
+}
+
+extern "C" int swv2_dx_wgrad_fold(const void* ws, size_t ws_bytes, int rows, float* dW, float* db, const int32_t* nmap, int ldw, void* stream) {
+    SWV2_CHECK_ARG(ws && ws_bytes >= swv2_dx_wgrad_part_bytes(128, 128), "swv2_dx_wgrad_fold: workspace smaller than swv2_dx_wgrad_ws_bytes");
+    return swv2_tn_slab_fold_qkv(ws, rows, dW, db, nmap, ldw, (hipStream_t)stream);
+}
+
 extern "C" int swv2_block_wgrad(const swv2_wgrad_item* it, int slices, void* ws, size_t ws_bytes, void* stream) {
-    return swv2_block_wgrad_ln(it, slices, ws, ws_bytes, nullptr, stream);
+    return swv2_block_wgrad_ln(it, slices, ws, ws_bytes, nullptr, nullptr, stream);
 }
 
 namespace {
@@ -564,7 +576,8 @@
     return (int)block_wgrad_kernel_for(it, slices, ws_bytes);
 }
 
-int swv2_block_wgrad_ln(const swv2_wgrad_item* it, int slices, void* ws, size_t ws_bytes, const swv2_ln_partials* ln, void* stream) {
+int swv2_block_wgrad_ln(const swv2_wgrad_item* it, int slices, void* ws, size_t ws_bytes, const swv2_ln_partials* ln, const void* qkv_part,
+                        void* stream) {
     SWV2_CHECK_ARG(it && ws, "swv2_block_wgrad: null items or workspace");
     static const int want[4][2] = {{SWV2_OP_BF16, SWV2_OP_BF16_GELU}, {SWV2_OP_BF16, SWV2_OP_F32}, {SWV2_OP_BF16, SWV2_OP_HEADS},
                                    {SWV2_OP_HEADS, SWV2_OP_F32}};
@@ -580,8 +593,9 @@
                        "swv2_block_wgrad: item %d: only the qkv product's X rows are gathered (and they must be)", i);
     }
     switch (block_wgrad_kernel_for(it, slices, ws_bytes)) {
-        case BlockWgradKernel::SLAB: return swv2_tn_slab_launch(it, ws, ws_bytes, ln, (hipStream_t)stream);
+        case BlockWgradKernel::SLAB: return swv2_tn_slab_launch(it, ws, ws_bytes, ln, qkv_part, (hipStream_t)stream);
         case BlockWgradKernel::GROUPED: break;
     }
+    SWV2_CHECK_ARG(!qkv_part, "swv2_block_wgrad: qkv partials of the dx kernel on offer, but the slab kernel does not run these items");
     return launch_tn_group(it, slices, ws, ws_bytes, ln, (hipStream_t)stream);
 }
diff --git a/swin_v2_weather_amd/csrc/gemm_tn_slab.hip b/swin_v2_weather_amd/csrc/gemm_tn_slab.hip
--- a/swin_v2_weather_amd/csrc/gemm_tn_slab.hip
+++ b/swin_v2_weather_amd/csrc/gemm_tn_slab.hip
@@ -533,7 +533,7 @@
 
 struct SlPlan { bool ok; int set; int wgs[4], ntile[4], S[4]; size_t part_off[4], db_off[4], total; };
 
-SlPlan sl_plan(const swv2_wgrad_item* it, int cus) {
+SlPlan sl_plan(const swv2_wgrad_item* it, int cus, bool qkv_done = false) {
     SlPlan p = {};
     const int N[4] = {it[0].dy.cols, it[1].dy.cols, it[2].dy.cols, it[3].dy.cols};
     const int K[4] = {it[0].x.cols, it[1].x.cols, it[2].x.cols, it[3].x.cols};
@@ -548,14 +548,15 @@
     if (cus < 16 || cus > 1024) return p;
     double cost[4], tot = 0;
     const double wgt[4] = {1.55, 1.0, 1.0, 1.1};
+    const int np = qkv_done ? 3 : 4;
     for (int i = 0; i < 4; ++i) {
         const double xb = it[i].x.kind == SWV2_OP_F32 ? 4.0 : 2.0;
         p.ntile[i] = (N[i] / sh.TN[i]) * (K[i] / sh.TK[i]);
-        cost[i] = wgt[i] * (double)it[i].dy.rows * (2.0 * N[i] * (K[i] / sh.TK[i]) + xb * K[i] * (N[i] / sh.TN[i]));
+        cost[i] = i < np ? wgt[i] * (double)it[i].dy.rows * (2.0 * N[i] * (K[i] / sh.TK[i]) + xb * K[i] * (N[i] / sh.TN[i])) : 0.0;
         tot += cost[i];
     }
     int used = 0;
-    for (int i = 0; i < 4; ++i) {
+    for (int i = 0; i < np; ++i) {
         const int T = cdiv(it[i].dy.rows, sh.SR[i]);
         int sl = (int)(cus * cost[i] / tot / p.ntile[i] + 0.5);
         sl = std::max(1, std::min(sl, T));
@@ -566,7 +567,7 @@
     for (int guard = 0; used != cus && guard < 64; ++guard) {
         int best = -1;
         double br = 0;
-        for (int i = 0; i < 4; ++i) {
+        for (int i = 0; i < np; ++i) {
             const int T = cdiv(it[i].dy.rows, sh.SR[i]);
             if (used < cus ? (p.S[i] >= T || used + p.ntile[i] > cus) : p.S[i] <= 1) continue;
             const double r = cost[i] / p.S[i];
@@ -578,7 +579,6 @@
     }
     size_t off = 0;
     for (int i = 0; i < 4; ++i) {
-        const int T = cdiv(it[i].dy.rows, sh.SR[i]);
         if ((double)it[i].dy.rows * std::max(N[i], K[i]) * 4.0 >= 4.29e9) return p;
         p.part_off[i] = off;
         off += (size_t)p.wgs[i] * sh.TN[i] * sh.TK[i] * sizeof(float);
@@ -623,9 +623,13 @@
     return pl.ok && ws_bytes >= pl.total;
 }
 
-int swv2_tn_slab_launch(const swv2_wgrad_item* it, void* ws, size_t ws_bytes, const swv2_ln_partials* ln, hipStream_t st) {
-    const SlPlan pl = sl_plan(it, sl_cus());
+int swv2_tn_slab_launch(const swv2_wgrad_item* it, void* ws, size_t ws_bytes, const swv2_ln_partials* ln, const void* qkv_part, hipStream_t st) {
+    SlPlan pl = sl_plan(it, sl_cus(), qkv_part != nullptr);
     SWV2_CHECK_ARG(pl.ok && ws_bytes >= pl.total, "swv2_block_wgrad(slab): items or workspace not covered (swv2_tn_slab_covers)");
+    if (qkv_part) {
+        SWV2_CHECK_ARG(pl.set == 0 && swv2_dx_wgrad_part_bytes(it[3].x.cols, it[3].dy.cols / 3), "swv2_block_wgrad(slab): qkv partials at a shape the dx kernel does not cover");
+        pl.S[3] = std::min(SWV2_DXW_SLICES, cdiv(it[3].dy.rows, 64));
+    }
     const SlShape& sh = SL_SETS[pl.set];
     SlArgs a = {};
     SlRedArgs r = {};
@@ -639,6 +643,10 @@
         p.y = sl_op(it[i].dy); p.x = sl_op(it[i].x);
         p.part = (sl_part_t*)((char*)ws + pl.part_off[i]);
         p.dbpart = it[i].db ? (float*)((char*)ws + pl.db_off[i]) : nullptr;
+        if (i == 3 && qkv_part) {
+            p.part = (sl_part_t*)qkv_part;
+            p.dbpart = it[i].db ? (float*)((char*)qkv_part + (size_t)SWV2_DXW_SLICES * 384 * 128 * 2) : nullptr;
+        }
         p.M = it[i].dy.rows; p.N = it[i].dy.cols; p.K = it[i].x.cols;
         p.first = first; p.wgs = pl.wgs[i]; p.ntile = pl.ntile[i];
         first += pl.wgs[i];
@@ -668,3 +676,20 @@
     SWV2_CHECK_LAUNCH("swv2_block_wgrad(slab)");
     return 0;
 }
+
+int swv2_tn_slab_fold_qkv(const void* qkv_part, int rows, float* dW, float* db, const int32_t* nmap, int ldw, hipStream_t st) {
+    SWV2_CHECK_ARG(qkv_part && dW && rows > 0 && ldw >= 128 && swv2_dx_wgrad_part_bytes(128, 128), "swv2_dx_wgrad_fold: null partials / dW, no rows or pitch < 128");
+    const SlShape& sh = SL_SETS[0];
+    SlRedArgs r = {};
+    r.cpw = 1;
+    SlRed& q = r.p[3];
+    q.dW = dW; q.db = db; q.nmap = nmap; q.kmap = nullptr; q.part = (const sl_part_t*)qkv_part;
+    q.dbpart = db ? (const float*)((const char*)qkv_part + (size_t)SWV2_DXW_SLICES * 384 * 128 * 2) : nullptr;
+    q.ldw = ldw; q.N = 384; q.K = 128; q.TN = sh.TN[3]; q.TK = sh.TK[3]; q.WGK = sh.WGK[3];
+    q.IA = sh.TN[3] / (16 * sh.WGN[3]); q.JB = sh.TK[3] / (16 * sh.WGK[3]); q.ntk = 1; q.S = std::min(SWV2_DXW_SLICES, cdiv(rows, 64));
+    r.total = q.N * q.K / 256;
+    r.dbtotal = cdiv(q.N, 64);
+    hipLaunchKernelGGL(tn_slab_reduce_kernel, dim3(r.total + r.dbtotal), dim3(512), 0, st, r);
+    SWV2_CHECK_LAUNCH("swv2_dx_wgrad_fold");
+    return 0;
+}
diff --git a/swin_v2_weather_amd/networks/swinv2_global.py b/swin_v2_weather_amd/networks/swinv2_global.py
--- a/swin_v2_weather_amd/networks/swinv2_global.py
+++ b/swin_v2_weather_amd/networks/swinv2_global.py
@@ -124,12 +124,13 @@
         d.wgrad_group = int(os.environ.get("SWV2_WGRAD_GROUP", "1"))
         d.fuse_mlp = int(os.environ.get("SWV2_FUSE_MLP", "1"))
         d.fuse_proj_ln = int(os.environ.get("SWV2_FUSE_PROJ_LN", "1"))
+        d.dx_wgrad = int(os.environ.get("SWV2_DX_WGRAD", "1"))
         d.wgrad_ws = d.grad_zero = 1
         d.ln_ws_floats = d.wgrad_ws_bytes = 1 << 62
         full = L.block_plan(d)
         d.ln_ws_floats, d.wgrad_ws_bytes = full.need_ln_ws_floats, full.need_wgrad_ws_bytes
         self.launch_plan = lp = L.block_plan(d)
-        if any(getattr(lp, n) != getattr(full, n) for n in ("mlp_fused", "proj_ln_fused", "ln_deferred", "wgrad_grouped", "wgrad_kernel")):
+        if any(getattr(lp, n) != getattr(full, n) for n in ("mlp_fused", "proj_ln_fused", "ln_deferred", "wgrad_grouped", "wgrad_kernel", "dx_wgrad")):
             raise L.Swv2Error("swv2_block_plan: the reported workspace needs do not cover the full plan")
         d.wgrad_ws = d.grad_zero = None
         self.desc = d
```
